# danping/CoSLAM

Measured on AMD Instinct MI355X. Metric: frames/sec for track+local-BA loop, 8 cams 640x480 x 2000 feats (one frame = all 8 cameras), higher is better.
Workload: dtype f32 (KLT, f16 pyramid storage) + f64 (pose, BA)

## Files before the change

### coslam_amd/csrc/ncc.hip

```cpp
#include "cs_common.h"
#include "small_ops.h"

#pragma clang fp contract(off)

namespace {

constexpr int NC_HW = 5, NC_BW = 11, NC_LEN = 121, NC_PITCH = 128;

__global__ __launch_bounds__(256) void k_ncc_blocks(const unsigned char* __restrict__ img, int W, int H, int n,
                                                    const double* __restrict__ xs, const double* __restrict__ ys, double scale,
                                                    unsigned char* __restrict__ blocks, double* __restrict__ abc,
                                                    int* __restrict__ valid) {
    const int lane = threadIdx.x & 63;
    const int i = blockIdx.x * 4 + (threadIdx.x >> 6);
    if (i >= n) return;
    const double x = xs[i] * scale, y = ys[i] * scale;
    const int x0 = (int)x, y0 = (int)y;
    const bool ok = !(x0 - NC_HW < 0 || x0 + NC_HW >= W || y0 - NC_HW < 0 || y0 + NC_HW >= H);
    unsigned v0 = 0x80, v1 = 0x80;
    if (ok) {
        const int j0 = lane, j1 = lane + 64;
        const int yy0 = j0 / NC_BW, xx0 = j0 - yy0 * NC_BW;
        v0 = img[(size_t)(y0 + yy0 - NC_HW) * W + (x0 + xx0 - NC_HW)];
        if (j1 < NC_LEN) {
            const int yy1 = j1 / NC_BW, xx1 = j1 - yy1 * NC_BW;
            v1 = img[(size_t)(y0 + yy1 - NC_HW) * W + (x0 + xx1 - NC_HW)];
        }
    }
    blocks[(size_t)i * NC_PITCH + lane] = (unsigned char)v0;
    blocks[(size_t)i * NC_PITCH + 64 + lane] = (unsigned char)v1;
    const unsigned w0 = ok ? v0 : 0u, w1 = (ok && lane + 64 < NC_LEN) ? v1 : 0u;
    unsigned a = w0 + w1;
    unsigned b = w0 * w0 + w1 * w1;
#pragma unroll
    for (int off = 32; off >= 1; off >>= 1) {
        a += __shfl_xor(a, off, 64);
        b += __shfl_xor(b, off, 64);
    }
    if (lane == 0) {
        valid[i] = ok ? 1 : 0;
        const double A = (double)a, B = (double)b;
        abc[4 * (size_t)i] = ok ? A : 0.0;
        abc[4 * (size_t)i + 1] = ok ? B : 0.0;
        abc[4 * (size_t)i + 2] = ok ? 1 / sqrt((double)NC_LEN * B - A * A) : 0.0;
        abc[4 * (size_t)i + 3] = ok ? A / (double)NC_LEN : 0.0;
    }
}

__device__ __forceinline__ int nc_floorf(float v) {
    const int i = (int)v;
    return i - (i > v);
}
__device__ __forceinline__ int nc_clip(int x, int a, int b) { return x >= a ? (x < b ? x : b - 1) : a; }
__device__ __forceinline__ int nc_sat_short(int v) { return v < -32768 ? -32768 : (v > 32767 ? 32767 : v); }

constexpr int NC_MAX_CAMS = 16;
struct NcCamSet {
    const unsigned char* img[NC_MAX_CAMS];
    unsigned char* scaled[NC_MAX_CAMS];
    const double* x[NC_MAX_CAMS];
    const double* y[NC_MAX_CAMS];
    unsigned char* blocks[NC_MAX_CAMS];
    double* abc[NC_MAX_CAMS];
    int* valid[NC_MAX_CAMS];
};

__global__ __launch_bounds__(256) void k_resize_linear_u8(NcCamSet S, int W, int H, double scale_x, double scale_y, int Wd, int Hd) {
    const unsigned char* __restrict__ src = S.img[blockIdx.z];
    unsigned char* __restrict__ dst = S.scaled[blockIdx.z];
    const int dx = blockIdx.x * 64 + (threadIdx.x & 63), dy = blockIdx.y * 4 + (threadIdx.x >> 6);
    if (dx >= Wd || dy >= Hd) return;
    float fx = (float)((dx + 0.5) * scale_x - 0.5);
    int sx = nc_floorf(fx);
    fx -= sx;
    if (sx < 0) fx = 0, sx = 0;
    bool edge = false;
    if (sx + 1 >= W) {
        edge = true;
        if (sx >= W - 1) fx = 0, sx = W - 1;
    }
    const int a0 = nc_sat_short(__float2int_rn((1.f - fx) * 2048.f)), a1 = nc_sat_short(__float2int_rn(fx * 2048.f));
    float fy = (float)((dy + 0.5) * scale_y - 0.5);
    const int sy = nc_floorf(fy);
    fy -= sy;
    const int b0 = nc_sat_short(__float2int_rn((1.f - fy) * 2048.f)), b1 = nc_sat_short(__float2int_rn(fy * 2048.f));
    const unsigned char* S0 = src + (size_t)nc_clip(sy, 0, H) * W;
    const unsigned char* S1 = src + (size_t)nc_clip(sy + 1, 0, H) * W;
    int r0, r1;
    if (!edge) {
        r0 = S0[sx] * a0 + S0[sx + 1] * a1;
        r1 = S1[sx] * a0 + S1[sx + 1] * a1;
    } else {
        r0 = S0[sx] * 2048;
        r1 = S1[sx] * 2048;
    }
    dst[(size_t)dy * Wd + dx] = (unsigned char)((((b0 * (r0 >> 4)) >> 16) + ((b1 * (r1 >> 4)) >> 16) + 2) >> 2);
}

__global__ __launch_bounds__(256) void k_ncc_blocks_subpix(NcCamSet S, int W, int H, int n, double scale, int scaled) {
    const int cam = blockIdx.y;
    const unsigned char* __restrict__ img = scaled ? S.scaled[cam] : S.img[cam];
    const double* __restrict__ xs = S.x[cam];
    const double* __restrict__ ys = S.y[cam];
    unsigned char* __restrict__ blocks = S.blocks[cam];
    double* __restrict__ abc = S.abc[cam];
    int* __restrict__ valid = S.valid[cam];
    const int lane = threadIdx.x & 63;
    const int p = blockIdx.x * 4 + (threadIdx.x >> 6);
    if (p >= n) return;
    const int win = NC_BW;
    const double px = scaled ? xs[p] * scale : xs[p], py = scaled ? ys[p] * scale : ys[p];
    float fxc = (float)px, fyc = (float)py;
    fxc -= (win - 1) * 0.5f;
    fyc -= (win - 1) * 0.5f;
    const int ipx = nc_floorf(fxc), ipy = nc_floorf(fyc);
    const float a = fxc - ipx, b = fyc - ipy;
    const int a11 = __float2int_rn((1.f - a) * (1.f - b) * 65536.f), a12 = __float2int_rn(a * (1.f - b) * 65536.f),
              a21 = __float2int_rn((1.f - a) * b * 65536.f), a22 = __float2int_rn(a * b * 65536.f);
    const int b1 = __float2int_rn((1.f - b) * 65536.f), b2 = __float2int_rn(b * 65536.f);
    const bool inside = 0 <= ipx && ipx < W - win && 0 <= ipy && ipy < H - win;
    int rx = 0, rw = win, ry = 0, rh = win, col0 = ipx, row0 = ipy;
    if (!inside) {
        if (ipx >= 0) {
            col0 = ipx, rx = 0;
        } else {
            col0 = 0, rx = -ipx;
            if (rx > win) rx = win;
        }
        if (ipx < W - win) {
            rw = win;
        } else {
            rw = W - ipx - 1;
            if (rw < 0) col0 += rw, rw = 0;
        }
        if (ipy >= 0) {
            row0 = ipy, ry = 0;
        } else {
            row0 = 0, ry = -ipy;
        }
        if (ipy < H - win) {
            rh = win;
        } else {
            rh = H - ipy - 1;
            if (rh < 0) row0 += rh, rh = 0;
        }
    }
    unsigned v[2] = {0x80u, 0x80u};
#pragma unroll
    for (int h = 0; h < 2; ++h) {
        const int q = lane + 64 * h;
        if (q >= NC_LEN) continue;
        const int i = q / win, j = q - i * win;
        int t;
        if (inside) {
            const unsigned char* s = img + (size_t)(ipy + i) * W + ipx;
            t = s[j] * a11 + s[j + 1] * a12 + s[j + W] * a21 + s[j + W + 1] * a22;
        } else {
            const int adv = (i < rh ? i : rh) - ry;
            const int rt = row0 + (adv > 0 ? adv : 0);
            const int rb = rt + ((i < ry || i >= rh) ? 0 : 1);
            const unsigned char* s = img + (size_t)rt * W + (col0 - rx);
            const unsigned char* s2 = img + (size_t)rb * W + (col0 - rx);
            if (j < rx)
                t = s[rx] * b1 + s2[rx] * b2;
            else if (j >= rw)
                t = s[rw] * b1 + s2[rw] * b2;
            else
                t = s[j] * a11 + s[j + 1] * a12 + s2[j] * a21 + s2[j + 1] * a22;
        }
        v[h] = (unsigned)((t + (1 << 15)) >> 16) & 0xffu;
    }
    blocks[(size_t)p * NC_PITCH + lane] = (unsigned char)v[0];
    blocks[(size_t)p * NC_PITCH + 64 + lane] = (unsigned char)v[1];
    const unsigned w0 = v[0], w1 = (lane + 64 < NC_LEN) ? v[1] : 0u;
    unsigned sa = w0 + w1;
    unsigned sb = w0 * w0 + w1 * w1;
#pragma unroll
    for (int off = 32; off >= 1; off >>= 1) {
        sa += __shfl_xor(sa, off, 64);
        sb += __shfl_xor(sb, off, 64);
    }
    if (lane == 0) {
        const double A = (double)sa, B = (double)sb;
        abc[4 * (size_t)p] = A;
        abc[4 * (size_t)p + 1] = B;
        abc[4 * (size_t)p + 2] = 1 / sqrt((double)NC_LEN * B - A * A);
        abc[4 * (size_t)p + 3] = A / (double)NC_LEN;
        if (valid) valid[p] = 1;
    }
}

__global__ __launch_bounds__(256) void k_ncc_unmapped_mask(int n, const int* __restrict__ state, const int* __restrict__ slot2map,
                                                           int* __restrict__ valid) {
    const int i = blockIdx.x * 256 + threadIdx.x;
    if (i < n) valid[i] = (state[i] >= 0 && slot2map[i] < 0) ? 1 : 0;
}

struct NcSide {
    const double* x;
    const double* y;
    const unsigned char* blocks;
    const double* abc;
    const int* valid;
    int n;
};
struct NcArgs {
    double F[9];
    const double* dF;
    NcSide s1, s2;
    double epiMax, nccMin, wNone;
    double* epiMat;
    double* nccMat;
    cs_ncc_pair* pairs;
    int pairCap;
    int* pairCount;
};

typedef int nc_i32x4 __attribute__((ext_vector_type(4)));

__device__ __forceinline__ long nc_row_chunk(const unsigned char* blocks, int row, int n, int byteOff) {
    if (row >= n) return 0;
    const unsigned long long u = *(const unsigned long long*)(blocks + (size_t)row * NC_PITCH + byteOff);
    return (long)(u ^ 0x8080808080808080ull);
}

constexpr int NC_MAX_JOBS = 8;
struct NcJobs {
    NcArgs job[NC_MAX_JOBS];
};
constexpr int NC_CT = 4;
constexpr int NC_TP = 136;
constexpr int NC_TILE_BYTES = 64 * NC_TP + 64 * 40;
struct NcColRegs {
    nc_i32x4 q0, q1;
    double x, y, A, C;
    int valid;
};
__device__ __forceinline__ void nc_tile_fetch(const NcSide& S2, int j0, int N, int tid, NcColRegs& r) {
    const int row = j0 + (tid >> 2);
    r.q0 = r.q1 = (nc_i32x4){0, 0, 0, 0};
    if (row < N) {
        const nc_i32x4* src = (const nc_i32x4*)(S2.blocks + (size_t)row * NC_PITCH + 32 * (tid & 3));
        r.q0 = src[0], r.q1 = src[1];
        const int sh = (int)0x80808080;
#pragma unroll
        for (int k = 0; k < 4; ++k) r.q0[k] ^= sh, r.q1[k] ^= sh;
    }
    r.x = r.y = r.A = r.C = 0.0, r.valid = 0;
    if (tid < 64 && j0 + tid < N) {
        const int j = j0 + tid;
        r.x = S2.x[j], r.y = S2.y[j], r.A = S2.abc[4 * (size_t)j], r.C = S2.abc[4 * (size_t)j + 2], r.valid = S2.valid[j];
    }
}
__device__ __forceinline__ void nc_tile_store(unsigned char* buf, int tid, const NcColRegs& r) {
    nc_i32x4* dst = (nc_i32x4*)(buf + (tid >> 2) * NC_TP + 32 * (tid & 3));
    long* d8 = (long*)dst;
    const long* s8 = (const long*)&r.q0;
    d8[0] = s8[0], d8[1] = s8[1];
    s8 = (const long*)&r.q1;
    d8[2] = s8[0], d8[3] = s8[1];
    if (tid < 64) {
        double* c = (double*)(buf + 64 * NC_TP);
        c[tid] = r.x, c[64 + tid] = r.y, c[128 + tid] = r.A, c[192 + tid] = r.C;
        ((int*)(c + 256))[tid] = r.valid;
    }
}
template <bool SPARSE>
__global__ __launch_bounds__(256) void k_ncc_epi_mat(NcJobs J) {
    __shared__ __attribute__((aligned(16))) unsigned char sTile[2][NC_TILE_BYTES];
    const NcArgs& A = J.job[blockIdx.z];
    const int tid = threadIdx.x, lane = tid & 63, wv = tid >> 6;
    const int M = A.s1.n, N = A.s2.n;
    if ((int)blockIdx.y * 64 >= M || (int)blockIdx.x * NC_CT * 64 >= N) return;
    const int i0 = blockIdx.y * 64 + 16 * wv;
    const bool rowsIn = i0 < M;
    double Fm[9];
#pragma unroll
    for (int k = 0; k < 9; ++k) Fm[k] = A.dF ? A.dF[k] : A.F[k];
    const int lr = lane & 15, lk = lane >> 4;
    long a[4];
#pragma unroll
    for (int ks = 0; ks < 4; ++ks) a[ks] = nc_row_chunk(A.s1.blocks, i0 + lr, M, 32 * ks + 8 * lk);
    double x1[4], y1[4], A1[4], C1[4];
    int v1[4], s1[4];
#pragma unroll
    for (int r = 0; r < 4; ++r) {
        const int i = i0 + 4 * lk + r;
        const bool in = i < M;
        x1[r] = in ? A.s1.x[i] : 0.0;
        y1[r] = in ? A.s1.y[i] : 0.0;
        A1[r] = in ? A.s1.abc[4 * (size_t)i] : 0.0;
        C1[r] = in ? A.s1.abc[4 * (size_t)i + 2] : 0.0;
        v1[r] = in ? A.s1.valid[i] : 0;
        s1[r] = (int)A1[r] - NC_LEN * 128;
    }
    const int jBase = blockIdx.x * NC_CT * 64;
    NcColRegs cr;
    nc_tile_fetch(A.s2, jBase, N, tid, cr);
    nc_tile_store(sTile[0], tid, cr);
    __syncthreads();
    for (int ct = 0; ct < NC_CT; ++ct) {
        const int j0 = jBase + ct * 64;
        if (j0 >= N) break;
        const bool more = ct + 1 < NC_CT && j0 + 64 < N;
        if (more) nc_tile_fetch(A.s2, j0 + 64, N, tid, cr);
        const unsigned char* tile = sTile[ct & 1];
        const double* cc = (const double*)(tile + 64 * NC_TP);
        const int* cv = (const int*)(cc + 256);
        if (rowsIn) {
            nc_i32x4 acc[4];
#pragma unroll
            for (int t = 0; t < 4; ++t) acc[t] = (nc_i32x4){0, 0, 0, 0};
#pragma unroll
            for (int ks = 0; ks < 4; ++ks) {
                const int off = 32 * ks + 8 * lk;
                long b[4];
#pragma unroll
                for (int t = 0; t < 4; ++t) b[t] = *(const long*)(tile + (16 * t + lr) * NC_TP + off);
#pragma unroll
                for (int t = 0; t < 4; ++t) acc[t] = __builtin_amdgcn_mfma_i32_16x16x32_i8(a[ks], b[t], acc[t], 0, 0, 0);
            }
#pragma unroll
            for (int t = 0; t < 4; ++t) {
                const int jl = 16 * t + lr, j = j0 + jl;
                if (j >= N) continue;
                const double bx = cc[jl], by = cc[64 + jl];
                const double A2 = cc[128 + jl], C2 = cc[192 + jl];
                const int v2 = cv[jl];
                const int s2 = (int)A2 - NC_LEN * 128;
                const double l0 = (Fm[0] * bx + Fm[1] * by) + Fm[2];
                const double l1 = (Fm[3] * bx + Fm[4] * by) + Fm[5];
                const double l2 = (Fm[6] * bx + Fm[7] * by) + Fm[8];
                const double nn = sqrt(l0 * l0 + l1 * l1);
                const double den = nn > 0 ? nn : 1.0;
                const double numMax = (A.epiMax * den) * (1.0 + 1e-12);
#pragma unroll
                for (int r = 0; r < 4; ++r) {
                    const int i = i0 + 4 * lk + r;
                    if (i >= M) continue;
                    const double num = fabs((l0 * x1[r] + l1 * y1[r]) + l2);
                    double e = A.wNone, c = A.wNone;
                    bool pass = false;
                    double epiErr = 0;
                    bool near = v1[r] && v2 && !(num > numMax);
                    if (near) {
                        epiErr = num / den;
                        near = epiErr <= A.epiMax;
                    }
                    if (near) {
                        const int d = acc[t][r] + 128 * s1[r] + 128 * s2 + NC_LEN * 128 * 128;
                        const double ncc = (((double)NC_LEN * (double)d - A1[r] * A2) * C1[r]) * C2;
                        if (ncc >= A.nccMin) {
                            e = epiErr;
                            c = ncc;
                            pass = true;
                        }
                    }
                    if (SPARSE) {
                        if (pass) {
                            const int at = atomicAdd(A.pairCount, 1);
                            if (at < A.pairCap) {
                                cs_ncc_pair q;
                                q.i = i, q.j = j, q.epi = e, q.ncc = c;
                                A.pairs[at] = q;
                            }
                        }
                    } else {
                        A.epiMat[(size_t)i * N + j] = e;
                        A.nccMat[(size_t)i * N + j] = c;
                    }
                }
            }
        }
        if (more) nc_tile_store(sTile[(ct + 1) & 1], tid, cr);
        __syncthreads();
    }
}

}

extern "C" int cs_ncc_blocks_dev(int device, void* hip_stream, const unsigned char* d_img, int W, int H, int n, const double* d_x,
                                 const double* d_y, double scale, unsigned char* d_blocks, double* d_abc, int* d_valid) {
    if (W < NC_BW || H < NC_BW || n < 0 || !(scale > 0)) {
        cs_set_error("cs_ncc_blocks_dev: bad arguments (image at least 11 x 11, scale > 0)");
        return CS_ERR_INVALID;
    }
    if (n == 0) return CS_OK;
    if (!d_img || !d_x || !d_y || !d_blocks || !d_abc || !d_valid) {
        cs_set_error("cs_ncc_blocks_dev: null pointer");
        return CS_ERR_INVALID;
    }
    CS_HIP(hipSetDevice(device));
    hipLaunchKernelGGL(k_ncc_blocks, dim3((unsigned)((n + 3) / 4)), dim3(256), 0, (hipStream_t)hip_stream, d_img, W, H, n, d_x, d_y,
                       scale, d_blocks, d_abc, d_valid);
    CS_CHECK_LAUNCH();
    return CS_OK;
}

extern "C" int cs_ncc_unmapped_mask_dev(int device, void* hip_stream, int n, const int* d_state, const int* d_slot2map, int* d_valid) {
    if (n < 0 || (n && (!d_state || !d_slot2map || !d_valid))) {
        cs_set_error("cs_ncc_unmapped_mask_dev: bad arguments");
        return CS_ERR_INVALID;
    }
    if (n == 0) return CS_OK;
    CS_HIP(hipSetDevice(device));
    hipLaunchKernelGGL(k_ncc_unmapped_mask, dim3((n + 255) / 256), dim3(256), 0, (hipStream_t)hip_stream, n, d_state, d_slot2map, d_valid);
    CS_CHECK_LAUNCH();
    return CS_OK;
}

extern "C" int cs_ncc_scaled_dims(int W, int H, double scale, int* Ws, int* Hs) {
    if (!Ws || !Hs || W <= 0 || H <= 0 || !(scale > 0)) {
        cs_set_error("cs_ncc_scaled_dims: bad arguments");
        return CS_ERR_INVALID;
    }
    *Ws = (int)lrint(W * scale);
    *Hs = (int)lrint(H * scale);
    return CS_OK;
}

static int ncc_get_blocks_group_impl(int device, void* hip_stream, int nCams, const cs_ncc_cam* cams, int W, int H, int n, double scale,
                                     bool writeValid);
extern "C" int cs_ncc_get_blocks_dev(int device, void* hip_stream, const unsigned char* d_img, int W, int H, int n, const double* d_x,
                                     const double* d_y, double scale, unsigned char* d_scaled, unsigned char* d_blocks, double* d_abc,
                                     int* d_valid) {
    if (!d_img || W <= 0 || H <= 0 || n < 0 || (n && (!d_x || !d_y || !d_blocks || !d_abc)) || !(scale > 0) ||
        (scale != 1.0 && !d_scaled)) {
        cs_set_error("cs_ncc_get_blocks_dev: bad arguments");
        return CS_ERR_INVALID;
    }
    cs_ncc_cam one;
    memset(&one, 0, sizeof(one));
    one.img = d_img, one.x = d_x, one.y = d_y, one.scaled = d_scaled, one.blocks = d_blocks, one.abc = d_abc, one.valid = d_valid;
    return ncc_get_blocks_group_impl(device, hip_stream, 1, &one, W, H, n, scale, true);
}

extern "C" int cs_ncc_get_blocks_group_dev(int device, void* hip_stream, int nCams, const cs_ncc_cam* cams, int W, int H, int n,
                                           double scale) {
    return ncc_get_blocks_group_impl(device, hip_stream, nCams, cams, W, H, n, scale, false);
}
static int ncc_get_blocks_group_impl(int device, void* hip_stream, int nCams, const cs_ncc_cam* cams, int W, int H, int n, double scale,
                                     bool writeValid) {
    if (nCams < 1 || nCams > NC_MAX_CAMS || !cams || W <= 0 || H <= 0 || n < 0 || !(scale > 0)) {
        cs_set_error("cs_ncc_get_blocks_group_dev: bad arguments (1..%d cameras)", NC_MAX_CAMS);
        return CS_ERR_INVALID;
    }
    NcCamSet S;
    memset(&S, 0, sizeof(S));
    for (int c = 0; c < nCams; ++c) {
        const cs_ncc_cam& q = cams[c];
        if (!q.img || (n && (!q.x || !q.y || !q.blocks || !q.abc)) || (scale != 1.0 && !q.scaled)) {
            cs_set_error("cs_ncc_get_blocks_group_dev: null pointer in camera %d", c);
            return CS_ERR_INVALID;
        }
        S.img[c] = q.img, S.scaled[c] = q.scaled, S.x[c] = q.x, S.y[c] = q.y, S.blocks[c] = q.blocks, S.abc[c] = q.abc, S.valid[c] = writeValid ? q.valid : nullptr;
    }
    CS_HIP(hipSetDevice(device));
    hipStream_t s = (hipStream_t)hip_stream;
    int Ws = W, Hs = H;
    if (scale != 1.0) {
        Ws = (int)lrint(W * scale), Hs = (int)lrint(H * scale);
        if (Ws < 1 || Hs < 1) {
            cs_set_error("cs_ncc_get_blocks_group_dev: the scaled image is empty");
            return CS_ERR_INVALID;
        }
        hipLaunchKernelGGL(k_resize_linear_u8, dim3((Ws + 63) / 64, (Hs + 3) / 4, nCams), dim3(256), 0, s, S, W, H, 1. / scale, 1. / scale, Ws, Hs);
    }
    if (n > 0) hipLaunchKernelGGL(k_ncc_blocks_subpix, dim3((n + 3) / 4, nCams), dim3(256), 0, s, S, Ws, Hs, n, scale, scale != 1.0 ? 1 : 0);
    CS_CHECK_LAUNCH();
    return CS_OK;
}

extern "C" int cs_ncc_get_scaled_blocks_group_dev(int device, void* hip_stream, int nCams, const cs_ncc_cam* cams, int Ws, int Hs, int n,
                                                  double scale) {
    if (nCams < 1 || nCams > NC_MAX_CAMS || !cams || Ws <= 0 || Hs <= 0 || n < 0 || !(scale > 0)) {
        cs_set_error("cs_ncc_get_scaled_blocks_group_dev: bad arguments (1..%d cameras)", NC_MAX_CAMS);
        return CS_ERR_INVALID;
    }
    NcCamSet S;
    memset(&S, 0, sizeof(S));
    for (int c = 0; c < nCams; ++c) {
        const cs_ncc_cam& q = cams[c];
        if (!q.img || (n && (!q.x || !q.y || !q.blocks || !q.abc))) {
            cs_set_error("cs_ncc_get_scaled_blocks_group_dev: null pointer in camera %d", c);
            return CS_ERR_INVALID;
        }
        S.img[c] = q.img, S.scaled[c] = const_cast<unsigned char*>(q.img) , S.x[c] = q.x, S.y[c] = q.y;
        S.blocks[c] = q.blocks, S.abc[c] = q.abc, S.valid[c] = nullptr;
    }
    if (n == 0) return CS_OK;
    CS_HIP(hipSetDevice(device));
    hipLaunchKernelGGL(k_ncc_blocks_subpix, dim3((n + 3) / 4, nCams), dim3(256), 0, (hipStream_t)hip_stream, S, Ws, Hs, n, scale, 1);
    CS_CHECK_LAUNCH();
    return CS_OK;
}

extern "C" int cs_ncc_small_dims(int W, int H, double scale, int* Ws, int* Hs) {
    if (!Ws || !Hs || W <= 0 || H <= 0 || !(scale > 0)) {
        cs_set_error("cs_ncc_small_dims: bad arguments");
        return CS_ERR_INVALID;
    }
    *Ws = (int)(W * scale);
    *Hs = (int)(H * scale);
    return CS_OK;
}
extern "C" int cs_ncc_small_image_dev(int device, void* hip_stream, const unsigned char* d_img, int W, int H, double scale,
                                      unsigned char* d_small) {
    int Ws = 0, Hs = 0;
    if (!d_img || !d_small || cs_ncc_small_dims(W, H, scale, &Ws, &Hs) != CS_OK || Ws < 1 || Hs < 1) {
        cs_set_error("cs_ncc_small_image_dev: bad arguments (%d x %d, scale %g)", W, H, scale);
        return CS_ERR_INVALID;
    }
    NcCamSet S;
    memset(&S, 0, sizeof(S));
    S.img[0] = d_img, S.scaled[0] = d_small;
    CS_HIP(hipSetDevice(device));
    const double inv_x = (double)Ws / W, inv_y = (double)Hs / H;
    hipLaunchKernelGGL(k_resize_linear_u8, dim3((Ws + 63) / 64, (Hs + 3) / 4, 1), dim3(256), 0, (hipStream_t)hip_stream, S, W, H, 1. / inv_x,
                       1. / inv_y, Ws, Hs);
    CS_CHECK_LAUNCH();
    return CS_OK;
}

extern "C" int cs_ncc_epi_mat_dev(int device, void* hip_stream, const double F[9], int M, const double* d_x1, const double* d_y1,
                                  const unsigned char* d_blocks1, const double* d_abc1, const int* d_valid1, int N,
                                  const double* d_x2, const double* d_y2, const unsigned char* d_blocks2, const double* d_abc2,
                                  const int* d_valid2, double epiMax, double nccMin, double wNone, double* d_epiMat,
                                  double* d_nccMat) {
    if (!F || M < 0 || N < 0) {
        cs_set_error("cs_ncc_epi_mat_dev: bad arguments");
        return CS_ERR_INVALID;
    }
    if (M == 0 || N == 0) return CS_OK;
    if (!d_x1 || !d_y1 || !d_blocks1 || !d_abc1 || !d_valid1 || !d_x2 || !d_y2 || !d_blocks2 || !d_abc2 || !d_valid2 || !d_epiMat ||
        !d_nccMat) {
        cs_set_error("cs_ncc_epi_mat_dev: null pointer");
        return CS_ERR_INVALID;
    }
    NcArgs A;
    memset(&A, 0, sizeof(A));
    memcpy(A.F, F, sizeof(A.F));
    A.s1 = {d_x1, d_y1, d_blocks1, d_abc1, d_valid1, M};
    A.s2 = {d_x2, d_y2, d_blocks2, d_abc2, d_valid2, N};
    A.epiMax = epiMax;
    A.nccMin = nccMin;
    A.wNone = wNone;
    A.epiMat = d_epiMat;
    A.nccMat = d_nccMat;
    CS_HIP(hipSetDevice(device));
    A.pairs = nullptr, A.pairCap = 0, A.pairCount = nullptr;
    NcJobs J;
    J.job[0] = A;
    hipLaunchKernelGGL(k_ncc_epi_mat<false>, dim3((unsigned)((N + 64 * NC_CT - 1) / (64 * NC_CT)), (unsigned)((M + 63) / 64)), dim3(256), 0,
                       (hipStream_t)hip_stream, J);
    CS_CHECK_LAUNCH();
    return CS_OK;
}

extern "C" int cs_ncc_epi_pairs_dev(int device, void* hip_stream, const double F[9], int M, const double* d_x1, const double* d_y1,
                                    const unsigned char* d_blocks1, const double* d_abc1, const int* d_valid1, int N, const double* d_x2,
                                    const double* d_y2, const unsigned char* d_blocks2, const double* d_abc2, const int* d_valid2,
                                    double epiMax, double nccMin, cs_ncc_pair* d_pairs, int pairCap, int* d_pairCount) {
    if (!F || M < 0 || N < 0 || pairCap < 0 || !d_pairCount || (pairCap > 0 && !d_pairs)) {
        cs_set_error("cs_ncc_epi_pairs_dev: bad arguments");
        return CS_ERR_INVALID;
    }
    CS_HIP(hipSetDevice(device));
    CS_HIP(hipMemsetAsync(d_pairCount, 0, sizeof(int), (hipStream_t)hip_stream));
    if (M == 0 || N == 0) return CS_OK;
    if (!d_x1 || !d_y1 || !d_blocks1 || !d_abc1 || !d_valid1 || !d_x2 || !d_y2 || !d_blocks2 || !d_abc2 || !d_valid2) {
        cs_set_error("cs_ncc_epi_pairs_dev: null pointer");
        return CS_ERR_INVALID;
    }
    NcArgs A;
    memset(&A, 0, sizeof(A));
    memcpy(A.F, F, sizeof(A.F));
    A.s1 = {d_x1, d_y1, d_blocks1, d_abc1, d_valid1, M};
    A.s2 = {d_x2, d_y2, d_blocks2, d_abc2, d_valid2, N};
    A.epiMax = epiMax;
    A.nccMin = nccMin;
    A.wNone = -1.0;
    A.epiMat = A.nccMat = nullptr;
    A.pairs = d_pairs, A.pairCap = pairCap, A.pairCount = d_pairCount;
    NcJobs J;
    J.job[0] = A;
    hipLaunchKernelGGL(k_ncc_epi_mat<true>, dim3((unsigned)((N + 64 * NC_CT - 1) / (64 * NC_CT)), (unsigned)((M + 63) / 64)), dim3(256), 0,
                       (hipStream_t)hip_stream, J);
    CS_CHECK_LAUNCH();
    return CS_OK;
}

struct NcFmArgs {
    int n;
    int camA[NC_MAX_JOBS], camB[NC_MAX_JOBS];
    const double* iK[NC_MAX_JOBS][2];
    const double *R, *t;
    double* F;
};
__global__ void k_ncc_fmats(NcFmArgs A) {
    const int k = threadIdx.x;
    if (k >= A.n) return;
    const double *Ra = A.R + 9 * A.camA[k], *Rb = A.R + 9 * A.camB[k], *ta = A.t + 3 * A.camA[k], *tb = A.t + 3 * A.camB[k];
    double R[9], t[3], E[9], T[9];
    for (int i = 0; i < 3; ++i)
        for (int j = 0; j < 3; ++j) R[3 * i + j] = (Ra[3 * i] * Rb[3 * j] + Ra[3 * i + 1] * Rb[3 * j + 1]) + Ra[3 * i + 2] * Rb[3 * j + 2];
    for (int i = 0; i < 3; ++i) t[i] = ta[i] - ((R[3 * i] * tb[0] + R[3 * i + 1] * tb[1]) + R[3 * i + 2] * tb[2]);
    const double X[9] = {0, -t[2], t[1], t[2], 0, -t[0], -t[1], t[0], 0};
    for (int i = 0; i < 3; ++i)
        for (int j = 0; j < 3; ++j) E[3 * i + j] = (X[3 * i] * R[j] + X[3 * i + 1] * R[3 + j]) + X[3 * i + 2] * R[6 + j];
    const double *Ka = A.iK[k][0], *Kb = A.iK[k][1];
    for (int i = 0; i < 3; ++i)
        for (int j = 0; j < 3; ++j) T[3 * i + j] = (Ka[i] * E[j] + Ka[3 + i] * E[3 + j]) + Ka[6 + i] * E[6 + j];
    for (int i = 0; i < 3; ++i)
        for (int j = 0; j < 3; ++j) A.F[9 * k + 3 * i + j] = (T[3 * i] * Kb[j] + T[3 * i + 1] * Kb[3 + j]) + T[3 * i + 2] * Kb[6 + j];
}
extern "C" int cs_ncc_fmats_dev(int device, void* hip_stream, int nCams, int nPairs, const int* camA, const int* camB, const double* const* d_iK,
                                const double* d_R, const double* d_t, double* d_F) {
    if (nCams < 1 || nPairs < 0 || nPairs > NC_MAX_JOBS || (nPairs && (!camA || !camB || !d_iK || !d_R || !d_t || !d_F))) {
        cs_set_error("cs_ncc_fmats_dev: bad arguments (<= %d pairs)", NC_MAX_JOBS);
        return CS_ERR_INVALID;
    }
    if (nPairs == 0) return CS_OK;
    NcFmArgs A;
    memset(&A, 0, sizeof(A));
    A.n = nPairs, A.R = d_R, A.t = d_t, A.F = d_F;
    for (int k = 0; k < nPairs; ++k) {
        if (camA[k] < 0 || camA[k] >= nCams || camB[k] < 0 || camB[k] >= nCams || !d_iK[camA[k]] || !d_iK[camB[k]]) {
            cs_set_error("cs_ncc_fmats_dev: bad pair %d", k);
            return CS_ERR_INVALID;
        }
        A.camA[k] = camA[k], A.camB[k] = camB[k], A.iK[k][0] = d_iK[camA[k]], A.iK[k][1] = d_iK[camB[k]];
    }
    CS_HIP(hipSetDevice(device));
    hipLaunchKernelGGL(k_ncc_fmats, dim3(1), dim3(64), 0, (hipStream_t)hip_stream, A);
    CS_CHECK_LAUNCH();
    return CS_OK;
}

extern "C" int cs_ncc_epi_pairs_group_dev(int device, void* hip_stream, int nCams, const cs_ncc_cam* cams, int n, int nJobs,
                                          const cs_ncc_pair_job* jobs, double epiMax, double nccMin, int pairCap) {
    if (nCams < 1 || nCams > NC_MAX_CAMS || !cams || n < 0 || nJobs < 0 || nJobs > NC_MAX_JOBS || (nJobs && !jobs) || pairCap < 0) {
        cs_set_error("cs_ncc_epi_pairs_group_dev: bad arguments (<= %d camera pairs per call)", NC_MAX_JOBS);
        return CS_ERR_INVALID;
    }
    if (nJobs == 0) return CS_OK;
    CS_HIP(hipSetDevice(device));
    hipStream_t s = (hipStream_t)hip_stream;
    NcJobs J;
    memset(&J, 0, sizeof(J));
    cs_small::List zero;
    for (int k = 0; k < nJobs; ++k) {
        const cs_ncc_pair_job& q = jobs[k];
        if (q.camA < 0 || q.camA >= nCams || q.camB < 0 || q.camB >= nCams || !q.count || (pairCap > 0 && !q.pairs)) {
            cs_set_error("cs_ncc_epi_pairs_group_dev: bad job %d", k);
            return CS_ERR_INVALID;
        }
        const cs_ncc_cam &a = cams[q.camA], &b = cams[q.camB];
        if (n && (!a.x || !a.y || !a.blocks || !a.abc || !a.valid || !b.x || !b.y || !b.blocks || !b.abc || !b.valid)) {
            cs_set_error("cs_ncc_epi_pairs_group_dev: null pointer in a camera of job %d", k);
            return CS_ERR_INVALID;
        }
        NcArgs& A = J.job[k];
        memcpy(A.F, q.F, sizeof(A.F));
        A.dF = q.dF;
        A.s1 = {a.x, a.y, a.blocks, a.abc, a.valid, n};
        A.s2 = {b.x, b.y, b.blocks, b.abc, b.valid, n};
        A.epiMax = epiMax, A.nccMin = nccMin, A.wNone = -1.0;
        A.epiMat = A.nccMat = nullptr;
        A.pairs = q.pairs, A.pairCap = pairCap, A.pairCount = q.count;
        zero.fill(q.count, 0, sizeof(int));
    }
    CS_HIP(zero.run(s));
    if (n == 0) return CS_OK;
    hipLaunchKernelGGL(k_ncc_epi_mat<true>, dim3((unsigned)((n + 64 * NC_CT - 1) / (64 * NC_CT)), (unsigned)((n + 63) / 64), (unsigned)nJobs), dim3(256), 0, s, J);
    CS_CHECK_LAUNCH();
    return CS_OK;
}

static int ncc_match_between_impl(int cutter, int device, const unsigned char* img1, int W1, int H1, int M, const double* x1,
                                  const double* y1, const unsigned char* img2, int W2, int H2, int N, const double* x2, const double* y2,
                                  double scale, const double F[9], double epiMax, double nccMin, double wNone, double* epiMat,
                                  double* nccMat, unsigned char* blocks1, double* abc1, int* valid1, unsigned char* blocks2,
                                  double* abc2, int* valid2) {
    if (!img1 || !img2 || !F || M < 0 || N < 0 || (M && (!x1 || !y1)) || (N && (!x2 || !y2)) || (M && N && (!epiMat || !nccMat))) {
        cs_set_error("cs_ncc_match_between: bad arguments");
        return CS_ERR_INVALID;
    }
    if (M == 0 || N == 0) return CS_OK;
    CS_HIP(hipSetDevice(device));
    const size_t i1 = (size_t)W1 * H1, i2 = (size_t)W2 * H2;
    auto al = [](size_t v) { return (v + 255) & ~(size_t)255; };
    size_t off = 0;
    const size_t oI1 = off; off += al(i1);
    const size_t oI2 = off; off += al(i2);
    const size_t oX1 = off; off += al(8 * (size_t)M);
    const size_t oY1 = off; off += al(8 * (size_t)M);
    const size_t oX2 = off; off += al(8 * (size_t)N);
    const size_t oY2 = off; off += al(8 * (size_t)N);
    const size_t inBytes = off;
    const size_t oB1 = off; off += al(128 * (size_t)M);
    const size_t oB2 = off; off += al(128 * (size_t)N);
    const size_t oC1 = off; off += al(32 * (size_t)M);
    const size_t oC2 = off; off += al(32 * (size_t)N);
    const size_t oV1 = off; off += al(4 * (size_t)M);
    const size_t oV2 = off; off += al(4 * (size_t)N);
    const size_t oE = off; off += al(8 * (size_t)M * N);
    const size_t oN = off; off += al(8 * (size_t)M * N);
    const size_t oS1 = off; off += al(cutter ? i1 : 0);
    const size_t oS2 = off; off += al(cutter ? i2 : 0);
    char* d = nullptr;
    if (hipMalloc((void**)&d, off) != hipSuccess) {
        cs_set_error("cs_ncc_match_between: out of device memory (%zu bytes)", off);
        return CS_ERR_HIP;
    }
    hipStream_t s = nullptr;
    int rc = CS_OK;
    hipError_t e = hipMemcpyAsync(d + oI1, img1, i1, hipMemcpyHostToDevice, s);
    if (e == hipSuccess) e = hipMemcpyAsync(d + oI2, img2, i2, hipMemcpyHostToDevice, s);
    if (e == hipSuccess) e = hipMemcpyAsync(d + oX1, x1, 8 * (size_t)M, hipMemcpyHostToDevice, s);
    if (e == hipSuccess) e = hipMemcpyAsync(d + oY1, y1, 8 * (size_t)M, hipMemcpyHostToDevice, s);
    if (e == hipSuccess) e = hipMemcpyAsync(d + oX2, x2, 8 * (size_t)N, hipMemcpyHostToDevice, s);
    if (e == hipSuccess) e = hipMemcpyAsync(d + oY2, y2, 8 * (size_t)N, hipMemcpyHostToDevice, s);
    (void)inBytes;
    if (cutter && scale > 1.0) {
        (void)hipFree(d);
        cs_set_error("cs_ncc_match_between_full: scale > 1 is not supported");
        return CS_ERR_INVALID;
    }
    if (e == hipSuccess && cutter) {
        rc = cs_ncc_get_blocks_dev(device, s, (const unsigned char*)(d + oI1), W1, H1, M, (const double*)(d + oX1), (const double*)(d + oY1),
                                   scale, (unsigned char*)(d + oS1), (unsigned char*)(d + oB1), (double*)(d + oC1), (int*)(d + oV1));
        if (rc == CS_OK)
            rc = cs_ncc_get_blocks_dev(device, s, (const unsigned char*)(d + oI2), W2, H2, N, (const double*)(d + oX2),
                                       (const double*)(d + oY2), scale, (unsigned char*)(d + oS2), (unsigned char*)(d + oB2),
                                       (double*)(d + oC2), (int*)(d + oV2));
        if (rc == CS_OK)
            rc = cs_ncc_epi_mat_dev(device, s, F, M, (const double*)(d + oX1), (const double*)(d + oY1), (const unsigned char*)(d + oB1),
                                    (const double*)(d + oC1), (const int*)(d + oV1), N, (const double*)(d + oX2),
                                    (const double*)(d + oY2), (const unsigned char*)(d + oB2), (const double*)(d + oC2),
                                    (const int*)(d + oV2), epiMax, nccMin, wNone, (double*)(d + oE), (double*)(d + oN));
    } else if (e == hipSuccess) {
        rc = cs_ncc_blocks_dev(device, s, (const unsigned char*)(d + oI1), W1, H1, M, (const double*)(d + oX1), (const double*)(d + oY1),
                               scale, (unsigned char*)(d + oB1), (double*)(d + oC1), (int*)(d + oV1));
        if (rc == CS_OK)
            rc = cs_ncc_blocks_dev(device, s, (const unsigned char*)(d + oI2), W2, H2, N, (const double*)(d + oX2),
                                   (const double*)(d + oY2), scale, (unsigned char*)(d + oB2), (double*)(d + oC2), (int*)(d + oV2));
        if (rc == CS_OK)
            rc = cs_ncc_epi_mat_dev(device, s, F, M, (const double*)(d + oX1), (const double*)(d + oY1), (const unsigned char*)(d + oB1),
                                    (const double*)(d + oC1), (const int*)(d + oV1), N, (const double*)(d + oX2),
                                    (const double*)(d + oY2), (const unsigned char*)(d + oB2), (const double*)(d + oC2),
                                    (const int*)(d + oV2), epiMax, nccMin, wNone, (double*)(d + oE), (double*)(d + oN));
    }
    if (rc == CS_OK && e == hipSuccess) e = hipMemcpyAsync(epiMat, d + oE, 8 * (size_t)M * N, hipMemcpyDeviceToHost, s);
    if (rc == CS_OK && e == hipSuccess) e = hipMemcpyAsync(nccMat, d + oN, 8 * (size_t)M * N, hipMemcpyDeviceToHost, s);
    auto back = [&](void* dst, size_t o, size_t bytes) {
        if (dst && rc == CS_OK && e == hipSuccess) e = hipMemcpyAsync(dst, d + o, bytes, hipMemcpyDeviceToHost, s);
    };
    back(blocks1, oB1, 128 * (size_t)M);
    back(blocks2, oB2, 128 * (size_t)N);
    back(abc1, oC1, 32 * (size_t)M);
    back(abc2, oC2, 32 * (size_t)N);
    back(valid1, oV1, 4 * (size_t)M);
    back(valid2, oV2, 4 * (size_t)N);
    if (rc == CS_OK && e == hipSuccess) e = hipStreamSynchronize(s);
    (void)hipFree(d);
    if (rc != CS_OK) return rc;
    if (e != hipSuccess) {
        cs_set_error("cs_ncc_match_between: %s", hipGetErrorString(e));
        return CS_ERR_HIP;
    }
    return CS_OK;
}

extern "C" int cs_ncc_match_between(int device, const unsigned char* img1, int W1, int H1, int M, const double* x1, const double* y1,
                                    const unsigned char* img2, int W2, int H2, int N, const double* x2, const double* y2,
                                    double scale, const double F[9], double epiMax, double nccMin, double wNone, double* epiMat,
                                    double* nccMat, unsigned char* blocks1, double* abc1, int* valid1, unsigned char* blocks2,
                                    double* abc2, int* valid2) {
    return ncc_match_between_impl(0, device, img1, W1, H1, M, x1, y1, img2, W2, H2, N, x2, y2, scale, F, epiMax, nccMin, wNone, epiMat,
                                  nccMat, blocks1, abc1, valid1, blocks2, abc2, valid2);
}

extern "C" int cs_ncc_match_between_full(int device, const unsigned char* img1, int W1, int H1, int M, const double* x1, const double* y1,
                                         const unsigned char* img2, int W2, int H2, int N, const double* x2, const double* y2,
                                         double scale, const double F[9], double epiMax, double nccMin, double wNone, double* epiMat,
                                         double* nccMat, unsigned char* blocks1, double* abc1, unsigned char* blocks2, double* abc2) {
    return ncc_match_between_impl(1, device, img1, W1, H1, M, x1, y1, img2, W2, H2, N, x2, y2, scale, F, epiMax, nccMin, wNone, epiMat,
                                  nccMat, blocks1, abc1, nullptr, blocks2, abc2, nullptr);
}
```

### coslam_amd/csrc/newpts.hip

```cpp
#include "cs_common.h"
#include "small_ops.h"

#pragma clang fp contract(off)

namespace {

constexpr int NP_MAX_CAMS = 16, NP_MAX_CAND = 2048, NP_MAX_SEEDS = 512, NP_MAX_TRACKS = 4096, NP_MAX_N = 32768;
constexpr int NP_MAX_DYN = 4096;
constexpr int NP_SEGS = 8;
constexpr int NP_DYN_PER_CAM = 1024;

struct NpArgs {
    int nCams, N, mapCap, curFrame, pairCap, minLen, W, H;
    double maxDisp, maxRpErr, sigma;
    const cs_ncc_pair* pairs[NP_MAX_CAMS];
    const int* pairCount[NP_MAX_CAMS];
    cs_poseupdate_cam cam[NP_MAX_CAMS];
    const double *R, *t;
    double *mapPts, *mapCov;
    unsigned char *mapFlags, *newPt;
    int *firstFrame, *pointFeat;
    int* mapCount;
    int* matchIdx;
    unsigned* rowMask;
    unsigned* colMask;
    int* seedIdx;
    int* seedCnt;
    unsigned* dynList;
    int* dynCnt;
    int* counts;
};

__device__ __forceinline__ bool np_before(double sa, unsigned ia, double sb, unsigned ib) {
    return sa > sb || (sa == sb && ia < ib);
}

__global__ __launch_bounds__(256) void k_np_prep(NpArgs A) {
    __shared__ int wTot[4];
    __shared__ int sBase;
    const int tid = threadIdx.x, lane = tid & 63, wv = tid >> 6, N = A.N, C = A.nCams, nP = C - 1;
    if (blockIdx.x == 0 && A.counts && tid < 4 + C) A.counts[tid] = 0;
    if ((int)blockIdx.x < nP * NP_SEGS) {
        const int a = blockIdx.x / NP_SEGS, seg = blockIdx.x % NP_SEGS, b = a + 1;
        const int cap = *A.mapCount < A.mapCap ? *A.mapCount : A.mapCap;
        const int per = ((cap + NP_SEGS - 1) / NP_SEGS + 255) / 256 * 256;
        const int m0 = seg * per, m1 = min(m0 + per, cap);
        int* out = A.seedIdx + ((size_t)a * NP_SEGS + seg) * NP_MAX_SEEDS;
        if (tid == 0) sBase = 0;
        __syncthreads();
        for (int c0 = m0; c0 < m1 && sBase < NP_MAX_SEEDS; c0 += 256) {
            const int m = c0 + tid;
            bool in = false;
            if (m < m1) {
                const unsigned char fl = A.mapFlags[m];
                in = !(fl & (CS_MAP_FALSE | CS_MAP_UNCERTAIN)) && A.pointFeat[(size_t)m * C + a] >= 0 && A.pointFeat[(size_t)m * C + b] >= 0;
            }
            const unsigned long long bal = __builtin_amdgcn_ballot_w64(in);
            if (lane == 0) wTot[wv] = __popcll(bal);
            __syncthreads();
            int k = sBase;
            for (int w = 0; w < wv; ++w) k += wTot[w];
            k += __popcll(bal & ((1ull << lane) - 1ull));
            if (in && k < NP_MAX_SEEDS) out[k] = m;
            __syncthreads();
            if (tid == 0) sBase = min(sBase + wTot[0] + wTot[1] + wTot[2] + wTot[3], NP_MAX_SEEDS);
            __syncthreads();
        }
        if (tid == 0) A.seedCnt[a * NP_SEGS + seg] = sBase;
        return;
    }
    const int c = blockIdx.x - nP * NP_SEGS;
    if (c >= C) return;
    if (tid == 0) sBase = 0;
    __syncthreads();
    for (int sl = tid; sl < N; sl += 256) {
        const int st = A.cam[c].state[sl], m = A.cam[c].slot2map[sl];
        if ((st == 0 || st == 1) && m >= 0 && m < A.mapCap && A.mapFlags[m] == CS_MAP_DYNAMIC) {
            const int x = (int)(A.cam[c].xy[sl] + 0.5), y = (int)(A.cam[c].xy[N + sl] + 0.5);
            if (x + 20 >= 0 && x - 20 < A.W && y + 20 >= 0 && y - 20 < A.H) {
                const int k = atomicAdd(&sBase, 1);
                if (k < NP_DYN_PER_CAM) A.dynList[(size_t)c * NP_DYN_PER_CAM + k] = ((unsigned)(y + 64) << 12) | (unsigned)(x + 64);
            }
        }
    }
    __syncthreads();
    if (tid == 0) A.dynCnt[c] = sBase;
}

__global__ __launch_bounds__(256) void k_np_match(NpArgs A) {
    __shared__ double sKey[NP_MAX_CAND];
    __shared__ unsigned sIdx[NP_MAX_CAND];
    __shared__ double sSeed[NP_MAX_SEEDS][4];
    __shared__ unsigned sRow[NP_MAX_N / 32], sCol[NP_MAX_N / 32];
    __shared__ int sNSeeds, sNCand;
    const int a = blockIdx.x, b = a + 1, tid = threadIdx.x, lane = tid & 63, wv = tid >> 6, N = A.N, C = A.nCams;
    const int nWords = (N + 31) / 32;
    for (int q = tid; q < nWords; q += 256) sRow[q] = 0, sCol[q] = 0;
    {
        int off[NP_SEGS + 1];
        off[0] = 0;
#pragma unroll
        for (int g = 0; g < NP_SEGS; ++g) off[g + 1] = off[g] + A.seedCnt[a * NP_SEGS + g];
        const int total = off[NP_SEGS] < NP_MAX_SEEDS ? off[NP_SEGS] : NP_MAX_SEEDS;
        if (tid == 0) sNSeeds = total, sNCand = 0;
        for (int k = tid; k < total; k += 256) {
            int g = 0, base = 0;
#pragma unroll
            for (int q = 1; q < NP_SEGS; ++q)
                if (k >= off[q]) g = q, base = off[q];
            const int m = A.seedIdx[((size_t)a * NP_SEGS + g) * NP_MAX_SEEDS + (k - base)];
            const int s1 = A.pointFeat[(size_t)m * C + a], s2 = A.pointFeat[(size_t)m * C + b];
            const double x1 = A.cam[a].xy[s1], y1 = A.cam[a].xy[N + s1], x2 = A.cam[b].xy[s2], y2 = A.cam[b].xy[N + s2];
            sSeed[k][0] = x1, sSeed[k][1] = y1, sSeed[k][2] = x2 - x1, sSeed[k][3] = y2 - y1;
        }
    }
    __syncthreads();
    const int nSeeds = sNSeeds;
    int nAll = *A.pairCount[a];
    if (nAll > A.pairCap) {
        nAll = A.pairCap;
        if (tid == 0 && A.counts) atomicOr(A.counts + 3, 1);
    }
    for (int q = wv; q < nAll; q += 4) {
        const cs_ncc_pair p = A.pairs[a][q];
        bool ok = p.i >= 0 && p.i < N && p.j >= 0 && p.j < N;
        if (ok && nSeeds > 0) {
            const double x1 = A.cam[a].xy[p.i], y1 = A.cam[a].xy[N + p.i];
            double best = 1.0e300;
            int bk = 0x7fffffff;
            for (int k = lane; k < nSeeds; k += 64) {
                const double dx = sSeed[k][0] - x1, dy = sSeed[k][1] - y1, d2 = dx * dx + dy * dy;
                if (d2 < best) best = d2, bk = k;
            }
#pragma unroll
            for (int off = 1; off < 64; off <<= 1) {
                const double ob = __shfl_xor(best, off, 64);
                const int ok_ = __shfl_xor(bk, off, 64);
                if (ob < best || (ob == best && ok_ < bk)) best = ob, bk = ok_;
            }
            if (bk == 0x7fffffff) bk = 0;
            const double ex = (A.cam[b].xy[p.j] - x1) - sSeed[bk][2];
            const double ey = (A.cam[b].xy[N + p.j] - y1) - sSeed[bk][3];
            ok = sqrt(ex * ex + ey * ey) <= A.maxDisp;
        }
        if (ok && lane == 0) {
            const int k = atomicAdd(&sNCand, 1);
            if (k < NP_MAX_CAND) sKey[k] = p.ncc, sIdx[k] = ((unsigned)p.i << 16) | (unsigned)p.j;
        }
    }
    __syncthreads();
    int L = sNCand;
    if (L > NP_MAX_CAND) {
        L = NP_MAX_CAND;
        if (tid == 0 && A.counts) atomicOr(A.counts + 3, 1);
    }
    int L2 = 1;
    while (L2 < L) L2 <<= 1;
    for (int q = L + tid; q < L2; q += 256) sKey[q] = -1.0e300, sIdx[q] = 0xFFFFFFFFu;
    __syncthreads();
    for (int k = 2; k <= L2; k <<= 1)
        for (int j = k >> 1; j > 0; j >>= 1) {
            for (int q = tid; q < L2; q += 256) {
                const int x = q ^ j;
                if (x > q) {
                    const bool up = (q & k) == 0;
                    const double ka = sKey[q], kb = sKey[x];
                    const unsigned ia = sIdx[q], ib = sIdx[x];
                    if (np_before(kb, ib, ka, ia) == up) sKey[q] = kb, sIdx[q] = ib, sKey[x] = ka, sIdx[x] = ia;
                }
            }
            __syncthreads();
        }
    if (tid == 0) {
        int n = 0;
        int* match = A.matchIdx + (size_t)a * N;
        for (int q = 0; q < L; ++q) {
            const unsigned id = sIdx[q], i = id >> 16, j = id & 0xFFFFu;
            if ((sRow[i >> 5] >> (i & 31)) & 1u) continue;
            if ((sCol[j >> 5] >> (j & 31)) & 1u) continue;
            sRow[i >> 5] |= 1u << (i & 31), sCol[j >> 5] |= 1u << (j & 31);
            match[i] = (int)j;
            ++n;
        }
        if (A.counts) A.counts[4 + a] = n;
    }
    __syncthreads();
    for (int q = tid; q < nWords; q += 256) A.rowMask[(size_t)a * nWords + q] = sRow[q], A.colMask[(size_t)a * nWords + q] = sCol[q];
}

constexpr int NP_LPT = 8;
constexpr int NP_TPB = 256 / NP_LPT;
static_assert(NP_MAX_CAMS <= 2 * NP_LPT, "a lane holds two views of a track");

struct NpTerm {
    double n[6], g[3];
};
__device__ __forceinline__ double np_pick(double a, double b, bool second) { return second ? b : a; }
__device__ __forceinline__ int np_pick_i(int a, int b, bool second) { return second ? b : a; }

__global__ __launch_bounds__(256) void k_np_reconstruct(NpArgs A) {
    __shared__ int sBase, sNTracks, sWave[4];
    __shared__ unsigned sTrk[NP_MAX_TRACKS];
    __shared__ int sDynOff[NP_MAX_CAMS + 2];
    const int tid = threadIdx.x, N = A.N, C = A.nCams, nP = C - 1;
    const int lane = tid & 63, wv = tid >> 6, r = tid & (NP_LPT - 1), gbase = lane & ~(NP_LPT - 1);
    if (tid == 0) sBase = 0, sNTracks = 0;
    __syncthreads();
    const int nWords = (N + 31) / 32, totalW = nP * nWords;
    for (int w0 = 0; w0 < totalW; w0 += 256) {
        const int w = w0 + tid;
        unsigned bits = 0;
        int a = 0, q = 0;
        if (w < totalW) {
            a = w / nWords, q = w - a * nWords;
            bits = A.rowMask[w];
            if (a > 0) bits &= ~A.colMask[(size_t)(a - 1) * nWords + q];
        }
        const int cnt = __popc(bits);
        int inc = cnt;
#pragma unroll
        for (int o = 1; o < 64; o <<= 1) {
            const int v = __shfl_up(inc, o, 64);
            if (lane >= o) inc += v;
        }
        if (lane == 63) sWave[wv] = inc;
        __syncthreads();
        int before = inc - cnt, total = 0;
        for (int k = 0; k < 4; ++k) {
            if (k < wv) before += sWave[k];
            total += sWave[k];
        }
        int rank = sNTracks + before;
        while (bits) {
            const int bit = __ffs(bits) - 1;
            bits &= bits - 1;
            if (rank < NP_MAX_TRACKS) sTrk[rank] = ((unsigned)a << 16) | (unsigned)(32 * q + bit);
            ++rank;
        }
        __syncthreads();
        if (tid == 0) sNTracks = min(sNTracks + total, NP_MAX_TRACKS);
        __syncthreads();
    }
    const int nTracks = sNTracks;
    int nLong = 0;
    for (int t0 = 0; t0 < nTracks; t0 += NP_TPB) {
        const int tk = t0 + tid / NP_LPT;
        int nv = 0, c0 = 0, vs0 = -1, vs1 = -1;
        if (tk < nTracks) {
            int c = (int)(sTrk[tk] >> 16), sl = (int)(sTrk[tk] & 0xFFFFu);
            c0 = c;
            for (;;) {
                if ((nv & (NP_LPT - 1)) == r) (nv < NP_LPT ? vs0 : vs1) = sl;
                ++nv;
                if (c >= nP || !((A.rowMask[(size_t)c * nWords + (sl >> 5)] >> (sl & 31)) & 1u)) break;
                sl = A.matchIdx[(size_t)c * N + sl];
                ++c;
            }
        }
        const bool lng = tk < nTracks && nv >= A.minLen;
        if (lng && r == 0) ++nLong;
        bool valid = false;
        double M[3] = {0, 0, 0}, cov[9] = {0, 0, 0, 0, 0, 0, 0, 0, 0}, err0 = 0, err1 = 0;
        unsigned char fl = 0;
        {
            NpTerm T0, T1;
#pragma unroll
            for (int kk = 0; kk < 2; ++kk) {
                NpTerm& T = kk ? T1 : T0;
#pragma unroll
                for (int q = 0; q < 6; ++q) T.n[q] = 0;
#pragma unroll
                for (int q = 0; q < 3; ++q) T.g[q] = 0;
                const int k = r + NP_LPT * kk, sl = kk ? vs1 : vs0;
                if (!lng || k >= nv) continue;
                const int cam = c0 + k;
                const cs_poseupdate_cam& Cm = A.cam[cam];
                const double* R = A.R + 9 * cam;
                const double* t = A.t + 3 * cam;
                const double mx = Cm.xy[sl], my = Cm.xy[N + sl];
                const double* iK = Cm.iK;
                const double w = (iK[6] * mx + iK[7] * my) + iK[8];
                const double x = ((iK[0] * mx + iK[1] * my) + iK[2]) / w, y = ((iK[3] * mx + iK[4] * my) + iK[5]) / w;
                const double a0[3] = {R[0] - x * R[6], R[1] - x * R[7], R[2] - x * R[8]}, a1[3] = {R[3] - y * R[6], R[4] - y * R[7], R[5] - y * R[8]};
                const double b0 = x * t[2] - t[0], b1 = y * t[2] - t[1];
                T.n[0] = a0[0] * a0[0] + a1[0] * a1[0];
                T.n[1] = a0[0] * a0[1] + a1[0] * a1[1];
                T.n[2] = a0[0] * a0[2] + a1[0] * a1[2];
                T.n[3] = a0[1] * a0[1] + a1[1] * a1[1];
                T.n[4] = a0[1] * a0[2] + a1[1] * a1[2];
                T.n[5] = a0[2] * a0[2] + a1[2] * a1[2];
#pragma unroll
                for (int q = 0; q < 3; ++q) T.g[q] = a0[q] * b0 + a1[q] * b1;
            }
            double Nn[6] = {0, 0, 0, 0, 0, 0}, g[3] = {0, 0, 0};
            for (int k = 0; k < NP_MAX_CAMS; ++k) {
                if (!__builtin_amdgcn_ballot_w64(lng && k < nv)) break;
                const int src = gbase + (k & (NP_LPT - 1));
                const bool second = k >= NP_LPT;
                double tn[6], tg[3];
#pragma unroll
                for (int q = 0; q < 6; ++q) tn[q] = __shfl(np_pick(T0.n[q], T1.n[q], second), src, 64);
#pragma unroll
                for (int q = 0; q < 3; ++q) tg[q] = __shfl(np_pick(T0.g[q], T1.g[q], second), src, 64);
                if (lng && k < nv) {
#pragma unroll
                    for (int q = 0; q < 6; ++q) Nn[q] = Nn[q] + tn[q];
#pragma unroll
                    for (int q = 0; q < 3; ++q) g[q] = g[q] + tg[q];
                }
            }
            double cf[6];
            if (lng) {
                cf[0] = Nn[3] * Nn[5] - Nn[4] * Nn[4], cf[1] = Nn[2] * Nn[4] - Nn[1] * Nn[5], cf[2] = Nn[1] * Nn[4] - Nn[2] * Nn[3];
                cf[3] = Nn[0] * Nn[5] - Nn[2] * Nn[2], cf[4] = Nn[1] * Nn[2] - Nn[0] * Nn[4], cf[5] = Nn[0] * Nn[3] - Nn[1] * Nn[1];
                const double det = (Nn[0] * cf[0] + Nn[1] * cf[1]) + Nn[2] * cf[2];
                M[0] = ((cf[0] * g[0] + cf[1] * g[1]) + cf[2] * g[2]) / det;
                M[1] = ((cf[1] * g[0] + cf[3] * g[1]) + cf[4] * g[2]) / det;
                M[2] = ((cf[2] * g[0] + cf[4] * g[1]) + cf[5] * g[2]) / det;
            }
            double S0[6], S1[6];
            bool out = false, dyn0 = false, dyn1 = false;
#pragma unroll
            for (int kk = 0; kk < 2; ++kk) {
                double* Sx = kk ? S1 : S0;
#pragma unroll
                for (int q = 0; q < 6; ++q) Sx[q] = 0;
                const int k = r + NP_LPT * kk, sl = kk ? vs1 : vs0;
                if (!lng || k >= nv) continue;
                const int cam = c0 + k;
                const cs_poseupdate_cam& Cm = A.cam[cam];
                const double* K = Cm.K;
                const double* R = A.R + 9 * cam;
                const double* t = A.t + 3 * cam;
                const double X = ((R[0] * M[0] + R[1] * M[1]) + R[2] * M[2]) + t[0];
                const double Y = ((R[3] * M[0] + R[4] * M[1]) + R[5] * M[2]) + t[1];
                const double Z = ((R[6] * M[0] + R[7] * M[1]) + R[8] * M[2]) + t[2];
                const double u = (K[0] * X + K[1] * Y) + K[2] * Z, vv = (K[3] * X + K[4] * Y) + K[5] * Z, w = (K[6] * X + K[7] * Y) + K[8] * Z;
                const double dx = Cm.xy[sl] - u / w, dy = Cm.xy[N + sl] - vv / w;
                const double e = sqrt(dx * dx + dy * dy);
                (kk ? err1 : err0) = e;
                if (e > A.maxRpErr || Z < 0) out = true;
                if (Cm.isStatic && !Cm.isStatic[sl]) (kk ? dyn1 : dyn0) = true;
                double KR[9], J[6];
#pragma unroll
                for (int i = 0; i < 3; ++i)
#pragma unroll
                    for (int j = 0; j < 3; ++j) KR[3 * i + j] = (K[3 * i] * R[j] + K[3 * i + 1] * R[3 + j]) + K[3 * i + 2] * R[6 + j];
                const double ww = w * w;
#pragma unroll
                for (int j = 0; j < 3; ++j) J[j] = (KR[j] * w - u * KR[6 + j]) / ww, J[3 + j] = (KR[3 + j] * w - vv * KR[6 + j]) / ww;
                Sx[0] = J[0] * J[0] + J[3] * J[3];
                Sx[1] = J[0] * J[1] + J[3] * J[4];
                Sx[2] = J[0] * J[2] + J[3] * J[5];
                Sx[3] = J[1] * J[1] + J[4] * J[4];
                Sx[4] = J[1] * J[2] + J[4] * J[5];
                Sx[5] = J[2] * J[2] + J[5] * J[5];
            }
            double S[6] = {0, 0, 0, 0, 0, 0};
            int nDyn = (dyn0 ? 1 : 0) + (dyn1 ? 1 : 0);
            for (int k = 0; k < NP_MAX_CAMS; ++k) {
                if (!__builtin_amdgcn_ballot_w64(lng && k < nv)) break;
                const int src = gbase + (k & (NP_LPT - 1));
                const bool second = k >= NP_LPT;
                double ts[6];
#pragma unroll
                for (int q = 0; q < 6; ++q) ts[q] = __shfl(np_pick(S0[q], S1[q], second), src, 64);
                if (lng && k < nv) {
#pragma unroll
                    for (int q = 0; q < 6; ++q) S[q] = S[q] + ts[q];
                }
            }
#pragma unroll
            for (int o = 1; o < NP_LPT; o <<= 1) {
                out |= __shfl_xor((int)out, o, 64) != 0;
                nDyn += __shfl_xor(nDyn, o, 64);
            }
            if (lng && !out) {
                valid = true;
                cf[0] = S[3] * S[5] - S[4] * S[4], cf[1] = S[2] * S[4] - S[1] * S[5], cf[2] = S[1] * S[4] - S[2] * S[3];
                cf[3] = S[0] * S[5] - S[2] * S[2], cf[4] = S[1] * S[2] - S[0] * S[4], cf[5] = S[0] * S[3] - S[1] * S[1];
                const double dS = (S[0] * cf[0] + S[1] * cf[1]) + S[2] * cf[2], s2 = A.sigma * A.sigma;
                cov[0] = (cf[0] / dS) * s2, cov[1] = (cf[1] / dS) * s2, cov[2] = (cf[2] / dS) * s2;
                cov[3] = cov[1], cov[4] = (cf[3] / dS) * s2, cov[5] = (cf[4] / dS) * s2;
                cov[6] = cov[2], cov[7] = cov[5], cov[8] = (cf[5] / dS) * s2;
                fl = nDyn > 1 ? CS_MAP_DYNAMIC : CS_MAP_UNCERTAIN;
            }
        }
        const unsigned long long lead = __builtin_amdgcn_ballot_w64(valid && r == 0);
        if (lane == 0) sWave[wv] = __popcll(lead);
        __syncthreads();
        int before = sBase + __popcll(lead & ((1ull << gbase) - 1ull)), total = 0;
        for (int k = 0; k < 4; ++k) {
            if (k < wv) before += sWave[k];
            total += sWave[k];
        }
        const int m = *A.mapCount + before;
        if (valid) {
            if (m < A.mapCap) {
                if (r < 3) A.mapPts[3 * (size_t)m + r] = M[r];
                double cr = cov[0];
#pragma unroll
                for (int q = 1; q < 8; ++q) cr = r == q ? cov[q] : cr;
                A.mapCov[9 * (size_t)m + r] = cr;
                if (r == 0) A.mapCov[9 * (size_t)m + 8] = cov[8], A.mapFlags[m] = fl, A.newPt[m] = 1, A.firstFrame[m] = A.curFrame;
#pragma unroll
                for (int kk = 0; kk < 2; ++kk) {
                    const int c = r + NP_LPT * kk, k = c - c0;
                    const int kSafe = (k >= 0 && k < nv) ? k : 0;
                    const int src = gbase + (kSafe & (NP_LPT - 1));
                    const int sv0 = __shfl(vs0, src, 64), sv1 = __shfl(vs1, src, 64);
                    const int sv = np_pick_i(sv0, sv1, kSafe >= NP_LPT);
                    if (c < C) A.pointFeat[(size_t)m * C + c] = (k >= 0 && k < nv) ? sv : -1;
                }
#pragma unroll
                for (int kk = 0; kk < 2; ++kk) {
                    const int k = r + NP_LPT * kk, sl = kk ? vs1 : vs0;
                    if (k >= nv) continue;
                    const_cast<int*>(A.cam[c0 + k].slot2map)[sl] = m;
                    if (A.cam[c0 + k].reprojErr) A.cam[c0 + k].reprojErr[sl] = kk ? err1 : err0;
                }
            } else if (A.counts && r == 0) {
                atomicOr(A.counts + 3, 2);
            }
        }
        __syncthreads();
        if (tid == 0) sBase += total;
        __syncthreads();
    }
    if (nLong && A.counts) atomicAdd(A.counts + 2, nLong);
    __syncthreads();
    const int first = *A.mapCount;
    int added = sBase;
    if (first + added > A.mapCap) added = A.mapCap - first;
    bool anyUncertain = false;
    for (int q = tid; q < added; q += 256) anyUncertain |= A.mapFlags[first + q] == CS_MAP_UNCERTAIN;
    if (__syncthreads_or(anyUncertain ? 1 : 0)) {
        __shared__ int sNDyn;
        unsigned* sDyn = sTrk;
        static_assert(NP_MAX_TRACKS >= NP_MAX_DYN && NP_MAX_CAMS <= 256 && NP_MAX_N <= 65536, "the dynamic features' list reuses the track table");
        int off = 0;
        bool over = false;
        for (int c = 0; c < C; ++c) {
            int n = A.dynCnt[c];
            if (n > NP_DYN_PER_CAM) n = NP_DYN_PER_CAM, over = true;
            if (off + n > NP_MAX_DYN) n = NP_MAX_DYN - off, over = true;
            if (tid == 0) sDynOff[c] = off;
            for (int k = tid; k < n; k += 256) sDyn[off + k] = A.dynList[(size_t)c * NP_DYN_PER_CAM + k];
            off += n;
        }
        if (tid == 0) sDynOff[C] = off, sNDyn = off;
        __syncthreads();
        for (int q = tid; q < added; q += 256) {
            const int m = first + q;
            if (A.mapFlags[m] != CS_MAP_DYNAMIC) continue;
            for (int c = 0; c < C; ++c) {
                const int sl = A.pointFeat[(size_t)m * C + c];
                if (sl < 0) continue;
                const int x = (int)(A.cam[c].xy[sl] + 0.5), y = (int)(A.cam[c].xy[N + sl] + 0.5);
                if (x + 20 >= 0 && x - 20 < A.W && y + 20 >= 0 && y - 20 < A.H) {
                    const int k = atomicAdd(&sNDyn, 1);
                    if (k < NP_MAX_DYN) sDyn[k] = ((unsigned)c << 24) | ((unsigned)(y + 64) << 12) | (unsigned)(x + 64);
                }
            }
        }
        __syncthreads();
        int nDynF = sNDyn;
        if (nDynF > NP_MAX_DYN) nDynF = NP_MAX_DYN, over = true;
        if (over && tid == 0 && A.counts) atomicOr(A.counts + 3, 4);
        const int offNew = sDynOff[C];
        for (int q0 = 0; q0 < added; q0 += NP_TPB) {
            const int q = q0 + tid / NP_LPT, m = first + q;
            const bool unc = q < added && A.mapFlags[m] == CS_MAP_UNCERTAIN;
            bool hit = false;
            if (unc) {
                for (int c = 0; c < C; ++c) {
                    const int sl = A.pointFeat[(size_t)m * C + c];
                    if (sl < 0) continue;
                    const int x = (int)(A.cam[c].xy[sl] + 0.5), y = (int)(A.cam[c].xy[N + sl] + 0.5);
                    if (x < 0 || x >= A.W || y < 0 || y >= A.H) continue;
                    for (int k = sDynOff[c] + r; k < sDynOff[c + 1]; k += NP_LPT) {
                        const unsigned d = sDyn[k];
                        const int dx = (int)(d & 0xFFFu) - 64 - x, dy = (int)((d >> 12) & 0xFFFu) - 64 - y;
                        hit |= dx >= -20 && dx <= 20 && dy >= -20 && dy <= 20;
                    }
                    for (int k = offNew + r; k < nDynF; k += NP_LPT) {
                        const unsigned d = sDyn[k];
                        if ((int)(d >> 24) != c) continue;
                        const int dx = (int)(d & 0xFFFu) - 64 - x, dy = (int)((d >> 12) & 0xFFFu) - 64 - y;
                        hit |= dx >= -20 && dx <= 20 && dy >= -20 && dy <= 20;
                    }
                }
            }
#pragma unroll
            for (int o = 1; o < NP_LPT; o <<= 1) hit |= __shfl_xor((int)hit, o, 64) != 0;
            if (unc && !hit && r == 0) A.mapFlags[m] = 0;
        }
    }
    if (tid == 0) {
        if (A.counts) A.counts[0] = added, A.counts[1] = nTracks;
        *A.mapCount = first + added;
    }
}

__global__ __launch_bounds__(256) void k_np_candidates(int n, int N, const int* __restrict__ state, const int* __restrict__ slot2map,
                                                       const int* __restrict__ trackSpan, const unsigned char* __restrict__ mapFlags, int mapCap,
                                                       int minTrack, int* __restrict__ valid, size_t validStride) {
    const int q = blockIdx.x * 256 + threadIdx.x;
    if (q >= n) return;
    const int c = q / N, s = q - c * N;
    const int st = state[q], m = slot2map[q];
    const int f1 = trackSpan[(size_t)c * 2 * N + s], f2 = trackSpan[(size_t)c * 2 * N + N + s];
    const bool tracked = (st == 0 || st == 1) && f1 >= 0 && f2 - f1 >= minTrack;
    const bool freeOrFalse = m < 0 || (m < mapCap && (mapFlags[m] & CS_MAP_FALSE));
    valid[(size_t)c * validStride + s] = tracked && freeOrFalse ? 1 : 0;
}

}

extern "C" size_t cs_newpts_scratch_bytes(int nCams, int N) {
    if (nCams < 2 || N < 1) return 0;
    const size_t nP = (size_t)nCams - 1, nW = ((size_t)N + 31) / 32;
    return sizeof(int) * (nP * ((size_t)N + 2 * nW) + nP * NP_SEGS * (NP_MAX_SEEDS + 1) + (size_t)nCams * (NP_DYN_PER_CAM + 1));
}

extern "C" int cs_ncc_candidate_mask_dev(int device, void* hip_stream, int nCams, int N, const int* d_state, const int* d_slot2map,
                                         const int* d_trackSpan, const unsigned char* d_mapFlags, int mapCap, int minTrack, int* d_valid,
                                         size_t validStride) {
    if (nCams < 1 || N < 1 || !d_state || !d_slot2map || !d_trackSpan || !d_mapFlags || !d_valid || (validStride && validStride < (size_t)N)) {
        cs_set_error("cs_ncc_candidate_mask_dev: bad arguments");
        return CS_ERR_INVALID;
    }
    CS_HIP(hipSetDevice(device));
    hipLaunchKernelGGL(k_np_candidates, dim3((nCams * N + 255) / 256), dim3(256), 0, (hipStream_t)hip_stream, nCams * N, N, d_state, d_slot2map,
                       d_trackSpan, d_mapFlags, mapCap, minTrack, d_valid, validStride ? validStride : (size_t)N);
    CS_CHECK_LAUNCH();
    return CS_OK;
}

extern "C" int cs_newpts_from_pairs_dev(int device, void* hip_stream, int nCams, int N, const cs_poseupdate_cam* cams,
                                        const cs_ncc_pair* const* d_pairs, const int* const* d_pairCount, int pairCap, const double* d_R,
                                        const double* d_t, double* d_mapPts, double* d_mapCov, unsigned char* d_mapFlags, unsigned char* d_newPt,
                                        int* d_firstFrame, int* d_pointFeat, int mapCap, int* d_mapCount, int curFrame, double maxDisp,
                                        double maxRpErr, double pixelErrVar, int minLen, int W, int H, void* d_scratch, int* d_counts) {
    if (W < 1 || H < 1 || W > 4011 || H > 4011) {
        cs_set_error("cs_newpts_from_pairs_dev: frame size 1..4011");
        return CS_ERR_INVALID;
    }
    if (nCams < 2 || nCams > NP_MAX_CAMS || N < 1 || N > NP_MAX_N || !cams || !d_pairs || !d_pairCount || pairCap < 1 || !d_R || !d_t || !d_mapPts ||
        !d_mapCov || !d_mapFlags || !d_newPt || !d_firstFrame || !d_pointFeat || mapCap < 1 || !d_mapCount || !d_scratch || minLen < 2) {
        cs_set_error("cs_newpts_from_pairs_dev: bad arguments (2..%d cameras, N <= %d)", NP_MAX_CAMS, NP_MAX_N);
        return CS_ERR_INVALID;
    }
    NpArgs A;
    memset(&A, 0, sizeof(A));
    A.nCams = nCams, A.N = N, A.mapCap = mapCap, A.curFrame = curFrame, A.pairCap = pairCap, A.minLen = minLen, A.W = W, A.H = H;
    A.maxDisp = maxDisp, A.maxRpErr = maxRpErr, A.sigma = pixelErrVar;
    for (int a = 0; a + 1 < nCams; ++a) {
        if (!d_pairs[a] || !d_pairCount[a]) {
            cs_set_error("cs_newpts_from_pairs_dev: null candidate list of camera pair %d", a);
            return CS_ERR_INVALID;
        }
        A.pairs[a] = d_pairs[a], A.pairCount[a] = d_pairCount[a];
    }
    for (int c = 0; c < nCams; ++c) {
        if (!cams[c].K || !cams[c].iK || !cams[c].xy || !cams[c].state || !cams[c].slot2map) {
            cs_set_error("cs_newpts_from_pairs_dev: null pointer in camera %d (K, iK, xy, state, slot2map)", c);
            return CS_ERR_INVALID;
        }
        A.cam[c] = cams[c];
    }
    A.R = d_R, A.t = d_t, A.mapPts = d_mapPts, A.mapCov = d_mapCov, A.mapFlags = d_mapFlags, A.newPt = d_newPt, A.firstFrame = d_firstFrame;
    A.pointFeat = d_pointFeat, A.mapCount = d_mapCount, A.matchIdx = (int*)d_scratch;
    A.rowMask = (unsigned*)d_scratch + (size_t)(nCams - 1) * N, A.colMask = A.rowMask + (size_t)(nCams - 1) * ((N + 31) / 32);
    A.seedIdx = (int*)(A.colMask + (size_t)(nCams - 1) * ((N + 31) / 32));
    A.seedCnt = A.seedIdx + (size_t)(nCams - 1) * NP_SEGS * NP_MAX_SEEDS;
    A.dynList = (unsigned*)(A.seedCnt + (size_t)(nCams - 1) * NP_SEGS);
    A.dynCnt = (int*)(A.dynList + (size_t)nCams * NP_DYN_PER_CAM);
    A.counts = d_counts;
    CS_HIP(hipSetDevice(device));
    hipStream_t s = (hipStream_t)hip_stream;
    hipLaunchKernelGGL(k_np_prep, dim3((nCams - 1) * NP_SEGS + nCams), dim3(256), 0, s, A);
    hipLaunchKernelGGL(k_np_match, dim3(nCams - 1), dim3(256), 0, s, A);
    hipLaunchKernelGGL(k_np_reconstruct, dim3(1), dim3(256), 0, s, A);
    CS_CHECK_LAUNCH();
    return CS_OK;
}
```

### coslam_amd/frameloop.py

```python
import contextlib
import ctypes as C
import hashlib
import os
import sys
import time

import numpy as np

import coslam_amd
from coslam_amd._lib import check
from coslam_amd.ba import BAInterCam, BAOutput, BAWindow, BAWorkspace, intercam_cams
from coslam_amd.grouping import CameraGroups, camera_grouping_dev, camera_grouping_scratch_bytes, grouping_cams
from coslam_amd.merge import MergeCandidates, merge_cams, merge_check_dev, merge_check_scratch_bytes
from coslam_amd.handback import handback_cams, handback_dev
from coslam_amd.liveview import LiveView
from coslam_amd.keyframe import keyframe_cams, keyframe_ready_dev, keyframe_snapshot_dev
from coslam_amd.ncc import (NCC_PAIR_DTYPE, ncc_cams, ncc_epi_pairs_group_dev, ncc_fmats_dev, ncc_get_blocks_group_dev, ncc_pair_jobs,
                            ncc_scaled_dims)
from coslam_amd.newpts import NewPtsJob, ncc_candidate_mask_dev, newpts_from_pairs_dev, newpts_scratch_bytes
from coslam_amd.pose import intraCamEstimate_batch_dev
from coslam_amd.poseupdate import TrackHistory, poseupdate_cams
from coslam_amd.register import (register_cams, register_cur_static_sequential_dev, register_decide_kinds_rounds_dev,
                                 register_decide_scratch_bytes, register_decide_static_dev, register_list_current_dev, register_passes,
                                 register_revisit_decide_dev, register_revisit_list_dev, register_revisit_rounds_dev,
                                 register_search_passes_dev)
from coslam_amd.results import loop_export_results
from coslam_amd.synth import csr_of_problem

PIXEL_ERR_VAR = 10.0
MAX_EPI_ERR = 6.0


class LoopConfig:
    def __init__(self, **kw):
        self.n_cams, self.W, self.H, self.levels, self.fw, self.fh = 8, 640, 480, 4, 50, 40
        self.pts_stride, self.n_col_blk, self.n_row_blk = 192, 16, 12
        self.key_every, self.n_key_frames = 5, 5
        self.ba_lag = 0
        self.p_reg = 4096
        self.hist = 64
        self.hist_store = 4096
        self.verdict_check_every = 100
        self.merge_tol_pix = 0.5
        self.pixel_err_reading = "variance"
        self.with_active_search = False
        self.ncc_every, self.ncc_pair_cap = 4, 1 << 16
        self.map_spare = 8192
        self.klt_cams_per_launch = 0
        self.klt_xcd_placement = True
        self.intracam_mapping = False
        self.keyframe_decision = False
        self.keyframe_drives = False
        self.keyframe_lag = 0
        self.keyframe_ratio = 0.93
        self.fused_registration = True
        self.feature_chains = True
        self.klt_fused = True
        self.prefetch = True
        self.with_pose_update = self.with_classify = self.with_register = self.with_mergability = self.with_ncc = True
        self.with_joint = self.with_intercam = True
        self.with_decide = True
        self.merge_every = 50
        self.revisit_rounds = 2
        self.sequential_registration = False
        self.native_comm = True
        self.klt_cus = 0
        self.pose_cus = 0
        self.klt_after_intracam = False
        self.device_wait = False
        self.camera_grouping = False
        self.group_min_overlap_num, self.group_min_overlap_area_ratio = 0, 0.0
        self.group_max_dist_ratio = 6.0
        self.merge_check = False
        self.merge_min_in_num, self.merge_min_in_area_ratio = 10, 0.5
        self.merge_max_cam_dist = 6.0
        self.live_view = False
        self.live_view_every, self.live_view_depth, self.live_view_trail_depth = 1, 8, 150
        self.live_view_cur_cap, self.live_view_dyn_cap = 0, 0
        self.export_frames = 0
        for k, v in kw.items():
            if not hasattr(self, k):
                raise TypeError(f"LoopConfig: unknown field {k}")
            setattr(self, k, v)

    @property
    def n_feat(self):
        return self.fw * self.fh


class FrameLoop:

    def __init__(self, cfg, scene, video, ic, klt_cfg, map_cov, rank=0, world=1, device=0, dist_backend="nccl", associate=None):
        import torch

        self.torch = torch
        self.cfg, self.sc, self.ic = cfg, scene, ic
        if cfg.pixel_err_reading not in ("variance", "std"):
            raise ValueError("LoopConfig.pixel_err_reading: 'variance' or 'std'")
        self.sig = (lambda v: float(np.sqrt(v))) if cfg.pixel_err_reading == "variance" else (lambda v: float(v))
        self.sig_pix = self.sig(PIXEL_ERR_VAR)
        self.rank, self.world, self.device = rank, world, device
        NA = cfg.n_cams
        if NA % world:
            raise ValueError(f"{NA} cameras do not shard over {world} ranks")
        if cfg.keyframe_drives and world > 1 and cfg.keyframe_lag <= 0:
            raise ValueError("LoopConfig.keyframe_drives: one rank only (the host reads the decision back every frame); keyframe_lag > 0 has every "
                             "rank read its replica's decision")
        self.nc = NA // world
        self.c0 = rank * self.nc
        self.my_cams = list(range(self.c0, self.c0 + self.nc))
        self.lag = cfg.ba_lag if cfg.ba_lag > 0 else min(max(world, 2), 4)
        if cfg.keyframe_drives and cfg.keyframe_lag > 0 and cfg.keyframe_lag >= self.lag * cfg.key_every:
            raise ValueError(f"LoopConfig.keyframe_lag {cfg.keyframe_lag}: must be below the BA apply lag of {self.lag} x {cfg.key_every} frames")
        if cfg.export_frames > 0 and not (cfg.with_pose_update and cfg.feature_chains):
            raise ValueError("LoopConfig.export_frames: the export reads the pose history and the feature references (with_pose_update, feature_chains)")
        if (cfg.n_key_frames - 1 + self.lag) * cfg.key_every + 1 > cfg.hist:
            raise ValueError("the pose history is shorter than a window + its apply lag")
        self.dev = torch.device("cuda", device)
        self.T = int(next(iter(video.values())).shape[0])
        self.video = video
        self.associate = associate
        self._timing = {} if os.environ.get("FRAMELOOP_TIMING") else None
        self._marks = [] if os.environ.get("FRAMELOOP_GPU_SECTIONS") else None
        self.grouping = None
        self.merge = None
        self.live = None
        self.setup_state(map_cov)
        self.setup_trackers(klt_cfg)
        self.setup_comm(dist_backend)
        self.setup_cameras()
        self.setup_registration()
        self.setup_keyframe_solves()
        self._init_ncc()

    def _z(self, shape, dt):
        return self.torch.zeros(shape, dtype=dt, device=self.dev)

    def setup_state(self, map_cov):
        torch, cfg, sc, dev, z = self.torch, self.cfg, self.sc, self.dev, self._z
        NA, N = cfg.n_cams, cfg.n_feat
        n_pts = len(sc.points)
        n_map = self.n_map = n_pts + cfg.map_spare
        f64, i32, u8 = torch.float64, torch.int32, torch.uint8
        K = np.ascontiguousarray(sc.K, dtype=np.float64)
        self.d_K = torch.from_numpy(np.tile(K.ravel(), NA)).to(dev)
        self.d_K1 = torch.from_numpy(K.ravel().copy()).to(dev)
        self.d_iK1 = torch.from_numpy(np.linalg.inv(K).ravel().copy()).to(dev)
        self.d_kud = z(7, f64)
        self.d_map = z((n_map, 3), f64)
        self.d_map[:n_pts] = torch.from_numpy(np.ascontiguousarray(sc.points, dtype=np.float64).copy()).to(dev)
        self.d_cov = z(n_map * 9, f64)
        self.d_cov[:n_pts * 9] = torch.from_numpy(np.ascontiguousarray(map_cov, dtype=np.float64).reshape(-1)[:n_pts * 9].copy()).to(dev)
        self.d_mapcount = torch.tensor([n_pts], dtype=i32, device=dev)
        self.n_pts0 = n_pts
        self.d_mapflags = z(n_map, u8)
        self.d_newpt, self.d_sfn, self.d_firstfrm = z(n_map, u8), z(n_map, i32), z(n_map, i32)
        self.d_slot2map = torch.full((NA, N), -1, dtype=i32, device=dev)
        self.d_trackspan = torch.full((NA, 2 * N), -1, dtype=i32, device=dev)
        self.d_xy, self.d_state = z((NA, 2 * N), f64), z((NA, N), i32)
        self.d_Ms, self.d_ms, self.d_sel = z((NA, cfg.pts_stride, 3), f64), z((NA, cfg.pts_stride, 2), f64), z((NA, cfg.pts_stride), i32)
        self.d_npts, self.d_opt, self.d_ok = z(NA, i32), z((NA, 96), u8), z(NA, i32)
        self.d_isstatic, self.d_reproj = torch.ones((NA, N), dtype=u8, device=dev), z((NA, N), f64)
        self.d_pf = torch.full((n_map, NA), -1, dtype=i32, device=dev)
        R0 = np.stack([sc.pose(c, 0)[0].ravel() for c in range(NA)])
        t0 = np.stack([sc.pose(c, 0)[1] for c in range(NA)])
        self.d_R = [torch.from_numpy(R0.copy()).to(dev), torch.from_numpy(R0.copy()).to(dev)]
        self.d_t = [torch.from_numpy(t0.copy()).to(dev), torch.from_numpy(t0.copy()).to(dev)]
        self.d_dests = [[z(N * 5, i32) for _ in range(self.nc)] for _ in range(2)]
        self.d_counts = [z(4, i32) for _ in range(self.nc)]
        self.d_cls_counts, self.d_apply_counts = z(2, i32), z(3, i32)
        self.d_mergeable = z((n_map, NA), u8)
        self.reg_out = dict(slot=torch.full((n_map, NA), -1, dtype=i32, device=dev), m=z((n_map, NA, 2), f64), var=z((n_map, NA, 4), f64),
                            dist=z((n_map, NA), f64), flags=z((n_map, NA), i32))
        self.d_curlist, self.d_curcount = torch.full((n_map,), -1, dtype=i32, device=dev), z(1, i32)
        self.d_curoverflow = z(1, i32)
        self.d_merge_counts = z(4, i32)

    def setup_trackers(self, klt_cfg):
        torch, cfg, dev, device = self.torch, self.cfg, self.dev, self.device
        self.klt_s, self.pose_s = torch.cuda.Stream(device=dev), torch.cuda.Stream(device=dev)
        if cfg.klt_cus > 0 or cfg.pose_cus > 0:
            L_ = coslam_amd.lib()
            if cfg.klt_cus > 0:
                h_ = L_.cs_stream_create_cu_range(device, 0, int(cfg.klt_cus))
                if not h_:
                    raise coslam_amd.CoslamHipError("cs_stream_create_cu_range: " + L_.cs_last_error().decode())
                self.klt_s = torch.cuda.ExternalStream(h_, device=dev)
            if cfg.pose_cus > 0:
                h_ = L_.cs_stream_create_cu_range(device, 256 - int(cfg.pose_cus), int(cfg.pose_cus))
                if not h_:
                    raise coslam_amd.CoslamHipError("cs_stream_create_cu_range: " + L_.cs_last_error().decode())
                self.pose_s = torch.cuda.ExternalStream(h_, device=dev)
        self.intracam_done = [torch.cuda.Event(), torch.cuda.Event()]
        self.klt_done = [torch.cuda.Event(), torch.cuda.Event()]
        self.dest_free = [torch.cuda.Event(), torch.cuda.Event()]
        self.trks = []
        for _ in self.my_cams:
            t = coslam_amd.KLT_SequenceTracker(klt_cfg, device=device)
            t.allocate(cfg.W, cfg.H, cfg.levels, cfg.fw, cfg.fh)
            if not cfg.klt_fused:
                t.set_fused(False)
            self.trks.append(t)
        self.grp = coslam_amd.KLT_TrackerGroup(self.trks)
        self.grp.set_stream(self.klt_s.cuda_stream)
        for t in self.trks:
            t.set_xcd_placement(cfg.klt_xcd_placement)
        if cfg.klt_cams_per_launch > 0:
            for t in self.trks:
                t.set_cu_count(min(256, (250 * cfg.klt_cams_per_launch + 60) // 8 + 5))
        elif cfg.klt_cus > 0:
            for t in self.trks:
                t.set_cu_count(int(cfg.klt_cus))
        self.stage_slot, self.h_frames = {}, None

    def setup_comm(self, dist_backend):
        self.xchg = self.native = self.native_fallback = None
        if self.world == 1:
            return
        from coslam_amd import multicam

        if self.cfg.native_comm and dist_backend == "nccl":
            import torch.distributed as dist_

            err = None
            try:
                self.native = multicam.NativeComm(self.world, self.rank, self.device)
            except coslam_amd.CoslamHipError as ex:
                err = str(ex)
            ok = self.torch.tensor([0 if err else 1], dtype=self.torch.int32, device=self.dev)
            dist_.all_reduce(ok, op=dist_.ReduceOp.MIN)
            if int(ok.item()) == 0:
                if self.native is not None:
                    self.native.close()
                    self.native = None
                self.native_fallback = err or "another rank could not create its communicator"
                print(f"[frameloop rank {self.rank}] libcoslam_hip's RCCL communicator is not available ({self.native_fallback}): "
                      "torch.distributed collectives instead", file=sys.stderr, flush=True)
        self.xchg = multicam.CameraExchange(self.cfg.n_feat * self.nc, self.dev, native=self.native, cams_per_rank=self.nc)

    def setup_cameras(self):
        torch, cfg, z = self.torch, self.cfg, self._z
        NA, N, nc, c0, n_map = cfg.n_cams, cfg.n_feat, self.nc, self.c0, self.n_map

        def hb_cam(g, dest):
            return dict(dest=dest, K=self.d_K1.data_ptr(), kud=self.d_kud.data_ptr(), mapPts=self.d_map.data_ptr(),
                        slot2map=self.d_slot2map[g].data_ptr(), trackSpan=self.d_trackspan[g].data_ptr(), xy=self.d_xy[g].data_ptr(),
                        state=self.d_state[g].data_ptr(), Ms=self.d_Ms[g].data_ptr(), ms=self.d_ms[g].data_ptr(), sel=self.d_sel[g].data_ptr(),
                        npts=self.d_npts[g:g + 1].data_ptr(), opt=self.d_opt[g].data_ptr(), pointFeat=self.d_pf.data_ptr() + 4 * g,
                        pointFeatStride=NA, nPointFeat=n_map, isStatic=(self.d_isstatic[g].data_ptr() if cfg.with_pose_update else 0))

        self.hb_own = [handback_cams([hb_cam(c0 + i, self.d_dests[b][i].data_ptr()) for i in range(nc)]) for b in range(2)]
        self.hb_other = None
        if self.world > 1:
            others = [g for g in range(NA) if g not in self.my_cams]
            self.hb_other = handback_cams([hb_cam(g, self.xchg.record_ptr(g, self.device)) for g in others])
        self.hb_all = handback_cams([hb_cam(g, self.d_dests[0][0].data_ptr()) for g in range(NA)])
        self.dest_ptrs = [[d.data_ptr() for d in self.d_dests[b]] for b in range(2)]
        self.cnt_ptrs = [c.data_ptr() for c in self.d_counts]
        self.img_ptrs = [[self.video[c][f].data_ptr() for c in self.my_cams] for f in range(self.T)]
        self.pose_upd = self.d_fref = self.d_rstat = None
        if cfg.with_pose_update:
            self.pose_upd = TrackHistory(NA, N, cfg.hist, device=self.device, storeLen=max(cfg.hist_store, cfg.hist))
            if cfg.export_frames > 0:
                self.pose_upd.set_archive(cfg.export_frames)
            self.d_merge_cache = z(self.pose_upd.mergability_cache_bytes(n_map), torch.uint8)
            if cfg.feature_chains:
                self.d_fref = torch.full((n_map, NA, 4), -1, dtype=torch.int32, device=self.dev)
                self.d_rstat = z((n_map, NA), torch.uint8)
            self.d_fref_counts = z(5, torch.int32)
            if self.d_fref is not None:
                self.pose_upd.set_classify_refs(self.d_fref.data_ptr(), self.d_rstat.data_ptr())
                self.pose_upd.set_merge_refs(self.d_fref.data_ptr(), self.d_rstat.data_ptr())
            self.pu_args = poseupdate_cams([dict(K=self.d_K1.data_ptr(), iK=self.d_iK1.data_ptr(), xy=self.d_xy[g].data_ptr(),
                                                 state=self.d_state[g].data_ptr(), slot2map=self.d_slot2map[g].data_ptr(),
                                                 trackSpan=self.d_trackspan[g].data_ptr(), reprojErr=self.d_reproj[g].data_ptr(),
                                                 isStatic=self.d_isstatic[g].data_ptr()) for g in range(NA)])
        self.reg_args = [register_cams([dict(K=self.d_K1.data_ptr(), R=self.d_R[b].data_ptr() + 72 * g, t=self.d_t[b].data_ptr() + 24 * g,
                                             xy=self.d_xy[g].data_ptr(), state=self.d_state[g].data_ptr(),
                                             slot2map=self.d_slot2map[g].data_ptr(), isStatic=self.d_isstatic[g].data_ptr())
                                        for g in range(NA)]) for b in range(2)]

    def setup_registration(self):
        torch, cfg, z = self.torch, self.cfg, self._z
        NA, n_map, i32, f64 = cfg.n_cams, self.n_map, torch.int32, torch.float64
        o_ = self.reg_out
        cur_pass = dict(P=cfg.p_reg, sigmaSearch=self.sig_pix, maxDist=3 * PIXEL_ERR_VAR, sigmaMerge=self.sig_pix, M=self.d_map.data_ptr(),
                        cov=self.d_cov.data_ptr(), pointFeat=self.d_pf.data_ptr(), slot=o_["slot"].data_ptr(), m=o_["m"].data_ptr(),
                        var=o_["var"].data_ptr(), dist=o_["dist"].data_ptr(), flags=o_["flags"].data_ptr(), mapFlags=self.d_mapflags.data_ptr(),
                        maxDistDynamic=4 * PIXEL_ERR_VAR, list=self.d_curlist.data_ptr())
        passes = [cur_pass]
        if cfg.with_active_search:
            self.act_out = dict(slot=z((1536, NA), i32), m=z((1536, NA, 2), f64), var=z((1536, NA, 4), f64), dist=z((1536, NA), f64),
                                flags=z((1536, NA), i32), pf=torch.full((1536, NA), -1, dtype=i32, device=self.dev))
            a_ = self.act_out
            passes.append(dict(P=1536, sigmaSearch=self.sig(2.5 * PIXEL_ERR_VAR), maxDist=3 * PIXEL_ERR_VAR, sigmaMerge=self.sig_pix,
                               M=self.d_map.data_ptr() + 24 * 1536, cov=self.d_cov.data_ptr() + 72 * 1536, pointFeat=a_["pf"].data_ptr(),
                               slot=a_["slot"].data_ptr(), m=a_["m"].data_ptr(), var=a_["var"].data_ptr(), dist=a_["dist"].data_ptr(),
                               flags=a_["flags"].data_ptr()))
        self.reg_passes = register_passes(passes)
        self._pass_current = (type(self.reg_passes[0]) * 1)(self.reg_passes[0])
        self.RV_CAP = 1024
        self.d_rvlist = torch.full((self.RV_CAP,), -1, dtype=i32, device=self.dev)
        self.d_rv_visit, self.d_rv_next = z(n_map, i32), z(n_map, i32)
        self.d_rv_reg = [z(n_map, torch.uint8), z(n_map, torch.uint8)]
        self.d_rv_counts, self.d_rv_listcounts = z(4, i32), z(4, i32)
        self.rv_pass = register_passes([dict(cur_pass, P=self.RV_CAP, list=self.d_rvlist.data_ptr())])
        nr = max(cfg.revisit_rounds, 1)
        self.d_rvlists = torch.full((nr, self.RV_CAP), -1, dtype=i32, device=self.dev)
        self.d_rvcounts = z(nr + 1, i32)
        self.rv_passes = [register_passes([dict(cur_pass, P=self.RV_CAP, list=self.d_rvlists[r].data_ptr())]) for r in range(nr)]
        self.sequential_registration = bool(cfg.sequential_registration)
        self._cand = None
        if self.world > 1 and self._decides():
            n = 3 * self.nc * cfg.p_reg
            self._cand = (z(n, i32), z(n * self.world, i32))

    def setup_keyframe_solves(self):
        torch, cfg, NA, N, device = self.torch, self.cfg, self.cfg.n_cams, self.cfg.n_feat, self.device
        self.ba_ws = BAWorkspace(device)
        self.ic_ws = BAWorkspace(device)
        self.ic_wss, self.n_ic_workers = [self.ic_ws], 1
        self.win = self.out = None
        if cfg.with_joint and self.pose_upd is not None:
            self.win = BAWindow(NA, cfg.n_key_frames, N, self.n_map, device=device)
            self.win.reserve(self.ba_ws)
            self.out = BAOutput(NA, cfg.n_key_frames, self.n_map, n_slots=8 if not cfg.keyframe_drives else min(self.lag * cfg.key_every + 6, 64),
                                device=device)
            self.out.attach(self.ba_ws)
            if self.d_fref is not None:
                self.out.set_feat_refs(self.d_fref.data_ptr(), self.d_rstat.data_ptr())
            self.recv_rec = self._z((2, self.out.record_bytes), torch.uint8)
        self.icam = None
        if self.ic is None:
            self.icam = BAInterCam(NA, N, cfg.pts_stride, self.n_map, max_dyn=60, device=device)
            self.ic_cams = intercam_cams([dict(K=self.d_K1.data_ptr(), xy=self.d_xy[g].data_ptr(), state=self.d_state[g].data_ptr(),
                                               slot2map=self.d_slot2map[g].data_ptr(), trackSpan=self.d_trackspan[g].data_ptr(),
                                               isStatic=self.d_isstatic[g].data_ptr()) for g in range(NA)])
        else:
            ic = self.ic
            iptr, icam, ixy = csr_of_problem(ic)
            self.ic_ws.upload(ic["Ks"], ic["Rs0"], ic["ts0"], ic["pts0"], iptr, icam, ixy)
            self.d_iR = torch.from_numpy(ic["Rs0"].reshape(-1).copy()).to(self.dev)
            self.d_iT = torch.from_numpy(ic["ts0"].reshape(-1).copy()).to(self.dev)
            self.d_iM = torch.from_numpy(ic["pts0"].reshape(-1).copy()).to(self.dev)
        self.n_pushed = self.n_windows = self.n_key = self.n_my_solves = self.n_my_ic = 0
        self.skip_busy, self.n_skipped = False, 0
        self.apply_at = {}
        self.applied, self.last_apply, self.pushed_frames = 0, None, []
        self.n_empty_solves = 0
        self.kf = None

    def _sec(self, name):
        if self._timing is None:
            return contextlib.nullcontext()

        @contextlib.contextmanager
        def cm():
            t0 = time.perf_counter()
            try:
                yield
            finally:
                self._timing[name] = self._timing.get(name, 0.0) + time.perf_counter() - t0
        return cm()

    def _mark(self, i, name):
        if self._marks is not None:
            e = self.torch.cuda.Event(enable_timing=True)
            e.record(self.pose_s)
            self._marks.append((i, name, e))

    def gpu_sections(self, first_frame=0):
        cfg, out, by = self.cfg, {}, {}
        for i, name, e in self._marks or []:
            by.setdefault(i, []).append((name, e))
        for i, ms in by.items():
            if i < first_frame:
                continue
            kind = ("ncc+" if self.ncc is not None and i % cfg.ncc_every == 0 else "") + ("key" if i % 5 == 0 else "plain")
            for (n0, e0), (n1, e1) in zip(ms[:-1], ms[1:]):
                acc = out.setdefault(kind, {}).setdefault(n0 + " -> " + n1, [0.0, 0])
                acc[0] += e0.elapsed_time(e1) * 1e3
                acc[1] += 1
            acc = out.setdefault(kind, {}).setdefault("WHOLE FRAME on the pose stream", [0.0, 0])
            acc[0] += ms[0][1].elapsed_time(ms[-1][1]) * 1e3
            acc[1] += 1
        return {k: {n: round(a / c, 1) for n, (a, c) in v.items()} | {"frames": max(c for _, c in v.values())} for k, v in out.items()}

    def vid(self, i):
        return i % self.T

    def _init_ncc(self):
        torch, cfg, z = self.torch, self.cfg, self._z
        self.ncc = None
        NA, N = cfg.n_cams, cfg.n_feat
        if not cfg.with_ncc or NA < 2 or self.pose_upd is None:
            return
        ws_, hs_ = ncc_scaled_dims(cfg.W, cfg.H, 0.3)
        rec = N * 128 + N * 32 + N * 4
        self.ncc = dict(small=z((self.nc, ws_ * hs_), torch.uint8), rec=z((NA, rec), torch.uint8), rec_bytes=rec, runs=0,
                        send=z((self.nc, rec), torch.uint8) if self.world > 1 else None,
                        dF=z((NA - 1, 9), torch.float64),
                        pairs=z((NA - 1, cfg.ncc_pair_cap * NCC_PAIR_DTYPE.itemsize), torch.uint8), pair_count=z(NA - 1, torch.int32),
                        group={}, np_scr=z(newpts_scratch_bytes(NA, N), torch.uint8), np_cnt=z(4 + NA, torch.int32), new_total=0)
        r = self.ncc["rec"]
        self.ncc["blk"] = [r[g, :N * 128] for g in range(NA)]
        self.ncc["abc"] = [r[g, N * 128: N * 160] for g in range(NA)]
        self.ncc["valid"] = [r[g, N * 160:] for g in range(NA)]
        cams = [dict(K=self.d_K1.data_ptr(), iK=self.d_iK1.data_ptr(), xy=self.d_xy[g].data_ptr(), state=self.d_state[g].data_ptr(),
                     slot2map=self.d_slot2map[g].data_ptr(), isStatic=self.d_isstatic[g].data_ptr(), reprojErr=self.d_reproj[g].data_ptr())
                for g in range(NA)]
        self.ncc["job"] = NewPtsJob(cams, [self.ncc["pairs"][a].data_ptr() for a in range(NA - 1)],
                                    [self.ncc["pair_count"][a:a + 1].data_ptr() for a in range(NA - 1)])

    def _ncc_leg(self, i, f, dst):
        cfg, nc, c0, N, NA, ncc = self.cfg, self.nc, self.c0, self.cfg.n_feat, self.cfg.n_cams, self.ncc
        s_ = self.pose_s.cuda_stream
        ncc_candidate_mask_dev(s_, nc, N, self.d_state[c0].data_ptr(), self.d_slot2map[c0].data_ptr(), self.d_trackspan[c0].data_ptr(),
                               self.d_mapflags.data_ptr(), self.n_map, ncc["valid"][c0].data_ptr(), device=self.device,
                               validStride=ncc["rec"].stride(0) // 4)
        if f not in ncc["group"]:
            own = ncc_cams([dict(img=self.img_ptrs[f][k], x=self.d_xy[c0 + k].data_ptr(), y=self.d_xy[c0 + k].data_ptr() + 8 * N,
                                 scaled=ncc["small"][k].data_ptr(), blocks=ncc["blk"][c0 + k].data_ptr(), abc=ncc["abc"][c0 + k].data_ptr(),
                                 valid=ncc["valid"][c0 + k].data_ptr()) for k in range(nc)])
            allc = ncc_cams([dict(img=0, x=self.d_xy[g].data_ptr(), y=self.d_xy[g].data_ptr() + 8 * N, scaled=0, blocks=ncc["blk"][g].data_ptr(),
                                  abc=ncc["abc"][g].data_ptr(), valid=ncc["valid"][g].data_ptr()) for g in range(NA)])
            jobs_ = ncc_pair_jobs([dict(dF=ncc["dF"][a].data_ptr(), camA=a, camB=a + 1, pairs=ncc["pairs"][a].data_ptr(),
                                        count=ncc["pair_count"][a:a + 1].data_ptr()) for a in range(NA - 1)])
            ncc["group"][f] = (own, allc, jobs_)
        own, allc, jobs_ = ncc["group"][f]
        ncc_get_blocks_group_dev(s_, own, cfg.W, cfg.H, N, 0.3, device=self.device)
        if self.world > 1:
            self._gather_ncc_records()
        ncc_fmats_dev(s_, NA, list(range(NA - 1)), list(range(1, NA)), [self.d_iK1.data_ptr()] * NA, self.d_R[dst].data_ptr(),
                      self.d_t[dst].data_ptr(), ncc["dF"].data_ptr(), device=self.device)
        ncc_epi_pairs_group_dev(s_, allc, N, jobs_, 50.0, 0.80, cfg.ncc_pair_cap, device=self.device)
        newpts_from_pairs_dev(s_, ncc["job"], N, cfg.ncc_pair_cap, self.d_R[dst].data_ptr(), self.d_t[dst].data_ptr(), self.d_map.data_ptr(),
                              self.d_cov.data_ptr(), self.d_mapflags.data_ptr(), self.d_newpt.data_ptr(), self.d_firstfrm.data_ptr(),
                              self.d_pf.data_ptr(), self.n_map, self.d_mapcount.data_ptr(), i, ncc["np_scr"].data_ptr(), ncc["np_cnt"].data_ptr(),
                              maxDisp=80.0, maxRpErr=3.0, pixelErrVar=self.sig_pix, minLen=2, device=self.device, W=cfg.W, H=cfg.H)
        ncc["runs"] += 1

    def _allgather(self, send, recv, nbytes):
        if self.native is not None:
            check(coslam_amd.lib().cs_comm_allgather_dev(self.native.exchange_comm, self.pose_s.cuda_stream, send.data_ptr(), recv.data_ptr(),
                                                         nbytes), "cs_comm_allgather_dev")
        else:
            import torch.distributed as dist

            with self.torch.cuda.stream(self.pose_s):
                dist.all_gather_into_tensor(recv, send)

    def _gather_ncc_records(self):
        ncc, nc, c0 = self.ncc, self.nc, self.c0
        with self.torch.cuda.stream(self.pose_s):
            ncc["send"].copy_(ncc["rec"][c0:c0 + nc], non_blocking=True)
        self._allgather(ncc["send"].view(-1), ncc["rec"].view(-1), ncc["send"].numel())

    def first_frame(self):
        torch, cfg = self.torch, self.cfg
        NA = cfg.n_cams
        self.grp.detect_dev(self.img_ptrs[0], self.dest_ptrs[0], self.cnt_ptrs)
        self.grp.advanceFrame()
        self.grp.synchronize()
        if self.world > 1:
            with torch.cuda.stream(self.pose_s):
                self.xchg.pack_group(self.d_dests[0], self.d_R[0][self.c0:self.c0 + self.nc], self.d_t[0][self.c0:self.c0 + self.nc], self.pose_s)
                self.xchg.all_gather(self.pose_s)
            torch.cuda.synchronize()
        dests = []
        for g in range(NA):
            if g in self.my_cams:
                w = self.d_dests[0][g - self.c0].cpu().numpy()
            else:
                w = self.xchg.unpack(g, device=self.device)[0].cpu().numpy().reshape(-1)
            dests.append(np.ascontiguousarray(w, dtype=np.int32).view(coslam_amd.KLT_TrackedFeature))
        s2m = np.stack([self.associate(self.sc, g, 0, dests[g]) for g in range(NA)])
        self.d_slot2map.copy_(torch.from_numpy(s2m))
        with torch.cuda.stream(self.pose_s):
            self._handback(0, 0)
        torch.cuda.synchronize()
        self.d_slot2map.copy_(torch.from_numpy(s2m))
        torch.cuda.synchronize()
        if self.pose_upd is not None:
            self.pose_upd.detect_dynamic_dev(self.pose_s.cuda_stream, self.pu_args, self.d_R[0].data_ptr(), self.d_t[0].data_ptr(), self.n_map,
                                             self.d_mapflags.data_ptr(), 0, 20, 5, 3, MAX_EPI_ERR)
            torch.cuda.synchronize()
        if cfg.keyframe_decision or cfg.intracam_mapping or cfg.keyframe_drives:
            self.enable_keyframe_decision(0, 0)
        if cfg.merge_check and not cfg.camera_grouping:
            raise ValueError("LoopConfig.merge_check needs LoopConfig.camera_grouping: the check reads the key frame's record of the groups")
        if cfg.camera_grouping:
            self._enable_camera_grouping()
        if cfg.merge_check:
            self._enable_merge_check()
        if cfg.live_view:
            self.live = LiveView(cfg.n_cams, cfg.live_view_cur_cap or self.n_map, cfg.live_view_dyn_cap or max(1, self.n_map // 4),
                                 depth=cfg.live_view_depth, trail_depth=cfg.live_view_trail_depth, every=cfg.live_view_every, device=self.device)
            self.live_frames, self.live_published = 0, 0

    GROUP_RING = 128

    def _enable_camera_grouping(self):
        torch, cfg, NA, z = self.torch, self.cfg, self.cfg.n_cams, self._z
        cen = [-np.asarray(self.sc.pose(c, 0)[0], np.float64).reshape(3, 3).T @ np.asarray(self.sc.pose(c, 0)[1], np.float64) for c in range(NA)]
        dist = [float(np.linalg.norm(cen[a] - cen[c])) for a in range(NA) for c in range(a + 1, NA)]
        RING = self.GROUP_RING
        words = C.sizeof(CameraGroups) // 4
        self.grouping = dict(init_translation=float(np.mean(dist)) if dist else 0.0,
                             cams=[grouping_cams([dict(xy=self.d_xy[g].data_ptr(), R=self.d_R[q][g].data_ptr(), t=self.d_t[q][g].data_ptr())
                                                  for g in range(NA)]) for q in range(2)],
                             groups=z((RING, words), torch.int32), vcosts=z((RING, NA * NA), torch.float64), nshare=z((RING, NA * NA), torch.int32),
                             scratch=z(camera_grouping_scratch_bytes(NA, cfg.n_feat), torch.uint8),
                             ev=[torch.cuda.Event(), torch.cuda.Event()], calls=0, taken=0, frames=[], per_frame=[], more_than_one=0, first_such=None,
                             changes=0, last=None)
        torch.cuda.synchronize()

    def _camera_grouping(self, i, dst):
        cfg, g, RING = self.cfg, self.grouping, self.GROUP_RING
        half = RING // 2
        if g["calls"] - g["taken"] >= RING:
            self._grouping_take(half)
        slot = g["calls"] % RING
        camera_grouping_dev(self.pose_s.cuda_stream, g["cams"][dst], cfg.n_feat, self.n_map, self.d_mapcount.data_ptr(), self.d_pf.data_ptr(),
                            self.d_mapflags.data_ptr(), cfg.W, cfg.H, g["vcosts"][slot].data_ptr(), g["nshare"][slot].data_ptr(),
                            g["scratch"].data_ptr(), g["init_translation"], g["groups"][slot].data_ptr(), maxDistRatio=cfg.group_max_dist_ratio,
                            minOverlapNum=cfg.group_min_overlap_num, minOverlapAreaRatio=cfg.group_min_overlap_area_ratio, device=self.device)
        g["frames"].append(i)
        g["calls"] += 1
        if g["calls"] % half == 0:
            g["ev"][(slot // half) & 1].record(self.pose_s)

    def _grouping_take(self, n, synced=False):
        g, RING, NA = self.grouping, self.GROUP_RING, self.cfg.n_cams
        if n <= 0:
            return
        s0 = g["taken"] % RING
        if not synced:
            g["ev"][(s0 // (RING // 2)) & 1].synchronize()
        idx = [(s0 + k) % RING for k in range(n)]
        gr, vc, ns = g["groups"][idx].cpu().numpy(), g["vcosts"][idx].cpu().numpy(), g["nshare"][idx].cpu().numpy()
        for k in range(n):
            G = CameraGroups.from_bytes(gr[k].tobytes())
            groups = G.groups()
            if len(groups) > 1:
                g["more_than_one"] += 1
                if g["first_such"] is None:
                    g["first_such"] = g["frames"][k]
            if g["last"] is not None and g["last"]["groups"] != groups:
                g["changes"] += 1
            g["per_frame"].append(len(groups))
            g["last"] = dict(frame=g["frames"][k], groups=groups, vcosts=vc[k].reshape(NA, NA).copy(), nshare=ns[k].reshape(NA, NA).copy())
        del g["frames"][:n]
        g["taken"] += n

    MERGE_RING = 32

    def _enable_merge_check(self):
        torch, cfg, NA, z = self.torch, self.cfg, self.cfg.n_cams, self._z
        cams = [merge_cams([dict(xy=self.d_xy[g].data_ptr(), state=self.d_state[g].data_ptr(), slot2map=self.d_slot2map[g].data_ptr(),
                                 K=self.d_K1.data_ptr(), R=self.d_R[q][g].data_ptr(), t=self.d_t[q][g].data_ptr()) for g in range(NA)])
                for q in range(2)]
        self.merge = dict(cams=cams, snap_cams={}, ring=z((self.MERGE_RING, C.sizeof(MergeCandidates)), torch.uint8),
                          scratch=z(merge_check_scratch_bytes(NA, cfg.n_feat), torch.uint8), ev=[torch.cuda.Event(), torch.cuda.Event()], calls=0,
                          taken=0, frames=[], split=0, with_candidate=0, first_such=None, last=None)
        torch.cuda.synchronize()

    def _merge_check(self, f, dst, snap=None):
        cfg, m, g, RING = self.cfg, self.merge, self.grouping, self.MERGE_RING
        half = RING // 2
        if m["calls"] - m["taken"] >= RING:
            self._merge_take(half)
        slot = m["calls"] % RING
        behind = self._frame_now - f
        if behind < 0 or behind >= min(g["calls"], self.GROUP_RING):
            raise RuntimeError(f"FrameLoop: the group record of key frame {f} is no longer in the ring")
        if snap is None:
            cams = m["cams"][dst]
        else:
            if id(snap) not in m["snap_cams"]:
                NA = cfg.n_cams
                m["snap_cams"][id(snap)] = merge_cams([dict(xy=snap["xy"][c].data_ptr(), state=snap["st"][c].data_ptr(), slot2map=snap["s2m"][c].data_ptr(),
                                                            K=self.d_K1.data_ptr(), R=snap["R"][c].data_ptr(), t=snap["t"][c].data_ptr())
                                                       for c in range(NA)])
            cams = m["snap_cams"][id(snap)]
        merge_check_dev(self.pose_s.cuda_stream, cams, cfg.n_feat, self.n_map, self.d_mapcount.data_ptr(), self.d_map.data_ptr(),
                        self.d_mapflags.data_ptr(), cfg.W, cfg.H, g["groups"][(g["calls"] - 1 - behind) % self.GROUP_RING].data_ptr(), f,
                        m["ring"][slot].data_ptr(), m["scratch"].data_ptr(), minInNum=cfg.merge_min_in_num,
                        minInAreaRatio=cfg.merge_min_in_area_ratio, maxCamDist=cfg.merge_max_cam_dist, allPairs=False, device=self.device)
        m["frames"].append(f)
        m["calls"] += 1
        if m["calls"] % half == 0:
            m["ev"][(slot // half) & 1].record(self.pose_s)

    def _merge_take(self, n, synced=False):
        m, RING = self.merge, self.MERGE_RING
        if n <= 0:
            return
        s0 = m["taken"] % RING
        if not synced:
            m["ev"][(s0 // (RING // 2)) & 1].synchronize()
        recs = m["ring"][[(s0 + k) % RING for k in range(n)]].cpu().numpy()
        for k in range(n):
            r = MergeCandidates.from_bytes(recs[k].tobytes())
            m["split"] += r.groupNum > 1
            if r.nMergeInfo > 0:
                m["with_candidate"] += 1
                if m["first_such"] is None:
                    m["first_such"] = m["frames"][k]
            m["last"] = r
        del m["frames"][:n]
        m["taken"] += n

    def merge_stats(self):
        if self.merge is None:
            return None
        m = self.merge
        self.torch.cuda.synchronize()
        self._merge_take(m["calls"] - m["taken"], synced=True)
        last = m["last"]
        out = dict(key_frames_checked=m["taken"], key_frames_with_more_than_one_group=int(m["split"]),
                   key_frames_with_a_candidate=m["with_candidate"], first_such_frame=m["first_such"],
                   last_frame=None if last is None else int(last.frame), last_group_num=None if last is None else int(last.groupNum),
                   last_info=None if last is None else [list(x) for x in last.infos()],
                   min_in_num=self.cfg.merge_min_in_num, min_in_area_ratio=self.cfg.merge_min_in_area_ratio, max_cam_dist=self.cfg.merge_max_cam_dist)
        if last is not None:
            out.update({"last_" + k: v for k, v in last.tables(self.cfg.n_cams).items()})
        return out

    def _live_view(self, i, dst):
        g = self.grouping
        d_groups = g["groups"][(g["calls"] - 1) % self.GROUP_RING].data_ptr() if g is not None and g["calls"] else None
        self.live.frame_dev(self.pose_s.cuda_stream, i, self.n_map, self.d_mapcount.data_ptr(), self.d_pf.data_ptr(), self.d_mapflags.data_ptr(),
                            self.d_map.data_ptr(), self.d_R[dst].data_ptr(), self.d_t[dst].data_ptr(), d_groups)
        self.live_frames += 1
        self.live_published += i % self.cfg.live_view_every == 0

    def live_snapshot(self, frame=None):
        if self.live is None:
            return None
        return self.live.snapshot(frame)

    def live_trails(self, trj_len=150):
        if self.live is None:
            return None
        return self.live.trails(self.pose_s.cuda_stream, min(int(trj_len), self.cfg.live_view_trail_depth))

    def live_stats(self):
        if self.live is None:
            return None
        self.torch.cuda.synchronize()
        s, tr = self.live.snapshot(), self.live_trails()
        out = dict(frames=self.live_frames, frames_published=self.live_published, trails=len(tr), longest_trail=max([len(p) for _, p in tr], default=0))
        if s is not None:
            out.update({k: s[k] for k in ("frame", "nCur", "nDyn", "curOverflow", "dynOverflow", "curOverflowTotal", "dynOverflowTotal", "nStatic", "nDynamic", "nStaticFeat", "nDynamicFeat")})
        return out

    def grouping_stats(self):
        if self.grouping is None:
            return None
        g = self.grouping
        self.torch.cuda.synchronize()
        self._grouping_take(g["calls"] - g["taken"], synced=True)
        last = g["last"]
        return dict(groups_per_frame=list(g["per_frame"]), last_groups=None if last is None else last["groups"],
                    frames_with_more_than_one_group=g["more_than_one"], first_such_frame=g["first_such"], group_changes=g["changes"],
                    last_vcosts=None if last is None else last["vcosts"].tolist(), last_nshare=None if last is None else last["nshare"].tolist(),
                    last_frame=None if last is None else last["frame"], init_cam_translation=g["init_translation"])

    def enable_keyframe_decision(self, frame, b):
        torch, cfg, NA, z = self.torch, self.cfg, self.cfg.n_cams, self._z
        torch.cuda.synchronize()
        i32, f64 = torch.int32, torch.float64
        st, fl, s2m = self.d_state.cpu().numpy(), self.d_mapflags.cpu().numpy(), self.d_slot2map.cpu().numpy()
        km = [int((((st[g] == 0) | (st[g] == 1)) & (s2m[g] >= 0) & ((fl[np.clip(s2m[g], 0, len(fl) - 1)] & 7) == 0)).sum()) for g in range(NA)]
        self.kf = dict(frame=torch.full((NA,), int(frame), dtype=i32, device=self.dev), mapped=torch.tensor(km, dtype=i32, device=self.dev),
                       selfR=self.d_R[b].clone(), selfT=self.d_t[b].clone(), ready=z(NA + 2, i32), cnt=z(2 * NA, i32), cen=z((NA, 3), f64),
                       stats=z(5, i32), frames=0, placed=[], not_applied=0)
        Rn, tn = self.d_R[b].cpu().numpy().reshape(NA, 3, 3), self.d_t[b].cpu().numpy()
        cen = np.stack([-Rn[g].T @ tn[g] for g in range(NA)])
        dist = [np.linalg.norm(cen[a] - cen[c]) for a in range(NA) for c in range(a + 1, NA)]
        self.kf["min_translation"] = float(np.mean(dist) / 4.5) if dist else 0.1
        self.kf["cams"] = [keyframe_cams([dict(state=self.d_state[g].data_ptr(), slot2map=self.d_slot2map[g].data_ptr(),
                                               R=self.d_R[q][g].data_ptr(), t=self.d_t[q][g].data_ptr(), keyFrame=self.kf["frame"][g:].data_ptr(),
                                               keyMapped=self.kf["mapped"][g:].data_ptr(), selfR=self.kf["selfR"][g].data_ptr(),
                                               selfT=self.kf["selfT"][g].data_ptr()) for g in range(NA)]) for q in range(2)]
        if cfg.intracam_mapping and self.pose_upd is not None:
            self.kf.update(im_scr=z(self.pose_upd.newpts_intracam_scratch_bytes(), torch.uint8), im_cnt=z(3, i32), im_total=z(3, torch.int64))
        if cfg.keyframe_drives and cfg.keyframe_lag > 0:
            self.kf["lag_ring"], self.kf["lag_blocked"] = self._kf_lag_ring(), 0
        torch.cuda.synchronize()

    def _kf_lag_ring(self):
        torch, cfg, NA, N, z = self.torch, self.cfg, self.cfg.n_cams, self.cfg.n_feat, self._z
        ring = []
        for _ in range(cfg.keyframe_lag + 1):
            xy, st, s2m = z((NA, 2 * N), torch.float64), z((NA, N), torch.int32), z((NA, N), torch.int32)
            R, t = z((NA, 9), torch.float64), z((NA, 3), torch.float64)
            hb = handback_cams([dict(dest=self.d_dests[0][0].data_ptr(), K=self.d_K1.data_ptr(), kud=self.d_kud.data_ptr(), mapPts=self.d_map.data_ptr(),
                                     slot2map=s2m[g].data_ptr(), trackSpan=self.d_trackspan[g].data_ptr(), xy=xy[g].data_ptr(), state=st[g].data_ptr(),
                                     Ms=self.d_Ms[g].data_ptr(), ms=self.d_ms[g].data_ptr(), sel=self.d_sel[g].data_ptr(),
                                     npts=self.d_npts[g:g + 1].data_ptr(), opt=self.d_opt[g].data_ptr(), pointFeat=0, pointFeatStride=NA, nPointFeat=0,
                                     isStatic=0) for g in range(NA)])
            ring.append(dict(xy=xy, st=st, s2m=s2m, R=R, t=t, hb=hb, word=torch.zeros(1, dtype=torch.int32).pin_memory(),
                             ev=torch.cuda.Event(), frame=-1))
        return ring

    def _kf_lag_record(self, i, dst):
        k, NA = self.kf, self.cfg.n_cams
        sl = k["lag_ring"][i % (self.cfg.keyframe_lag + 1)]
        keyframe_snapshot_dev(self.pose_s.cuda_stream, NA, self.cfg.n_feat, self.d_xy.data_ptr(), self.d_state.data_ptr(), self.d_slot2map.data_ptr(),
                              self.d_R[dst].data_ptr(), self.d_t[dst].data_ptr(), k["ready"][NA + 1:].data_ptr(), sl["xy"].data_ptr(), sl["st"].data_ptr(),
                              sl["s2m"].data_ptr(), sl["R"].data_ptr(), sl["t"].data_ptr(), sl["word"].data_ptr(), device=self.device)
        sl["ev"].record(self.pose_s)
        sl["frame"] = i

    def _kf_lag_act(self, i, dst):
        k, D = self.kf, self.cfg.keyframe_lag
        f = i - D
        sl = k["lag_ring"][f % (D + 1)]
        if f < 1 or sl["frame"] != f:
            return
        if not sl["ev"].query():
            k["lag_blocked"] += 1
            sl["ev"].synchronize()
        if int(sl["word"][0]) == 0:
            return
        k["placed"].append(f)
        self._key_frame(f, dst, snap=sl)

    def keyframe_stats(self):
        if not self.kf:
            return None
        a = self.kf["stats"].cpu().tolist()
        im = None if "im_total" not in self.kf else dict(zip(("candidates_tried", "points_added", "points_dropped_map_full"), self.kf["im_total"].cpu().tolist()))
        return dict(frames=self.kf["frames"], intracam_new_map_points=im, frames_with_a_camera_ready=a[0], frames_with_decrease_ie_key_frames_added=a[1],
                    cameras_saying_decrease=a[2], cameras_saying_view_angle=a[3], cameras_saying_translation=a[4],
                    min_cam_translation=self.kf["min_translation"], key_frames_placed_by_the_decision=list(self.kf["placed"]),
                    windows_not_applied_history_too_short=self.kf["not_applied"], last_key_frame_per_camera=self.kf["frame"].cpu().tolist(),
# ... 452 lines not shown
```

### coslam_amd/ncc.py

```python
import ctypes as C

import numpy as np

from ._lib import check, lib


def ncc_blocks_dev(stream_ptr, d_img, W, H, n, d_x, d_y, scale, d_blocks, d_abc, d_valid, device=0):
    check(lib().cs_ncc_blocks_dev(int(device), stream_ptr, d_img, int(W), int(H), int(n), d_x, d_y, scale, d_blocks, d_abc,
                                  d_valid), "cs_ncc_blocks_dev")


def ncc_epi_mat_dev(stream_ptr, F, M, d_x1, d_y1, d_blocks1, d_abc1, d_valid1, N, d_x2, d_y2, d_blocks2, d_abc2, d_valid2, epiMax,
                    nccMin, wNone, d_epiMat, d_nccMat, device=0):
    F = np.ascontiguousarray(F, dtype=np.float64).reshape(9)
    check(lib().cs_ncc_epi_mat_dev(int(device), stream_ptr, F.ctypes.data, int(M), d_x1, d_y1, d_blocks1, d_abc1, d_valid1, int(N), d_x2, d_y2,
                                   d_blocks2, d_abc2, d_valid2, epiMax, nccMin, wNone, d_epiMat, d_nccMat),
          "cs_ncc_epi_mat_dev")


NCC_PAIR_DTYPE = np.dtype([("i", "<i4"), ("j", "<i4"), ("epi", "<f8"), ("ncc", "<f8")])
C_RECORD_TYPES = {"NCC_PAIR_DTYPE": "cs_ncc_pair"}


def ncc_epi_pairs_dev(stream_ptr, F, M, d_x1, d_y1, d_blocks1, d_abc1, d_valid1, N, d_x2, d_y2, d_blocks2, d_abc2, d_valid2, epiMax,
                      nccMin, d_pairs, pairCap, d_pairCount, device=0):
    F = np.ascontiguousarray(F, dtype=np.float64).reshape(9)
    check(lib().cs_ncc_epi_pairs_dev(int(device), stream_ptr, F.ctypes.data, int(M), d_x1, d_y1, d_blocks1, d_abc1, d_valid1, int(N), d_x2, d_y2,
                                     d_blocks2, d_abc2, d_valid2, epiMax, nccMin, d_pairs, int(pairCap), d_pairCount),
          "cs_ncc_epi_pairs_dev")


class NccCam(C.Structure):
    _c_type_ = "cs_ncc_cam"
    _fields_ = [(n, C.c_void_p) for n in ("img", "x", "y", "scaled", "blocks", "abc", "valid")]


class NccPairJob(C.Structure):
    _c_type_ = "cs_ncc_pair_job"
    _fields_ = [("F", C.c_double * 9), ("camA", C.c_int), ("camB", C.c_int), ("pairs", C.c_void_p), ("count", C.c_void_p), ("dF", C.c_void_p)]


def ncc_cams(cams):
    arr = (NccCam * len(cams))()
    for a, c in zip(arr, cams):
        for n, _ in NccCam._fields_:
            v = c.get(n)
            setattr(a, n, int(v) if v else None)
    return arr


def ncc_pair_jobs(jobs):
    arr = (NccPairJob * len(jobs))()
    for a, q in zip(arr, jobs):
        if q.get("F") is not None:
            F = np.ascontiguousarray(q["F"], dtype=np.float64).reshape(9)
            for k in range(9):
                a.F[k] = float(F[k])
        a.camA, a.camB, a.pairs, a.count = int(q["camA"]), int(q["camB"]), int(q["pairs"]), int(q["count"])
        if q.get("dF"):
            a.dF = int(q["dF"])
    return arr


def ncc_fmats_dev(stream_ptr, nCams, camA, camB, d_iK, d_R, d_t, d_F, device=0):
    n = len(camA)
    ca, cb = (C.c_int * n)(*[int(v) for v in camA]), (C.c_int * n)(*[int(v) for v in camB])
    ik = (C.c_void_p * nCams)(*[int(v) for v in d_iK])
    check(lib().cs_ncc_fmats_dev(int(device), stream_ptr, int(nCams), n, ca, cb, ik, d_R, d_t, d_F),
          "cs_ncc_fmats_dev")


def ncc_get_blocks_group_dev(stream_ptr, cams, W, H, n, scale, device=0):
    arr = cams if isinstance(cams, C.Array) else ncc_cams(cams)
    check(lib().cs_ncc_get_blocks_group_dev(int(device), stream_ptr, len(arr), arr, int(W), int(H), int(n), scale),
          "cs_ncc_get_blocks_group_dev")


def ncc_epi_pairs_group_dev(stream_ptr, cams, n, jobs, epiMax, nccMin, pairCap, device=0):
    arr = cams if isinstance(cams, C.Array) else ncc_cams(cams)
    jb = jobs if isinstance(jobs, C.Array) else ncc_pair_jobs(jobs)
    check(lib().cs_ncc_epi_pairs_group_dev(int(device), stream_ptr, len(arr), arr, int(n), len(jb), jb, epiMax, nccMin,
                                           int(pairCap)), "cs_ncc_epi_pairs_group_dev")


def ncc_match_between(img1, x1, y1, img2, x2, y2, scale, F, epiMax, nccMin, wNone=-1.0, device=0):
    img1 = np.ascontiguousarray(img1, dtype=np.uint8)
    img2 = np.ascontiguousarray(img2, dtype=np.uint8)
    a = [np.ascontiguousarray(v, dtype=np.float64) for v in (x1, y1, x2, y2)]
    M, N = len(a[0]), len(a[2])
    F = np.ascontiguousarray(F, dtype=np.float64).reshape(9)
    epi, ncc = np.zeros((M, N)), np.zeros((M, N))
    b1, b2 = np.zeros((M, 128), np.uint8), np.zeros((N, 128), np.uint8)
    c1, c2 = np.zeros((M, 4)), np.zeros((N, 4))
    v1, v2 = np.zeros(M, np.int32), np.zeros(N, np.int32)
    p = lambda v: v.ctypes.data
    check(lib().cs_ncc_match_between(int(device), p(img1), img1.shape[1], img1.shape[0], M, p(a[0]), p(a[1]), p(img2), img2.shape[1], img2.shape[0],
                                     N, p(a[2]), p(a[3]), scale, p(F), epiMax, nccMin, wNone, p(epi), p(ncc), p(b1), p(c1), p(v1), p(b2), p(c2),
                                     p(v2)), "cs_ncc_match_between")
    return dict(epi=epi, ncc=ncc, blocks1=b1, abc1=c1, valid1=v1, blocks2=b2, abc2=c2, valid2=v2)


def ncc_get_blocks_dev(stream_ptr, d_img, W, H, n, d_x, d_y, scale, d_scaled, d_blocks, d_abc, d_valid=0, device=0):
    check(lib().cs_ncc_get_blocks_dev(int(device), stream_ptr, d_img, int(W), int(H), int(n), d_x, d_y, scale, d_scaled, d_blocks, d_abc,
                                      d_valid), "cs_ncc_get_blocks_dev")


def ncc_scaled_dims(W, H, scale):
    ws, hs = C.c_int(0), C.c_int(0)
    check(lib().cs_ncc_scaled_dims(int(W), int(H), scale, C.byref(ws), C.byref(hs)), "cs_ncc_scaled_dims")
    return ws.value, hs.value


def ncc_match_between_full(img1, x1, y1, img2, x2, y2, scale, F, epiMax, nccMin, wNone=-1.0, device=0):
    img1 = np.ascontiguousarray(img1, dtype=np.uint8)
    img2 = np.ascontiguousarray(img2, dtype=np.uint8)
    a = [np.ascontiguousarray(v, dtype=np.float64) for v in (x1, y1, x2, y2)]
    M, N = len(a[0]), len(a[2])
    F = np.ascontiguousarray(F, dtype=np.float64).reshape(9)
    epi, ncc = np.zeros((M, N)), np.zeros((M, N))
    b1, b2 = np.zeros((M, 128), np.uint8), np.zeros((N, 128), np.uint8)
    c1, c2 = np.zeros((M, 4)), np.zeros((N, 4))
    p = lambda v: v.ctypes.data
    check(lib().cs_ncc_match_between_full(int(device), p(img1), img1.shape[1], img1.shape[0], M, p(a[0]), p(a[1]), p(img2), img2.shape[1],
                                          img2.shape[0], N, p(a[2]), p(a[3]), scale, p(F), epiMax, nccMin, wNone, p(epi), p(ncc), p(b1), p(c1), p(b2),
                                          p(c2)), "cs_ncc_match_between_full")
    return dict(epi=epi, ncc=ncc, blocks1=b1, abc1=c1, blocks2=b2, abc2=c2)
```

### include/coslam_hip.h

```cpp
#ifndef COSLAM_HIP_H
#define COSLAM_HIP_H

#include <stddef.h>
#include <stdint.h>

#ifdef __cplusplus
extern "C" {
#endif

#define CS_OK 0
#define CS_ERR_INVALID (-1)
#define CS_ERR_NO_DEVICE (-2)
#define CS_ERR_HIP (-3)
#define CS_ERR_ALLOC (-4)
#define CS_ERR_NUMERIC (-5)

int cs_version(void);
const char* cs_last_error(void);
int cs_debug_set(const char* key, int value);
int cs_device_count(void);


typedef struct cs_klt_feature {
    int status;
// ... 473 lines not shown
    const int* pointMap;
    const int* obsPtr;
    const int* obsCam;
    const double* obsXY;
    const cs_merge_info* info;
    const unsigned char* infoValid;
    const double *infoR, *infoT;
    int maxPoints, maxObs, maxViews, maxInfo;
    const double *solvedRs, *solvedTs;
    const double* solvedPts;
    const int* outlier;
} cs_merge_constraints_buffers;
typedef struct cs_merge_constraints cs_merge_constraints;
cs_merge_constraints* cs_merge_constraints_create(int device, int nCams, int N, int maxMatches, int maxMap);
void cs_merge_constraints_destroy(cs_merge_constraints* mc);
int cs_merge_constraints_assemble_dev(cs_merge_constraints* mc, const cs_track_history* h, void* hip_stream, const cs_merge_cam* cams,
                                      const cs_feat_ref* d_featRef, int nMap, const double* d_mapPts, const cs_camera_groups* d_groups, int gId1,
                                      int gId2, int maxiCam, int maxjCam, int f1, int f2, const int* d_matches, int nMatches);
int cs_merge_constraints_assemble(cs_merge_constraints* mc, const cs_track_history* h, void* hip_stream, const cs_merge_cam* cams,
                                  const cs_feat_ref* d_featRef, int nMap, const double* d_mapPts, const cs_camera_groups* d_groups, int gId1,
                                  int gId2, int maxiCam, int maxjCam, int f1, int f2, const int* h_matches, int nMatches);
int cs_merge_info_dev(cs_merge_constraints* mc, void* hip_stream, const cs_camera_groups* d_groups, int gId1, int gId2, const double* d_Rs,
                      const double* d_Ts);
int cs_merge_constraints_solve(cs_merge_constraints* mc, void* hip_stream);
struct cs_ba_stats;
int cs_merge_constraints_solution(const cs_merge_constraints* mc, int which, double* Rs, double* Ts, double* pts, int* outlier,
                                  struct cs_ba_stats* stats);
int cs_merge_constraints_info_dev(cs_merge_constraints* mc, void* hip_stream, const cs_camera_groups* d_groups, int gId1, int gId2);
int cs_merge_constraints_buffers_get(const cs_merge_constraints* mc, cs_merge_constraints_buffers* out);
int cs_merge_constraints_header_get(cs_merge_constraints* mc, void* hip_stream, cs_merge_constraints_header* h_out);
int cs_merge_constraints_download(cs_merge_constraints* mc, void* hip_stream, const void* d_src, void* h_dst, size_t bytes);
int cs_merge_constraints_apply_map_dev(cs_merge_constraints* mc, void* hip_stream, int* const* d_slot2map, int* d_pointFeat,
                                       cs_feat_ref* d_featRef, unsigned char* d_refStatic, int nMap, double* d_mapPts, int applyPoints,
                                       int* d_counts);

#define CS_MERGE_MATCH_MAX_JOBS 256
struct cs_ncc_pair;
struct cs_ncc_cam;
enum { CS_MERGE_MATCH_PAIRS_OVERFLOW = 1, CS_MERGE_MATCH_MATCHES_OVERFLOW = 2 };
typedef struct {
    const double* xy;
    const int* state;
    const double* K;
    const unsigned char* imgSmall;
    double imgScale;
} cs_merge_match_cam;
typedef struct {
    int iCam, jCam;
    double E[9];
    int nSeeds;
    const double* seeds;
} cs_merge_match_job;
typedef struct {
    const int* matches;
    const double* scores;
    const int* counts;
    const struct cs_ncc_pair* pairs;
    const int* pairCount;
    const unsigned char* blocks;
    const double* abc;
    const int* valid;
    int nCams, N, maxJobs, maxSeeds, pairCap, maxMatches;
} cs_merge_match_buffers;
typedef struct { int count, flags, candidates, rounds; } cs_merge_match_count;
typedef struct cs_merge_match cs_merge_match;
cs_merge_match* cs_merge_match_create(int device, int nCams, int N, int maxJobs, int maxSeeds, int pairCap, int maxMatches);
void cs_merge_match_destroy(cs_merge_match* mm);
int cs_merge_match_fmat(const double K1[9], const double K2[9], const double E[9], double F[9]);
int cs_merge_match_run_dev(cs_merge_match* mm, void* hip_stream, const cs_merge_match_cam* cams , int Ws, int Hs,
                           int nJobs, const cs_merge_match_job* jobs , double epiMax, double nccMin, double maxDisp);
int cs_merge_match_from_pairs_dev(cs_merge_match* mm, void* hip_stream, int nJobs, const struct cs_ncc_pair* const* d_pairs ,
                                  const int* const* d_pairCount , const double* const* d_xy1 ,
                                  const double* const* d_xy2 , const int* nSeeds ,
                                  const double* const* seeds , double maxDisp);
int cs_merge_match_counts(cs_merge_match* mm, void* hip_stream, int nJobs, cs_merge_match_count* h_out);
int cs_merge_match_buffers_get(const cs_merge_match* mm, cs_merge_match_buffers* out);
int cs_merge_match_download(cs_merge_match* mm, void* hip_stream, const void* d_src, void* h_dst, size_t bytes);
int cs_ncc_get_scaled_blocks_group_dev(int device, void* hip_stream, int nCams, const struct cs_ncc_cam* cams , int Ws, int Hs, int n,
                                       double scale);
int cs_ncc_small_dims(int W, int H, double scale, int* Ws, int* Hs);
int cs_ncc_small_image_dev(int device, void* hip_stream, const unsigned char* d_img, int W, int H, double scale, unsigned char* d_small);
typedef struct {
    int status;
    int entry;
    int maxk, maxiCam, maxjCam, maxgId1, maxgId2;
    int gid1, gid2, camid1, camid2;
} cs_merge_match_choice;
int cs_merge_match_select(int nInfo, const cs_merge_info* info, const int* surfNum, const unsigned char* ematOk, const int* nccNum,
                          const unsigned char* eligible, const int* groupSize, cs_merge_match_choice* out);

#define CS_MERGE_FRONT_MAX_JOBS 256
enum { CS_MERGE_FRONT_TOO_FEW = 1, CS_MERGE_FRONT_NO_MODEL = 2 };
typedef struct {
    const double* pts;
    const float* desc;
    const double* K;
    int n;
} cs_merge_front_cam;
typedef struct { int iCam, jCam; } cs_merge_front_job;
typedef struct {
    int surfNum, ematOk, inlierNum, rounds , bestHyp , flags;
    double E[9];
    double epiErr;
} cs_merge_front_result;
typedef struct {
    const int* matches;
    const float* dist;
    const int* count;
    const unsigned char* inlierFlag;
    const double* seeds;
    const int* newMatches;
    const cs_merge_front_result* results;
    const int* hypSample;
    const int* hypCount;
    const double* hypE;
    const double* pix;
    const int* valid;
    int nCams, maxPts, dimDesc, maxJobs, maxHyp;
} cs_merge_front_buffers;
typedef struct cs_merge_front cs_merge_front;
cs_merge_front* cs_merge_front_create(int device, int nCams, int maxPts, int dimDesc, int maxJobs, int maxHyp);
void cs_merge_front_destroy(cs_merge_front* mf);
int cs_merge_front_run_dev(cs_merge_front* mf, void* hip_stream, const cs_merge_front_cam* cams , int nJobs,
                           const cs_merge_front_job* jobs , double ratio, double maxDist, int nRansac, double maxEpiErr,
                           int minInlierNum, unsigned long long seed);
int cs_merge_front_match_dev(cs_merge_front* mf, void* hip_stream, const cs_merge_front_cam* cams , int nJobs,
                             const cs_merge_front_job* jobs , double ratio, double maxDist);
int cs_merge_front_from_matches_dev(cs_merge_front* mf, void* hip_stream, const cs_merge_front_cam* cams , int nJobs,
                                    const cs_merge_front_job* jobs , const int* const* matches ,
                                    const int* nMatches , int nRansac, double maxEpiErr, int minInlierNum, unsigned long long seed);
int cs_merge_front_results(cs_merge_front* mf, void* hip_stream, int nJobs, cs_merge_front_result* h_out);
int cs_merge_front_buffers_get(const cs_merge_front* mf, cs_merge_front_buffers* out);
int cs_merge_front_download(cs_merge_front* mf, void* hip_stream, const void* d_src, void* h_dst, size_t bytes);

#define CS_SURF_MAX_OCTAVES 5
#define CS_SURF_MAX_LAYERS 6
#define CS_SURF_ORI_SAMPLES 109
#define CS_SURF_ORI_WINDOWS 72
typedef struct {
    const double* pts;
    const float* desc;
    const double* size;
    const double* angle;
    const double* response;
    const unsigned char* laplacian;
    const int* octave;
    const int* layer;
    const int* cell;
    const int* count;
    const int* overflow;
    const unsigned int* integral;
    const double* det;
    const unsigned char* lap;
    int nCams, W, H, maxPts, nOctaves, nOctaveLayers, dimDesc, mapElems;
    int mapW[CS_SURF_MAX_OCTAVES], mapH[CS_SURF_MAX_OCTAVES];
    int mapOff[CS_SURF_MAX_OCTAVES * CS_SURF_MAX_LAYERS];
    int layerSize[CS_SURF_MAX_OCTAVES * CS_SURF_MAX_LAYERS];
    int layerFits[CS_SURF_MAX_OCTAVES * CS_SURF_MAX_LAYERS];
} cs_surf_buffers;
typedef struct cs_surf cs_surf;
cs_surf* cs_surf_create(int device, int nCams, int W, int H, int maxPts, int nOctaves, int nOctaveLayers, int dimDesc);
void cs_surf_destroy(cs_surf* sf);
int cs_surf_run_dev(cs_surf* sf, void* hip_stream, const unsigned char* const* d_img , int pitch, double hessianThreshold,
                    int upright);
int cs_surf_integral_dev(cs_surf* sf, void* hip_stream, const unsigned char* const* d_img , int pitch);
int cs_surf_layers_dev(cs_surf* sf, void* hip_stream, const unsigned char* const* d_img , int pitch);
int cs_surf_detect_dev(cs_surf* sf, void* hip_stream, const unsigned char* const* d_img , int pitch, double hessianThreshold);
int cs_surf_counts(cs_surf* sf, void* hip_stream, int* count, int* overflow);
int cs_surf_buffers_get(const cs_surf* sf, cs_surf_buffers* out);
int cs_surf_download(cs_surf* sf, void* hip_stream, const void* d_src, void* h_dst, size_t bytes);

int cs_track_history_set_classify_refs(cs_track_history* h, cs_feat_ref* d_featRef, unsigned char* d_refStatic);

int cs_track_history_set_merge_refs(cs_track_history* h, cs_feat_ref* d_featRef, unsigned char* d_refStatic);

int cs_check_unify_dev(const cs_track_history* h, void* hip_stream, const cs_poseupdate_cam* cams, int nPairs, const int* d_pf1,
                       const int* d_pf2, const double* d_M1, const double* d_M2, double pixelErrVar, unsigned char* d_ok, double* d_M,
                       double* d_cov);
int cs_check_unify_ref_dev(const cs_track_history* h, void* hip_stream, const cs_poseupdate_cam* cams, int nPairs, const cs_feat_ref* d_ref1,
                           const cs_feat_ref* d_ref2, const double* d_M1, const double* d_M2, double pixelErrVar, unsigned char* d_ok, double* d_M,
                           double* d_cov);
int cs_register_decide_merge_dev(const cs_track_history* h, void* hip_stream, const cs_poseupdate_cam* cams, int P, int mapBase, const int* d_slot,
                                 const int* d_flags, const unsigned char* d_mergeable, unsigned char* d_mapFlags, int* d_pointFeat, double* d_mapPts,
                                 double* d_mapCov, double pixelErrVar, unsigned char* d_attached, unsigned char* d_regged, void* d_scratch,
                                 int* d_counts, int onlyCam);
size_t cs_register_decide_merge_scratch_bytes(int P, int nList, int nCams);
int cs_register_decide_merge_list_dev(const cs_track_history* h, void* hip_stream, const cs_poseupdate_cam* cams, int P, int mapBase,
                                      const int* d_list, int nList, const int* d_slot, const int* d_flags, const unsigned char* d_mergeable,
                                      unsigned char* d_mapFlags, int* d_pointFeat, double* d_mapPts, double* d_mapCov, double pixelErrVar,
                                      unsigned char* d_attached, unsigned char* d_regged, void* d_scratch, int* d_counts, int onlyCam);


int cs_map_points_classify_dev(const cs_track_history* h, void* hip_stream, const cs_poseupdate_cam* cams, int* d_pointFeat, int nMap,
                               const int* d_featFrame, const int* d_featFirst, int curFrame, double* d_mapPts, double* d_mapCov,
                               unsigned char* d_mapFlags, unsigned char* d_newPt, int* d_staticFrameNum, const int* d_firstFrame,
                               double pixelVar, int* d_counts);
int cs_pose_update_classify_frame_dev(cs_track_history* h, void* hip_stream, const cs_poseupdate_cam* cams, int* d_pointFeat, int nMap,
                                      const double* d_R, const double* d_t, double* d_mapPts, double* d_mapCov, unsigned char* d_mapFlags,
                                      int largeErr, double pixelErrVar, int frame, int maxLen, int minLen, int minOutNum, double maxEpiErr,
                                      int* d_numNodes, int* d_numOut, int* d_numDyn, const int* d_featFrame, const int* d_featFirst,
                                      unsigned char* d_newPt, int* d_staticFrameNum, const int* d_firstFrame, double pixelVarClassify,
                                      int* d_clsCounts);

typedef struct cs_posegraph cs_posegraph;
int cs_posegraph_create(int device, int nGraphs, const int* nodePtr, const int* edgePtr, const unsigned char* fixed,
                        const int* id1, const int* id2, cs_posegraph** out);
void cs_posegraph_destroy(cs_posegraph* g);
int cs_posegraph_counts(const cs_posegraph* g, int* nNodes, int* nEdges, int* nComponents, int* maxHalfBandwidth);
int cs_posegraph_relax_dev(cs_posegraph* g, void* hip_stream, const double* d_nodeR, const double* d_nodeT,
                           const double* d_edgeR, const double* d_edgeT, double* d_newR, double* d_newT);
int cs_posegraph_status(cs_posegraph* g, void* hip_stream, int* nFailed, int* firstFailedGraph);
int cs_posegraph_relax(cs_posegraph* g, const double* nodeR, const double* nodeT, const double* edgeR, const double* edgeT,
                       double* newR, double* newT);
int cs_posegraph_edges_dev(cs_posegraph* g, void* hip_stream, const double* d_nodeR, const double* d_nodeT, double* d_edgeR,
                           double* d_edgeT);
int cs_posegraph_set_poses_dev(int device, void* hip_stream, int n, const int* d_nodeIdx, const double* d_R, const double* d_t,
                               double* d_nodeR, double* d_nodeT);
int cs_posegraph_create_scaled(int device, int nGraphs, const int* nodePtr, const int* edgePtr, const unsigned char* fixed,
                               const int* id1, const int* id2, const int* scaleId, cs_posegraph** out);
int cs_posegraph_relax_scaled_dev(cs_posegraph* g, void* hip_stream, const double* d_nodeR, const double* d_nodeT,
                                  const double* d_edgeR, const double* d_edgeT, double* d_newR, double* d_newT, double* d_edgeS);
int cs_posegraph_relax_scaled(cs_posegraph* g, const double* nodeR, const double* nodeT, const double* edgeR, const double* edgeT,
                              double* newR, double* newT, double* edgeS);
int cs_posegraph_scaled_counts(const cs_posegraph* g, int* nScales, int* nBorderNodes, int* maxInteriorHalfBandwidth);
typedef struct cs_posegraph_after_ba_rec {
    cs_posegraph* g;
    int device;
    int nCams;
    const int* d_camNode;
    const double* d_Rs;
    const double* d_Ts;
    double* d_nodeR;
    double* d_nodeT;
    const double* d_edgeR;
    const double* d_edgeT;
    double* d_newR;
    double* d_newT;
} cs_posegraph_after_ba_rec;
int cs_posegraph_after_ba(void* hip_stream, void* rec );

typedef struct cs_export_cam {
    const char* videoFilePath;
    const double* K;
    const double* kc;
    int W, H;
    int startFrameInVideo;
    int nPoses;
    const int* poseFrame;
    const double* poseR;
    const double* poseT;
    const int* featPtr;
    const long long* featPointId;
    const double* featXY;
} cs_export_cam;
int cs_export_results_v1(const char* dirPath, int nCams, const cs_export_cam* cams, int curFrame, int nPts, const long long* ptId,
                         const double* ptM, const double* ptCov, int covAsReference);
typedef struct cs_loop_export_cam {
    const char* videoFilePath;
    const double* K;
    const double* kc;
    int W, H;
    int startFrameInVideo;
} cs_loop_export_cam;
int cs_loop_export_results(const char* dirPath, const cs_track_history* h, void* hip_stream, const cs_feat_ref* d_featRef, int nMap,
                           const double* d_M, const double* d_cov, const unsigned char* d_mapFlags, const cs_loop_export_cam* cams,
                           int covAsReference, long long* stats);

int cs_ncc_blocks_dev(int device, void* hip_stream, const unsigned char* d_img, int W, int H, int n, const double* d_x,
                      const double* d_y, double scale, unsigned char* d_blocks, double* d_abc, int* d_valid);
int cs_ncc_epi_mat_dev(int device, void* hip_stream, const double F[9] , int M, const double* d_x1, const double* d_y1,
                       const unsigned char* d_blocks1, const double* d_abc1, const int* d_valid1, int N, const double* d_x2,
                       const double* d_y2, const unsigned char* d_blocks2, const double* d_abc2, const int* d_valid2,
                       double epiMax, double nccMin, double wNone, double* d_epiMat, double* d_nccMat);
typedef struct cs_ncc_pair {
    int i, j;
    double epi, ncc;
} cs_ncc_pair;
int cs_ncc_epi_pairs_dev(int device, void* hip_stream, const double F[9] , int M, const double* d_x1, const double* d_y1,
                         const unsigned char* d_blocks1, const double* d_abc1, const int* d_valid1, int N, const double* d_x2,
                         const double* d_y2, const unsigned char* d_blocks2, const double* d_abc2, const int* d_valid2,
                         double epiMax, double nccMin, cs_ncc_pair* d_pairs, int pairCap, int* d_pairCount);
typedef struct cs_ncc_cam {
    const unsigned char* img;
    const double* x;
    const double* y;
    unsigned char* scaled;
    unsigned char* blocks;
    double* abc;
    int* valid;
} cs_ncc_cam;
typedef struct cs_ncc_pair_job {
    double F[9];
    int camA, camB;
    cs_ncc_pair* pairs;
    int* count;
    const double* dF;
} cs_ncc_pair_job;
int cs_ncc_fmats_dev(int device, void* hip_stream, int nCams, int nPairs, const int* camA, const int* camB, const double* const* d_iK,
                     const double* d_R, const double* d_t, double* d_F);
int cs_ncc_get_blocks_group_dev(int device, void* hip_stream, int nCams, const cs_ncc_cam* cams , int W, int H, int n,
                                double scale);
int cs_ncc_epi_pairs_group_dev(int device, void* hip_stream, int nCams, const cs_ncc_cam* cams , int n, int nJobs,
                               const cs_ncc_pair_job* jobs , double epiMax, double nccMin, int pairCap);
int cs_ncc_unmapped_mask_dev(int device, void* hip_stream, int n, const int* d_state, const int* d_slot2map, int* d_valid);
int cs_ncc_scaled_dims(int W, int H, double scale, int* Ws, int* Hs);
int cs_ncc_get_blocks_dev(int device, void* hip_stream, const unsigned char* d_img, int W, int H, int n, const double* d_x,
                          const double* d_y, double scale, unsigned char* d_scaled, unsigned char* d_blocks, double* d_abc, int* d_valid);
int cs_ncc_match_between_full(int device, const unsigned char* img1, int W1, int H1, int M, const double* x1, const double* y1,
                              const unsigned char* img2, int W2, int H2, int N, const double* x2, const double* y2, double scale,
                              const double F[9], double epiMax, double nccMin, double wNone, double* epiMat, double* nccMat,
                              unsigned char* blocks1, double* abc1, unsigned char* blocks2, double* abc2);
int cs_ncc_match_between(int device, const unsigned char* img1, int W1, int H1, int M, const double* x1, const double* y1,
                         const unsigned char* img2, int W2, int H2, int N, const double* x2, const double* y2, double scale,
                         const double F[9], double epiMax, double nccMin, double wNone, double* epiMat, double* nccMat,
                         unsigned char* blocks1, double* abc1, int* valid1, unsigned char* blocks2, double* abc2, int* valid2);

int cs_ncc_candidate_mask_dev(int device, void* hip_stream, int nCams, int N, const int* d_state, const int* d_slot2map,
                              const int* d_trackSpan, const unsigned char* d_mapFlags, int mapCap, int minTrack , int* d_valid,
                              size_t validStride );
size_t cs_newpts_scratch_bytes(int nCams, int N);
int cs_newpts_from_pairs_dev(int device, void* hip_stream, int nCams, int N, const cs_poseupdate_cam* cams,
                             const cs_ncc_pair* const* d_pairs , const int* const* d_pairCount ,
                             int pairCap, const double* d_R, const double* d_t, double* d_mapPts, double* d_mapCov, unsigned char* d_mapFlags,
                             unsigned char* d_newPt, int* d_firstFrame, int* d_pointFeat, int mapCap, int* d_mapCount, int curFrame,
                             double maxDisp, double maxRpErr, double pixelErrVar, int minLen, int W, int H, void* d_scratch, int* d_counts);


#define CS_BA_FLAG_CHOL_FAILED 1
#define CS_BA_FLAG_NO_PROGRESS 2
#define CS_BA_FLAG_SOLVER_TIMEOUT 4
typedef struct cs_ba_stats {
    double cost0, cost;
    int nIterTotal, nOuter, nOutliers, flags;
} cs_ba_stats;

int cs_ba_robust(int C, int P, int nObs, const double* Ks, double* Rs, double* Ts, double* pts, const int* obs_ptr,
                 const int* obs_cam, const double* obs_xy, int nCamsCon, int nPtsCon, double maxErr, int maxIter,
                 int innerMaxIter, int* out_outlier, cs_ba_stats* stats, int device);

typedef struct cs_ba cs_ba;
cs_ba* cs_ba_create(int device);
void cs_ba_destroy(cs_ba* b);
void* cs_ba_stream(cs_ba* b);
int cs_ba_set_stream(cs_ba* b, void* hip_stream);
int cs_ba_robust_h(cs_ba* b, int C, int P, int nObs, const double* Ks, double* Rs, double* Ts, double* pts,
                   const int* obs_ptr, const int* obs_cam, const double* obs_xy, int nCamsCon, int nPtsCon,
                   double maxErr, int maxIter, int innerMaxIter, int* out_outlier, cs_ba_stats* stats);
int cs_ba_upload(cs_ba* b, int C, int P, int nObs, const double* Ks, const double* Rs, const double* Ts,
                 const double* pts, const int* obs_ptr, const int* obs_cam, const double* obs_xy);
int cs_ba_solve_dev(cs_ba* b, void* hip_stream, int C, int P, int nObs, const double* d_Rs0, const double* d_Ts0,
                    const double* d_pts0, int nCamsCon, int nPtsCon, double maxErr, int maxIter, int innerMaxIter);
int cs_ba_solve_async(cs_ba* b, void* after_stream, int C, int P, int nObs, const double* d_Rs0, const double* d_Ts0,
                      const double* d_pts0, int nCamsCon, int nPtsCon, double maxErr, int maxIter, int innerMaxIter);
int cs_ba_wait(cs_ba* b);
int cs_ba_pending(cs_ba* b);
long long cs_ba_completed(cs_ba* b);
typedef struct cs_ba_window cs_ba_window;
cs_ba_window* cs_ba_window_create(int device, int nCams, int nKeyFrames, int N, int nMapPts);
void cs_ba_window_destroy(cs_ba_window* w);
int cs_ba_window_push_dev(cs_ba_window* w, void* hip_stream, const cs_handback_cam* cams, const double* d_K, int kShared,
                          const double* d_R, const double* d_t, int frame);
int cs_ba_solve_window_async(cs_ba* b, cs_ba_window* w, void* after_stream, const double* d_mapPts, const unsigned char* d_mapStatic,
                             int nCamsCon, int nPtsCon, double maxErr, int maxIter, int innerMaxIter);
int cs_ba_solve_window_flags_async(cs_ba* b, cs_ba_window* w, void* after_stream, const double* d_mapPts, const unsigned char* d_mapFlags,
                                   int nCamsCon, int nPtsCon, double maxErr, int maxIter, int innerMaxIter);
typedef struct cs_ba_output cs_ba_output;
cs_ba_output* cs_ba_output_create(int device, int nCams, int nKeyFrames, int nMapPts, int nSlots);
void cs_ba_output_destroy(cs_ba_output* o);
int cs_ba_output_attach(cs_ba_output* o, cs_ba* b);
size_t cs_ba_output_record_bytes(const cs_ba_output* o);
long long cs_ba_output_packed(cs_ba_output* o);
int cs_ba_output_wait(cs_ba_output* o, long long seq, void** d_record);
int cs_ba_output_wait_dev(cs_ba_output* o, long long seq, void* hip_stream, int timeoutMs, void** d_record);
int cs_ba_output_wait_errors(cs_ba_output* o);
int cs_ba_output_slot(cs_ba_output* o, long long seq, void** d_record);
int cs_ba_output_header(cs_ba_output* o, const void* d_record, void* hip_stream, int hdr8[8], int keyFrames[16]);
int cs_ba_output_arrays(cs_ba_output* o, const void* d_record, const double** d_Rs, const double** d_Ts, const double** d_pts,
                        const int** d_pointMap, const unsigned char** d_ptOutlier);
int cs_ba_output_apply_dev(cs_ba_output* o, const void* d_record, void* hip_stream, cs_track_history* h, cs_ba_window* w,
                           const cs_poseupdate_cam* cams, const int* d_pointFeat, int nMap, double* d_mapPts, double* d_mapCov,
                           unsigned char* d_mapFlags, double pixelErrVar, int firstKeyFrame, int keyEvery, double* d_Rcur, double* d_tcur,
                           int* d_counts);
int cs_ba_output_apply_seq_dev(cs_ba_output* o, const void* d_record, long long seq, void* hip_stream, cs_track_history* h, cs_ba_window* w,
                               const cs_poseupdate_cam* cams, const int* d_pointFeat, int nMap, double* d_mapPts, double* d_mapCov,
                               unsigned char* d_mapFlags, double pixelErrVar, int firstKeyFrame, int keyEvery, double* d_Rcur,
                               double* d_tcur, int* d_counts);
int cs_ba_output_apply_frames_dev(cs_ba_output* o, const void* d_record, long long seq, void* hip_stream, cs_track_history* h, cs_ba_window* w,
                                  const cs_poseupdate_cam* cams, const int* d_pointFeat, int nMap, double* d_mapPts, double* d_mapCov,
                                  unsigned char* d_mapFlags, double pixelErrVar, const int* keyFrames, int nKeyFrames, double* d_Rcur,
                                  double* d_tcur, int* d_counts);
int cs_ba_output_set_feat_refs(cs_ba_output* o, const void* d_featRef, const unsigned char* d_refStatic);
#define CS_BA_APPLY_POSES 1
#define CS_BA_APPLY_POINTS 2
#define CS_BA_APPLY_FALSE 4
#define CS_BA_APPLY_UPDATE 8
#define CS_BA_APPLY_ALL 15
int cs_ba_output_set_apply_mask(cs_ba_output* o, int mask);
typedef struct cs_intercam_cam {
    const double* K;
    const double* xy;
    const int* state;
    const int* slot2map;
    const int* trackSpan;
    const unsigned char* isStatic;
} cs_intercam_cam;
typedef struct cs_ba_intercam cs_ba_intercam;
cs_ba_intercam* cs_ba_intercam_create(int device, int nCams, int N, int ptsStride, int nMapPts, int maxDyn );
void cs_ba_intercam_destroy(cs_ba_intercam* ic);
int cs_ba_solve_intercam_async(cs_ba* b, cs_ba_intercam* ic, void* after_stream, const cs_intercam_cam* cams , int W, int H,
                               int nColBlk, int nRowBlk, const double* d_R, const double* d_t, const double* d_mapPts,
                               const unsigned char* d_mapFlags, const unsigned char* d_newPt, const int* d_pointFeat, double maxErr,
                               int maxIter, int innerMaxIter);
int cs_ba_intercam_last_problem(cs_ba_intercam* ic, int* C, int* P, int* nObs, int* nStatic, const int** d_pointMap);
int cs_ba_intercam_apply_dev(cs_ba* b, cs_ba_intercam* ic, void* hip_stream, cs_track_history* h, const cs_poseupdate_cam* cams, int N,
                             const int* d_pointFeat, int nMap, double* d_Rcur, double* d_tcur, double* d_mapPts, double* d_mapCov,
                             unsigned char* d_mapFlags, double pixelErrVar, int* d_numNodes, int* d_numOut);
int cs_ba_reserve_for_window(cs_ba* b, cs_ba_window* w);
int cs_ba_worker_stats(cs_ba* b, int* jobs, double* gpu_ms_total, double* gpu_ms_last, double* gpu_ms_max,
                       double* gpu_ms_parse );
int cs_ba_window_last_problem(cs_ba_window* w, int* C, int* P, int* nObs, const int** d_pointMap, int* keyFrames);
int cs_ba_problem_buffers(cs_ba* b, const double** d_Ks, const int** d_obs_ptr, const int** d_obs_cam, const double** d_obs_xy);
typedef int (*cs_ba_followup_fn)(void* hip_stream, void* user);
int cs_ba_set_followup(cs_ba* b, cs_ba_followup_fn fn, void* user);
int cs_ba_result_buffers(cs_ba* b, double** d_Rs, double** d_Ts, double** d_pts);
enum {
    CS_BA_PH_COST0 = 0,
    CS_BA_PH_CONTROL0 = 1,
    CS_BA_PH_LIN_SCHUR = 2,
    CS_BA_PH_SOLVE_UPDATE = 3,
    CS_BA_PH_CONTROL1 = 4,
    CS_BA_PH_FLAG = 5,
    CS_BA_PH_OUTER_END = 6,
    CS_BA_PH_FINAL_PREP = 7,
    CS_BA_PH_FINISH = 8
};
int cs_ba_dist_begin(cs_ba* b, void* hip_stream, int C, int P, int nObs, const double* d_Rs0, const double* d_Ts0,
                     const double* d_pts0, int nCamsCon, int nPtsCon, double maxErr, int innerMaxIter, int pLo, int pHi,
                     int addLambda);
int cs_ba_dist_phase(cs_ba* b, void* hip_stream, int phase);
int cs_ba_dist_buffers(cs_ba* b, void** d_S_rhs, int* n_red, void** d_scal, void** d_pts, void** d_outlier);
int cs_ba_download(cs_ba* b, int C, int P, int nObs, double* Rs, double* Ts, double* pts, int* out_outlier,
                   cs_ba_stats* stats);

typedef struct cs_comm cs_comm;
int cs_comm_available(void);
int cs_comm_unique_id(unsigned char id[128]);
cs_comm* cs_comm_create(const unsigned char id[128], int world, int rank, int device);
cs_comm* cs_comm_create_host(const char* name, int world, int rank, int device);
void cs_comm_destroy(cs_comm* c);
int cs_comm_world(const cs_comm* c);
int cs_comm_rank(const cs_comm* c);

typedef struct cs_exchange cs_exchange;
cs_exchange* cs_exchange_create(cs_comm* c, int nCamsLocal, int nFeatures);
void cs_exchange_destroy(cs_exchange* x);
int cs_exchange_allgather_dev(cs_exchange* x, void* hip_stream, const void* const* d_dests, const double* d_R,
                              const double* d_t);
int cs_exchange_buffers(cs_exchange* x, void** d_recv, size_t* record_bytes);

int cs_exchange_unpack_poses_dev(cs_exchange* x, void* hip_stream, double* d_R, double* d_t, int skipOwn);
int cs_comm_broadcast_dev(cs_comm* c, void* hip_stream, void* d_buf, size_t bytes, int root);

int cs_comm_allgather_dev(cs_comm* c, void* hip_stream, const void* d_send, void* d_recv, size_t bytes);

int cs_ba_dist_solve(cs_ba* b, cs_comm* c, void* hip_stream, int C, int P, int nObs, const double* d_Rs0, const double* d_Ts0,
                     const double* d_pts0, int nCamsCon, int nPtsCon, double maxErr, int maxIter, int innerMaxIter);

#ifdef __cplusplus
}
#endif
#endif
```

Measured before the change: 2075.

## Compact NCC candidates into lists and fuse front-end kernels for epipolar matching

Adds a front kernel that compacts candidate features per camera into an index list via ballot/popcount, and in the same launch runs the image resize, the fundamental-matrix computation and the pair-count reset. Block extraction and the epipolar/NCC pair kernel then work only over the compacted lists, so the M×N pair tile shrinks to candidates only. Epipolar line coefficients are also precomputed once per column when the tile is stored instead of per row group. This cuts launch count and wasted work on non-candidates, at the cost of more shared memory per tile and extra compaction buffers; grid sizing now has to cover the worst case, since counts live on the device.

```diff
diff --git a/coslam_amd/csrc/ncc.hip b/coslam_amd/csrc/ncc.hip
--- a/coslam_amd/csrc/ncc.hip
+++ b/coslam_amd/csrc/ncc.hip
@@ -1,4 +1,5 @@
 #include "cs_common.h"
+#include "ncc_candidate_dev.h"
 #include "small_ops.h"
 
 #pragma clang fp contract(off)
@@ -65,10 +66,9 @@
     int* valid[NC_MAX_CAMS];
 };
 
-__global__ __launch_bounds__(256) void k_resize_linear_u8(NcCamSet S, int W, int H, double scale_x, double scale_y, int Wd, int Hd) {
-    const unsigned char* __restrict__ src = S.img[blockIdx.z];
-    unsigned char* __restrict__ dst = S.scaled[blockIdx.z];
-    const int dx = blockIdx.x * 64 + (threadIdx.x & 63), dy = blockIdx.y * 4 + (threadIdx.x >> 6);
+__device__ __forceinline__ void nc_resize_block(const unsigned char* __restrict__ src, unsigned char* __restrict__ dst, int bx, int by, int W,
+                                                int H, double scale_x, double scale_y, int Wd, int Hd) {
+    const int dx = bx * 64 + (threadIdx.x & 63), dy = by * 4 + (threadIdx.x >> 6);
     if (dx >= Wd || dy >= Hd) return;
     float fx = (float)((dx + 0.5) * scale_x - 0.5);
     int sx = nc_floorf(fx);
@@ -96,20 +96,15 @@
     }
     dst[(size_t)dy * Wd + dx] = (unsigned char)((((b0 * (r0 >> 4)) >> 16) + ((b1 * (r1 >> 4)) >> 16) + 2) >> 2);
 }
-
-__global__ __launch_bounds__(256) void k_ncc_blocks_subpix(NcCamSet S, int W, int H, int n, double scale, int scaled) {
-    const int cam = blockIdx.y;
-    const unsigned char* __restrict__ img = scaled ? S.scaled[cam] : S.img[cam];
-    const double* __restrict__ xs = S.x[cam];
-    const double* __restrict__ ys = S.y[cam];
-    unsigned char* __restrict__ blocks = S.blocks[cam];
-    double* __restrict__ abc = S.abc[cam];
-    int* __restrict__ valid = S.valid[cam];
+__global__ __launch_bounds__(256) void k_resize_linear_u8(NcCamSet S, int W, int H, double scale_x, double scale_y, int Wd, int Hd) {
+    nc_resize_block(S.img[blockIdx.z], S.scaled[blockIdx.z], blockIdx.x, blockIdx.y, W, H, scale_x, scale_y, Wd, Hd);
+}
+
+__device__ __forceinline__ void nc_cut_block(const unsigned char* __restrict__ img, int W, int H, double x, double y, double scale, int scaled,
+                                             int p, unsigned char* __restrict__ blocks, double* __restrict__ abc, int* __restrict__ valid) {
     const int lane = threadIdx.x & 63;
-    const int p = blockIdx.x * 4 + (threadIdx.x >> 6);
-    if (p >= n) return;
     const int win = NC_BW;
-    const double px = scaled ? xs[p] * scale : xs[p], py = scaled ? ys[p] * scale : ys[p];
+    const double px = scaled ? x * scale : x, py = scaled ? y * scale : y;
     float fxc = (float)px, fyc = (float)py;
     fxc -= (win - 1) * 0.5f;
     fyc -= (win - 1) * 0.5f;
@@ -189,6 +184,12 @@
         if (valid) valid[p] = 1;
     }
 }
+__global__ __launch_bounds__(256) void k_ncc_blocks_subpix(NcCamSet S, int W, int H, int n, double scale, int scaled) {
+    const int cam = blockIdx.y;
+    const int p = blockIdx.x * 4 + (threadIdx.x >> 6);
+    if (p >= n) return;
+    nc_cut_block(scaled ? S.scaled[cam] : S.img[cam], W, H, S.x[cam][p], S.y[cam][p], scale, scaled, p, S.blocks[cam], S.abc[cam], S.valid[cam]);
+}
 
 __global__ __launch_bounds__(256) void k_ncc_unmapped_mask(int n, const int* __restrict__ state, const int* __restrict__ slot2map,
                                                            int* __restrict__ valid) {
@@ -203,6 +204,8 @@
     const double* abc;
     const int* valid;
     int n;
+    const int* cnt;
+    const int* idx;
 };
 struct NcArgs {
     double F[9];
@@ -227,15 +230,18 @@
 constexpr int NC_MAX_JOBS = 8;
 struct NcJobs {
     NcArgs job[NC_MAX_JOBS];
+    int ct;
 };
 constexpr int NC_CT = 4;
+constexpr int NC_LIST_CT = 4;
 constexpr int NC_TP = 136;
-constexpr int NC_TILE_BYTES = 64 * NC_TP + 64 * 40;
+constexpr int NC_TILE_BYTES = 64 * NC_TP + 64 * 60;
 struct NcColRegs {
     nc_i32x4 q0, q1;
     double x, y, A, C;
     int valid;
 };
+template <bool LIST>
 __device__ __forceinline__ void nc_tile_fetch(const NcSide& S2, int j0, int N, int tid, NcColRegs& r) {
     const int row = j0 + (tid >> 2);
     r.q0 = r.q1 = (nc_i32x4){0, 0, 0, 0};
@@ -249,10 +255,10 @@
     r.x = r.y = r.A = r.C = 0.0, r.valid = 0;
     if (tid < 64 && j0 + tid < N) {
         const int j = j0 + tid;
-        r.x = S2.x[j], r.y = S2.y[j], r.A = S2.abc[4 * (size_t)j], r.C = S2.abc[4 * (size_t)j + 2], r.valid = S2.valid[j];
-    }
-}
-__device__ __forceinline__ void nc_tile_store(unsigned char* buf, int tid, const NcColRegs& r) {
+        r.x = S2.x[j], r.y = S2.y[j], r.A = S2.abc[4 * (size_t)j], r.C = S2.abc[4 * (size_t)j + 2], r.valid = LIST ? S2.idx[j] : S2.valid[j];
+    }
+}
+__device__ __forceinline__ void nc_tile_store(unsigned char* buf, int tid, const NcColRegs& r, const double (&Fm)[9], double epiMax) {
     nc_i32x4* dst = (nc_i32x4*)(buf + (tid >> 2) * NC_TP + 32 * (tid & 3));
     long* d8 = (long*)dst;
     const long* s8 = (const long*)&r.q0;
@@ -261,17 +267,24 @@
     d8[2] = s8[0], d8[3] = s8[1];
     if (tid < 64) {
         double* c = (double*)(buf + 64 * NC_TP);
-        c[tid] = r.x, c[64 + tid] = r.y, c[128 + tid] = r.A, c[192 + tid] = r.C;
-        ((int*)(c + 256))[tid] = r.valid;
-    }
-}
-template <bool SPARSE>
+        const double l0 = (Fm[0] * r.x + Fm[1] * r.y) + Fm[2];
+        const double l1 = (Fm[3] * r.x + Fm[4] * r.y) + Fm[5];
+        const double l2 = (Fm[6] * r.x + Fm[7] * r.y) + Fm[8];
+        const double nn = sqrt(l0 * l0 + l1 * l1);
+        const double den = nn > 0 ? nn : 1.0;
+        const double numMax = (epiMax * den) * (1.0 + 1e-12);
+        c[tid] = l0, c[64 + tid] = l1, c[128 + tid] = l2, c[192 + tid] = den, c[256 + tid] = numMax, c[320 + tid] = r.A, c[384 + tid] = r.C;
+        ((int*)(c + 448))[tid] = r.valid;
+    }
+}
+template <bool SPARSE, bool LIST>
 __global__ __launch_bounds__(256) void k_ncc_epi_mat(NcJobs J) {
     __shared__ __attribute__((aligned(16))) unsigned char sTile[2][NC_TILE_BYTES];
     const NcArgs& A = J.job[blockIdx.z];
     const int tid = threadIdx.x, lane = tid & 63, wv = tid >> 6;
-    const int M = A.s1.n, N = A.s2.n;
-    if ((int)blockIdx.y * 64 >= M || (int)blockIdx.x * NC_CT * 64 >= N) return;
+    const int M = LIST ? *A.s1.cnt : A.s1.n, N = LIST ? *A.s2.cnt : A.s2.n;
+    const int nCT = LIST ? J.ct : NC_CT;
+    if ((int)blockIdx.y * 64 >= M || (int)blockIdx.x * nCT * 64 >= N) return;
     const int i0 = blockIdx.y * 64 + 16 * wv;
     const bool rowsIn = i0 < M;
     double Fm[9];
@@ -291,22 +304,22 @@
         y1[r] = in ? A.s1.y[i] : 0.0;
         A1[r] = in ? A.s1.abc[4 * (size_t)i] : 0.0;
         C1[r] = in ? A.s1.abc[4 * (size_t)i + 2] : 0.0;
-        v1[r] = in ? A.s1.valid[i] : 0;
+        v1[r] = in ? (LIST ? A.s1.idx[i] : A.s1.valid[i]) : 0;
         s1[r] = (int)A1[r] - NC_LEN * 128;
     }
-    const int jBase = blockIdx.x * NC_CT * 64;
+    const int jBase = blockIdx.x * nCT * 64;
     NcColRegs cr;
-    nc_tile_fetch(A.s2, jBase, N, tid, cr);
-    nc_tile_store(sTile[0], tid, cr);
+    nc_tile_fetch<LIST>(A.s2, jBase, N, tid, cr);
+    nc_tile_store(sTile[0], tid, cr, Fm, A.epiMax);
     __syncthreads();
-    for (int ct = 0; ct < NC_CT; ++ct) {
+    for (int ct = 0; ct < nCT; ++ct) {
         const int j0 = jBase + ct * 64;
         if (j0 >= N) break;
-        const bool more = ct + 1 < NC_CT && j0 + 64 < N;
-        if (more) nc_tile_fetch(A.s2, j0 + 64, N, tid, cr);
+        const bool more = ct + 1 < nCT && j0 + 64 < N;
+        if (more) nc_tile_fetch<LIST>(A.s2, j0 + 64, N, tid, cr);
         const unsigned char* tile = sTile[ct & 1];
         const double* cc = (const double*)(tile + 64 * NC_TP);
-        const int* cv = (const int*)(cc + 256);
+        const int* cv = (const int*)(cc + 448);
         if (rowsIn) {
             nc_i32x4 acc[4];
 #pragma unroll
@@ -324,16 +337,11 @@
             for (int t = 0; t < 4; ++t) {
                 const int jl = 16 * t + lr, j = j0 + jl;
                 if (j >= N) continue;
-                const double bx = cc[jl], by = cc[64 + jl];
-                const double A2 = cc[128 + jl], C2 = cc[192 + jl];
+                const double l0 = cc[jl], l1 = cc[64 + jl], l2 = cc[128 + jl];
+                const double den = cc[192 + jl], numMax = cc[256 + jl];
+                const double A2 = cc[320 + jl], C2 = cc[384 + jl];
                 const int v2 = cv[jl];
                 const int s2 = (int)A2 - NC_LEN * 128;
-                const double l0 = (Fm[0] * bx + Fm[1] * by) + Fm[2];
-                const double l1 = (Fm[3] * bx + Fm[4] * by) + Fm[5];
-                const double l2 = (Fm[6] * bx + Fm[7] * by) + Fm[8];
-                const double nn = sqrt(l0 * l0 + l1 * l1);
-                const double den = nn > 0 ? nn : 1.0;
-                const double numMax = (A.epiMax * den) * (1.0 + 1e-12);
 #pragma unroll
                 for (int r = 0; r < 4; ++r) {
                     const int i = i0 + 4 * lk + r;
@@ -342,7 +350,7 @@
                     double e = A.wNone, c = A.wNone;
                     bool pass = false;
                     double epiErr = 0;
-                    bool near = v1[r] && v2 && !(num > numMax);
+                    bool near = (LIST || (v1[r] && v2)) && !(num > numMax);
                     if (near) {
                         epiErr = num / den;
                         near = epiErr <= A.epiMax;
@@ -361,7 +369,7 @@
                             const int at = atomicAdd(A.pairCount, 1);
                             if (at < A.pairCap) {
                                 cs_ncc_pair q;
-                                q.i = i, q.j = j, q.epi = e, q.ncc = c;
+                                q.i = LIST ? v1[r] : i, q.j = LIST ? v2 : j, q.epi = e, q.ncc = c;
                                 A.pairs[at] = q;
                             }
                         }
@@ -372,7 +380,7 @@
                 }
             }
         }
-        if (more) nc_tile_store(sTile[(ct + 1) & 1], tid, cr);
+        if (more) nc_tile_store(sTile[(ct + 1) & 1], tid, cr, Fm, A.epiMax);
         __syncthreads();
     }
 }
@@ -550,8 +558,8 @@
     CS_HIP(hipSetDevice(device));
     A.pairs = nullptr, A.pairCap = 0, A.pairCount = nullptr;
     NcJobs J;
-    J.job[0] = A;
-    hipLaunchKernelGGL(k_ncc_epi_mat<false>, dim3((unsigned)((N + 64 * NC_CT - 1) / (64 * NC_CT)), (unsigned)((M + 63) / 64)), dim3(256), 0,
+    J.job[0] = A, J.ct = NC_CT;
+    hipLaunchKernelGGL((k_ncc_epi_mat<false, false>), dim3((unsigned)((N + 64 * NC_CT - 1) / (64 * NC_CT)), (unsigned)((M + 63) / 64)), dim3(256), 0,
                        (hipStream_t)hip_stream, J);
     CS_CHECK_LAUNCH();
     return CS_OK;
@@ -583,8 +591,8 @@
     A.epiMat = A.nccMat = nullptr;
     A.pairs = d_pairs, A.pairCap = pairCap, A.pairCount = d_pairCount;
     NcJobs J;
-    J.job[0] = A;
-    hipLaunchKernelGGL(k_ncc_epi_mat<true>, dim3((unsigned)((N + 64 * NC_CT - 1) / (64 * NC_CT)), (unsigned)((M + 63) / 64)), dim3(256), 0,
+    J.job[0] = A, J.ct = NC_CT;
+    hipLaunchKernelGGL((k_ncc_epi_mat<true, false>), dim3((unsigned)((N + 64 * NC_CT - 1) / (64 * NC_CT)), (unsigned)((M + 63) / 64)), dim3(256), 0,
                        (hipStream_t)hip_stream, J);
     CS_CHECK_LAUNCH();
     return CS_OK;
@@ -597,9 +605,7 @@
     const double *R, *t;
     double* F;
 };
-__global__ void k_ncc_fmats(NcFmArgs A) {
-    const int k = threadIdx.x;
-    if (k >= A.n) return;
+__device__ __forceinline__ void nc_fmat_pair(const NcFmArgs& A, int k, double* __restrict__ F) {
     const double *Ra = A.R + 9 * A.camA[k], *Rb = A.R + 9 * A.camB[k], *ta = A.t + 3 * A.camA[k], *tb = A.t + 3 * A.camB[k];
     double R[9], t[3], E[9], T[9];
     for (int i = 0; i < 3; ++i)
@@ -612,7 +618,12 @@
     for (int i = 0; i < 3; ++i)
         for (int j = 0; j < 3; ++j) T[3 * i + j] = (Ka[i] * E[j] + Ka[3 + i] * E[3 + j]) + Ka[6 + i] * E[6 + j];
     for (int i = 0; i < 3; ++i)
-        for (int j = 0; j < 3; ++j) A.F[9 * k + 3 * i + j] = (T[3 * i] * Kb[j] + T[3 * i + 1] * Kb[3 + j]) + T[3 * i + 2] * Kb[6 + j];
+        for (int j = 0; j < 3; ++j) F[3 * i + j] = (T[3 * i] * Kb[j] + T[3 * i + 1] * Kb[3 + j]) + T[3 * i + 2] * Kb[6 + j];
+}
+__global__ void k_ncc_fmats(NcFmArgs A) {
+    const int k = threadIdx.x;
+    if (k >= A.n) return;
+    nc_fmat_pair(A, k, A.F + 9 * k);
 }
 extern "C" int cs_ncc_fmats_dev(int device, void* hip_stream, int nCams, int nPairs, const int* camA, const int* camB, const double* const* d_iK,
                                 const double* d_R, const double* d_t, double* d_F) {
@@ -672,7 +683,205 @@
     }
     CS_HIP(zero.run(s));
     if (n == 0) return CS_OK;
-    hipLaunchKernelGGL(k_ncc_epi_mat<true>, dim3((unsigned)((n + 64 * NC_CT - 1) / (64 * NC_CT)), (unsigned)((n + 63) / 64), (unsigned)nJobs), dim3(256), 0, s, J);
+    hipLaunchKernelGGL((k_ncc_epi_mat<true, false>), dim3((unsigned)((n + 64 * NC_CT - 1) / (64 * NC_CT)), (unsigned)((n + 63) / 64), (unsigned)nJobs), dim3(256), 0, s, J);
+    CS_CHECK_LAUNCH();
+    return CS_OK;
+}
+
+namespace {
+
+struct NcListSet {
+    cs_ncc_list_cam cam[NC_MAX_CAMS];
+};
+struct NcFrontArgs {
+    NcListSet L;
+    int nCams, N, own0, nOwn, mapCap, minTrack;
+    const int *state, *slot2map, *trackSpan;
+    const unsigned char* mapFlags;
+    int W, H, Wd, Hd, gx, gy;
+    double inv_scale;
+    NcFmArgs fm;
+    double* dF[NC_MAX_JOBS];
+    int* count[NC_MAX_JOBS];
+};
+constexpr int NC_LIST_TRIPS = 8;
+
+__global__ __launch_bounds__(256) void k_ncc_front(NcFrontArgs A) {
+    __shared__ int sWave[NC_LIST_TRIPS][4];
+    const int tid = threadIdx.x, lane = tid & 63, wv = tid >> 6;
+    int b = blockIdx.x;
+    if (b < A.nCams) {
+        const cs_ncc_list_cam& C = A.L.cam[b];
+        int base = 0;
+        for (int s0 = 0; s0 < A.N; s0 += 256 * NC_LIST_TRIPS) {
+            unsigned long long m[NC_LIST_TRIPS];
+            double px[NC_LIST_TRIPS], py[NC_LIST_TRIPS];
+#pragma unroll
+            for (int k = 0; k < NC_LIST_TRIPS; ++k) {
+                const int s = s0 + 256 * k + tid;
+                px[k] = s < A.N ? C.x[s] : 0.0, py[k] = s < A.N ? C.y[s] : 0.0;
+                const bool cand = s < A.N && cs_ncc_is_candidate(b, s, A.N, A.state, A.slot2map, A.trackSpan, A.mapFlags, A.mapCap, A.minTrack);
+                m[k] = __ballot(cand);
+                if (lane == 0) sWave[k][wv] = __popcll(m[k]);
+            }
+            __syncthreads();
+#pragma unroll
+            for (int k = 0; k < NC_LIST_TRIPS; ++k) {
+                int before = 0, total = 0;
+#pragma unroll
+                for (int w = 0; w < 4; ++w) {
+                    const int t = sWave[k][w];
+                    total += t;
+                    if (w < wv) before += t;
+                }
+                if ((m[k] >> lane) & 1ull) {
+                    const int s = s0 + 256 * k + tid;
+                    const int r = base + before + __popcll(m[k] & ((1ull << lane) - 1ull));
+                    C.idx[r] = s, C.xc[r] = px[k], C.yc[r] = py[k];
+                }
+                base += total;
+            }
+            __syncthreads();
+        }
+        if (tid == 0) *C.count = base;
+        return;
+    }
+    b -= A.nCams;
+    const int perCam = A.gx * A.gy;
+    if (b < perCam * A.nOwn) {
+        const int k = b / perCam, q = b - k * perCam;
+        const cs_ncc_list_cam& C = A.L.cam[A.own0 + k];
+        nc_resize_block(C.img, C.scaled, q % A.gx, q / A.gx, A.W, A.H, A.inv_scale, A.inv_scale, A.Wd, A.Hd);
+        return;
+    }
+    if (tid < A.fm.n) nc_fmat_pair(A.fm, tid, A.dF[tid]);
+    if (wv == 1 && lane < A.fm.n) *A.count[lane] = 0;
+}
+
+__global__ __launch_bounds__(256) void k_ncc_blocks_list(NcListSet S, int own0, int W, int H, double scale, int scaled) {
+    const cs_ncc_list_cam& C = S.cam[own0 + blockIdx.y];
+    const int r = blockIdx.x * 4 + (threadIdx.x >> 6);
+    if (r >= *C.count) return;
+    nc_cut_block(scaled ? C.scaled : C.img, W, H, C.xc[r], C.yc[r], scale, scaled, r, C.blocks, C.abc, nullptr);
+}
+
+int nc_list_cams(const char* who, NcListSet& S, int nCams, const cs_ncc_list_cam* cams, int N, int own0, int nOwn, double scale) {
+    if (nCams < 1 || nCams > NC_MAX_CAMS || !cams || N < 1 || own0 < 0 || nOwn < 0 || own0 + nOwn > nCams || !(scale > 0)) {
+        cs_set_error("%s: bad arguments (1..%d cameras, the own cameras among them, scale > 0)", who, NC_MAX_CAMS);
+        return CS_ERR_INVALID;
+    }
+    memset(&S, 0, sizeof(S));
+    for (int c = 0; c < nCams; ++c) {
+        const cs_ncc_list_cam& q = cams[c];
+        const bool own = c >= own0 && c < own0 + nOwn;
+        if (!q.x || !q.y || !q.idx || !q.xc || !q.yc || !q.count || !q.blocks || !q.abc || (own && (!q.img || (scale != 1.0 && !q.scaled)))) {
+            cs_set_error("%s: null pointer in camera %d", who, c);
+            return CS_ERR_INVALID;
+        }
+        S.cam[c] = q;
+    }
+    return CS_OK;
+}
+
+}
+
+extern "C" int cs_ncc_leg_front_dev(int device, void* hip_stream, int nCams, const cs_ncc_list_cam* cams, int N, const int* d_state,
+                                    const int* d_slot2map, const int* d_trackSpan, const unsigned char* d_mapFlags, int mapCap, int minTrack,
+                                    int own0, int nOwn, int W, int H, double scale, int nJobs, const cs_ncc_pair_job* jobs,
+                                    const double* const* d_iK, const double* d_R, const double* d_t) {
+    NcFrontArgs A;
+    memset(&A, 0, sizeof(A));
+    const int rc = nc_list_cams("cs_ncc_leg_front_dev", A.L, nCams, cams, N, own0, nOwn, scale);
+    if (rc != CS_OK) return rc;
+    if (!d_state || !d_slot2map || !d_trackSpan || !d_mapFlags || W <= 0 || H <= 0 || nJobs < 0 || nJobs > NC_MAX_JOBS ||
+        (nJobs && (!jobs || !d_iK || !d_R || !d_t))) {
+        cs_set_error("cs_ncc_leg_front_dev: bad arguments (<= %d camera pairs)", NC_MAX_JOBS);
+        return CS_ERR_INVALID;
+    }
+    A.nCams = nCams, A.N = N, A.own0 = own0, A.nOwn = nOwn, A.mapCap = mapCap, A.minTrack = minTrack;
+    A.state = d_state, A.slot2map = d_slot2map, A.trackSpan = d_trackSpan, A.mapFlags = d_mapFlags;
+    A.W = W, A.H = H, A.inv_scale = 1. / scale;
+    if (scale != 1.0 && nOwn > 0) {
+        A.Wd = (int)lrint(W * scale), A.Hd = (int)lrint(H * scale);
+        if (A.Wd < 1 || A.Hd < 1) {
+            cs_set_error("cs_ncc_leg_front_dev: the scaled image is empty");
+            return CS_ERR_INVALID;
+        }
+        A.gx = (A.Wd + 63) / 64, A.gy = (A.Hd + 3) / 4;
+    }
+    A.fm.n = nJobs, A.fm.R = d_R, A.fm.t = d_t;
+    for (int k = 0; k < nJobs; ++k) {
+        const cs_ncc_pair_job& q = jobs[k];
+        if (q.camA < 0 || q.camA >= nCams || q.camB < 0 || q.camB >= nCams || !d_iK[q.camA] || !d_iK[q.camB] || !q.dF || !q.count) {
+            cs_set_error("cs_ncc_leg_front_dev: bad job %d (cameras, dF and count are needed)", k);
+            return CS_ERR_INVALID;
+        }
+        A.fm.camA[k] = q.camA, A.fm.camB[k] = q.camB, A.fm.iK[k][0] = d_iK[q.camA], A.fm.iK[k][1] = d_iK[q.camB];
+        A.dF[k] = const_cast<double*>(q.dF), A.count[k] = q.count;
+    }
+    CS_HIP(hipSetDevice(device));
+    hipLaunchKernelGGL(k_ncc_front, dim3((unsigned)(nCams + A.gx * A.gy * nOwn + 1)), dim3(256), 0, (hipStream_t)hip_stream, A);
+    CS_CHECK_LAUNCH();
+    return CS_OK;
+}
+
+extern "C" int cs_ncc_list_blocks_dev(int device, void* hip_stream, int nCams, const cs_ncc_list_cam* cams, int own0, int nOwn, int W, int H,
+                                      int N, double scale) {
+    NcListSet S;
+    const int rc = nc_list_cams("cs_ncc_list_blocks_dev", S, nCams, cams, N, own0, nOwn, scale);
+    if (rc != CS_OK) return rc;
+    if (W <= 0 || H <= 0) {
+        cs_set_error("cs_ncc_list_blocks_dev: bad image size");
+        return CS_ERR_INVALID;
+    }
+    if (nOwn == 0) return CS_OK;
+    int Ws = W, Hs = H;
+    if (scale != 1.0) {
+        Ws = (int)lrint(W * scale), Hs = (int)lrint(H * scale);
+        if (Ws < 1 || Hs < 1) {
+            cs_set_error("cs_ncc_list_blocks_dev: the scaled image is empty");
+            return CS_ERR_INVALID;
+        }
+    }
+    CS_HIP(hipSetDevice(device));
+    hipLaunchKernelGGL(k_ncc_blocks_list, dim3((unsigned)((N + 3) / 4), (unsigned)nOwn), dim3(256), 0, (hipStream_t)hip_stream, S, own0, Ws, Hs,
+                       scale, scale != 1.0 ? 1 : 0);
+    CS_CHECK_LAUNCH();
+    return CS_OK;
+}
+
+extern "C" int cs_ncc_list_pairs_dev(int device, void* hip_stream, int nCams, const cs_ncc_list_cam* cams, int N, int nJobs,
+                                     const cs_ncc_pair_job* jobs, double epiMax, double nccMin, int pairCap) {
+    NcListSet S;
+    const int rc = nc_list_cams("cs_ncc_list_pairs_dev", S, nCams, cams, N, 0, 0, 1.0);
+    if (rc != CS_OK) return rc;
+    if (nJobs < 0 || nJobs > NC_MAX_JOBS || (nJobs && !jobs) || pairCap < 0) {
+        cs_set_error("cs_ncc_list_pairs_dev: bad arguments (<= %d camera pairs per call)", NC_MAX_JOBS);
+        return CS_ERR_INVALID;
+    }
+    if (nJobs == 0) return CS_OK;
+    NcJobs J;
+    memset(&J, 0, sizeof(J));
+    for (int k = 0; k < nJobs; ++k) {
+        const cs_ncc_pair_job& q = jobs[k];
+        if (q.camA < 0 || q.camA >= nCams || q.camB < 0 || q.camB >= nCams || !q.count || (pairCap > 0 && !q.pairs)) {
+            cs_set_error("cs_ncc_list_pairs_dev: bad job %d", k);
+            return CS_ERR_INVALID;
+        }
+        const cs_ncc_list_cam &a = S.cam[q.camA], &b = S.cam[q.camB];
+        NcArgs& A = J.job[k];
+        memcpy(A.F, q.F, sizeof(A.F));
+        A.dF = q.dF;
+        A.s1 = {a.xc, a.yc, a.blocks, a.abc, nullptr, N, a.count, a.idx};
+        A.s2 = {b.xc, b.yc, b.blocks, b.abc, nullptr, N, b.count, b.idx};
+        A.epiMax = epiMax, A.nccMin = nccMin, A.wNone = -1.0;
+        A.epiMat = A.nccMat = nullptr;
+        A.pairs = q.pairs, A.pairCap = pairCap, A.pairCount = q.count;
+    }
+    J.ct = NC_LIST_CT;
+    CS_HIP(hipSetDevice(device));
+    hipLaunchKernelGGL((k_ncc_epi_mat<true, true>), dim3((unsigned)((N + 64 * J.ct - 1) / (64 * J.ct)), (unsigned)((N + 63) / 64), (unsigned)nJobs),
+                       dim3(256), 0, (hipStream_t)hip_stream, J);
     CS_CHECK_LAUNCH();
     return CS_OK;
 }
diff --git a/coslam_amd/csrc/ncc_candidate_dev.h b/coslam_amd/csrc/ncc_candidate_dev.h
--- /dev/null
+++ b/coslam_amd/csrc/ncc_candidate_dev.h
@@ -0,0 +1,16 @@
+#pragma once
+
+#include "cs_common.h"
+
+#ifdef __HIPCC__
+__device__ __forceinline__ bool cs_ncc_is_candidate(int c, int s, int N, const int* __restrict__ state, const int* __restrict__ slot2map,
+                                                    const int* __restrict__ trackSpan, const unsigned char* __restrict__ mapFlags, int mapCap,
+                                                    int minTrack) {
+    const size_t q = (size_t)c * N + s;
+    const int st = state[q], m = slot2map[q];
+    const int f1 = trackSpan[(size_t)c * 2 * N + s], f2 = trackSpan[(size_t)c * 2 * N + N + s];
+    const bool tracked = (st == 0 || st == 1) && f1 >= 0 && f2 - f1 >= minTrack;
+    const bool freeOrFalse = m < 0 || (m < mapCap && (mapFlags[m] & CS_MAP_FALSE));
+    return tracked && freeOrFalse;
+}
+#endif
diff --git a/coslam_amd/csrc/newpts.hip b/coslam_amd/csrc/newpts.hip
--- a/coslam_amd/csrc/newpts.hip
+++ b/coslam_amd/csrc/newpts.hip
@@ -1,4 +1,5 @@
 #include "cs_common.h"
+#include "ncc_candidate_dev.h"
 #include "small_ops.h"
 
 #pragma clang fp contract(off)
@@ -508,11 +509,7 @@
     const int q = blockIdx.x * 256 + threadIdx.x;
     if (q >= n) return;
     const int c = q / N, s = q - c * N;
-    const int st = state[q], m = slot2map[q];
-    const int f1 = trackSpan[(size_t)c * 2 * N + s], f2 = trackSpan[(size_t)c * 2 * N + N + s];
-    const bool tracked = (st == 0 || st == 1) && f1 >= 0 && f2 - f1 >= minTrack;
-    const bool freeOrFalse = m < 0 || (m < mapCap && (mapFlags[m] & CS_MAP_FALSE));
-    valid[(size_t)c * validStride + s] = tracked && freeOrFalse ? 1 : 0;
+    valid[(size_t)c * validStride + s] = cs_ncc_is_candidate(c, s, N, state, slot2map, trackSpan, mapFlags, mapCap, minTrack) ? 1 : 0;
 }
 
 }
diff --git a/coslam_amd/frameloop.py b/coslam_amd/frameloop.py
--- a/coslam_amd/frameloop.py
+++ b/coslam_amd/frameloop.py
@@ -15,9 +15,9 @@
 from coslam_amd.handback import handback_cams, handback_dev
 from coslam_amd.liveview import LiveView
 from coslam_amd.keyframe import keyframe_cams, keyframe_ready_dev, keyframe_snapshot_dev
-from coslam_amd.ncc import (NCC_PAIR_DTYPE, ncc_cams, ncc_epi_pairs_group_dev, ncc_fmats_dev, ncc_get_blocks_group_dev, ncc_pair_jobs,
+from coslam_amd.ncc import (NCC_PAIR_DTYPE, ncc_leg_front_dev, ncc_list_blocks_dev, ncc_list_cams, ncc_list_pairs_dev, ncc_pair_jobs,
                             ncc_scaled_dims)
-from coslam_amd.newpts import NewPtsJob, ncc_candidate_mask_dev, newpts_from_pairs_dev, newpts_scratch_bytes
+from coslam_amd.newpts import NewPtsJob, newpts_from_pairs_dev, newpts_scratch_bytes
 from coslam_amd.pose import intraCamEstimate_batch_dev
 from coslam_amd.poseupdate import TrackHistory, poseupdate_cams
 from coslam_amd.register import (register_cams, register_cur_static_sequential_dev, register_decide_kinds_rounds_dev,
@@ -400,12 +400,14 @@
         self.ncc = dict(small=z((self.nc, ws_ * hs_), torch.uint8), rec=z((NA, rec), torch.uint8), rec_bytes=rec, runs=0,
                         send=z((self.nc, rec), torch.uint8) if self.world > 1 else None,
                         dF=z((NA - 1, 9), torch.float64),
+                        xyc=z((NA, 2 * N), torch.float64), count=z(NA, torch.int32),
                         pairs=z((NA - 1, cfg.ncc_pair_cap * NCC_PAIR_DTYPE.itemsize), torch.uint8), pair_count=z(NA - 1, torch.int32),
                         group={}, np_scr=z(newpts_scratch_bytes(NA, N), torch.uint8), np_cnt=z(4 + NA, torch.int32), new_total=0)
         r = self.ncc["rec"]
         self.ncc["blk"] = [r[g, :N * 128] for g in range(NA)]
         self.ncc["abc"] = [r[g, N * 128: N * 160] for g in range(NA)]
-        self.ncc["valid"] = [r[g, N * 160:] for g in range(NA)]
+        self.ncc["idx"] = [r[g, N * 160:] for g in range(NA)]
+        self.ncc["valid"] = [self.ncc["count"][g:g + 1] for g in range(NA)]
         cams = [dict(K=self.d_K1.data_ptr(), iK=self.d_iK1.data_ptr(), xy=self.d_xy[g].data_ptr(), state=self.d_state[g].data_ptr(),
                      slot2map=self.d_slot2map[g].data_ptr(), isStatic=self.d_isstatic[g].data_ptr(), reprojErr=self.d_reproj[g].data_ptr())
                 for g in range(NA)]
@@ -415,25 +417,22 @@
     def _ncc_leg(self, i, f, dst):
         cfg, nc, c0, N, NA, ncc = self.cfg, self.nc, self.c0, self.cfg.n_feat, self.cfg.n_cams, self.ncc
         s_ = self.pose_s.cuda_stream
-        ncc_candidate_mask_dev(s_, nc, N, self.d_state[c0].data_ptr(), self.d_slot2map[c0].data_ptr(), self.d_trackspan[c0].data_ptr(),
-                               self.d_mapflags.data_ptr(), self.n_map, ncc["valid"][c0].data_ptr(), device=self.device,
-                               validStride=ncc["rec"].stride(0) // 4)
         if f not in ncc["group"]:
-            own = ncc_cams([dict(img=self.img_ptrs[f][k], x=self.d_xy[c0 + k].data_ptr(), y=self.d_xy[c0 + k].data_ptr() + 8 * N,
-                                 scaled=ncc["small"][k].data_ptr(), blocks=ncc["blk"][c0 + k].data_ptr(), abc=ncc["abc"][c0 + k].data_ptr(),
-                                 valid=ncc["valid"][c0 + k].data_ptr()) for k in range(nc)])
-            allc = ncc_cams([dict(img=0, x=self.d_xy[g].data_ptr(), y=self.d_xy[g].data_ptr() + 8 * N, scaled=0, blocks=ncc["blk"][g].data_ptr(),
-                                  abc=ncc["abc"][g].data_ptr(), valid=ncc["valid"][g].data_ptr()) for g in range(NA)])
+            own = range(c0, c0 + nc)
+            allc = ncc_list_cams([dict(img=self.img_ptrs[f][g - c0] if g in own else 0, scaled=ncc["small"][g - c0].data_ptr() if g in own else 0,
+                                       x=self.d_xy[g].data_ptr(), y=self.d_xy[g].data_ptr() + 8 * N, idx=ncc["idx"][g].data_ptr(),
+                                       xc=ncc["xyc"][g].data_ptr(), yc=ncc["xyc"][g].data_ptr() + 8 * N, count=ncc["count"][g:g + 1].data_ptr(),
+                                       blocks=ncc["blk"][g].data_ptr(), abc=ncc["abc"][g].data_ptr()) for g in range(NA)])
             jobs_ = ncc_pair_jobs([dict(dF=ncc["dF"][a].data_ptr(), camA=a, camB=a + 1, pairs=ncc["pairs"][a].data_ptr(),
                                         count=ncc["pair_count"][a:a + 1].data_ptr()) for a in range(NA - 1)])
-            ncc["group"][f] = (own, allc, jobs_)
-        own, allc, jobs_ = ncc["group"][f]
-        ncc_get_blocks_group_dev(s_, own, cfg.W, cfg.H, N, 0.3, device=self.device)
+            ncc["group"][f] = (allc, jobs_, (C.c_void_p * NA)(*[self.d_iK1.data_ptr()] * NA))
+        allc, jobs_, ik = ncc["group"][f]
+        ncc_leg_front_dev(s_, allc, N, self.d_state.data_ptr(), self.d_slot2map.data_ptr(), self.d_trackspan.data_ptr(), self.d_mapflags.data_ptr(),
+                          self.n_map, c0, nc, cfg.W, cfg.H, 0.3, jobs_, ik, self.d_R[dst].data_ptr(), self.d_t[dst].data_ptr(), device=self.device)
+        ncc_list_blocks_dev(s_, allc, c0, nc, cfg.W, cfg.H, N, 0.3, device=self.device)
         if self.world > 1:
             self._gather_ncc_records()
-        ncc_fmats_dev(s_, NA, list(range(NA - 1)), list(range(1, NA)), [self.d_iK1.data_ptr()] * NA, self.d_R[dst].data_ptr(),
-                      self.d_t[dst].data_ptr(), ncc["dF"].data_ptr(), device=self.device)
-        ncc_epi_pairs_group_dev(s_, allc, N, jobs_, 50.0, 0.80, cfg.ncc_pair_cap, device=self.device)
+        ncc_list_pairs_dev(s_, allc, N, jobs_, 50.0, 0.80, cfg.ncc_pair_cap, device=self.device)
         newpts_from_pairs_dev(s_, ncc["job"], N, cfg.ncc_pair_cap, self.d_R[dst].data_ptr(), self.d_t[dst].data_ptr(), self.d_map.data_ptr(),
                               self.d_cov.data_ptr(), self.d_mapflags.data_ptr(), self.d_newpt.data_ptr(), self.d_firstfrm.data_ptr(),
                               self.d_pf.data_ptr(), self.n_map, self.d_mapcount.data_ptr(), i, ncc["np_scr"].data_ptr(), ncc["np_cnt"].data_ptr(),
diff --git a/coslam_amd/ncc.py b/coslam_amd/ncc.py
--- a/coslam_amd/ncc.py
+++ b/coslam_amd/ncc.py
@@ -83,6 +83,43 @@
                                            int(pairCap)), "cs_ncc_epi_pairs_group_dev")
 
 
+class NccListCam(C.Structure):
+    _c_type_ = "cs_ncc_list_cam"
+    _fields_ = [(n, C.c_void_p) for n in ("img", "scaled", "x", "y", "idx", "xc", "yc", "count", "blocks", "abc")]
+
+
+def ncc_list_cams(cams):
+    arr = (NccListCam * len(cams))()
+    for a, c in zip(arr, cams):
+        for n, _ in NccListCam._fields_:
+            v = c.get(n)
+            setattr(a, n, int(v) if v else None)
+    return arr
+
+
+def ncc_leg_front_dev(stream_ptr, cams, N, d_state, d_slot2map, d_trackSpan, d_mapFlags, mapCap, own0, nOwn, W, H, scale, jobs, d_iK, d_R,
+                      d_t, minTrack=3, device=0):
+    arr = cams if isinstance(cams, C.Array) else ncc_list_cams(cams)
+    jb = jobs if isinstance(jobs, C.Array) else ncc_pair_jobs(jobs)
+    ik = d_iK if isinstance(d_iK, C.Array) else (C.c_void_p * len(arr))(*[int(v) for v in d_iK])
+    check(lib().cs_ncc_leg_front_dev(int(device), stream_ptr, len(arr), arr, int(N), d_state, d_slot2map, d_trackSpan, d_mapFlags, int(mapCap),
+                                     int(minTrack), int(own0), int(nOwn), int(W), int(H), scale, len(jb), jb, ik, d_R, d_t),
+          "cs_ncc_leg_front_dev")
+
+
+def ncc_list_blocks_dev(stream_ptr, cams, own0, nOwn, W, H, N, scale, device=0):
+    arr = cams if isinstance(cams, C.Array) else ncc_list_cams(cams)
+    check(lib().cs_ncc_list_blocks_dev(int(device), stream_ptr, len(arr), arr, int(own0), int(nOwn), int(W), int(H), int(N), scale),
+          "cs_ncc_list_blocks_dev")
+
+
+def ncc_list_pairs_dev(stream_ptr, cams, N, jobs, epiMax, nccMin, pairCap, device=0):
+    arr = cams if isinstance(cams, C.Array) else ncc_list_cams(cams)
+    jb = jobs if isinstance(jobs, C.Array) else ncc_pair_jobs(jobs)
+    check(lib().cs_ncc_list_pairs_dev(int(device), stream_ptr, len(arr), arr, int(N), len(jb), jb, epiMax, nccMin, int(pairCap)),
+          "cs_ncc_list_pairs_dev")
+
+
 def ncc_match_between(img1, x1, y1, img2, x2, y2, scale, F, epiMax, nccMin, wNone=-1.0, device=0):
     img1 = np.ascontiguousarray(img1, dtype=np.uint8)
     img2 = np.ascontiguousarray(img2, dtype=np.uint8)
diff --git a/include/coslam_hip.h b/include/coslam_hip.h
--- a/include/coslam_hip.h
+++ b/include/coslam_hip.h
@@ -799,6 +799,26 @@
                                 double scale);
 int cs_ncc_epi_pairs_group_dev(int device, void* hip_stream, int nCams, const cs_ncc_cam* cams , int n, int nJobs,
                                const cs_ncc_pair_job* jobs , double epiMax, double nccMin, int pairCap);
+typedef struct cs_ncc_list_cam {
+    const unsigned char* img;
+    unsigned char* scaled;
+    const double* x;
+    const double* y;
+    int* idx;
+    double* xc;
+    double* yc;
+    int* count;
+    unsigned char* blocks;
+    double* abc;
+} cs_ncc_list_cam;
+int cs_ncc_leg_front_dev(int device, void* hip_stream, int nCams, const cs_ncc_list_cam* cams , int N, const int* d_state,
+                         const int* d_slot2map, const int* d_trackSpan, const unsigned char* d_mapFlags, int mapCap, int minTrack ,
+                         int own0, int nOwn, int W, int H, double scale, int nJobs, const cs_ncc_pair_job* jobs ,
+                         const double* const* d_iK , const double* d_R, const double* d_t);
+int cs_ncc_list_blocks_dev(int device, void* hip_stream, int nCams, const cs_ncc_list_cam* cams , int own0, int nOwn, int W, int H,
+                           int N, double scale);
+int cs_ncc_list_pairs_dev(int device, void* hip_stream, int nCams, const cs_ncc_list_cam* cams , int N, int nJobs,
+                          const cs_ncc_pair_job* jobs , double epiMax, double nccMin, int pairCap);
 int cs_ncc_unmapped_mask_dev(int device, void* hip_stream, int n, const int* d_state, const int* d_slot2map, int* d_valid);
 int cs_ncc_scaled_dims(int W, int H, double scale, int* Ws, int* Hs);
 int cs_ncc_get_blocks_dev(int device, void* hip_stream, const unsigned char* d_img, int W, int H, int n, const double* d_x,
```

After: 2098, median of 6. No clear change (+1.1%).
